# Kangfei/NNGP-src

Hardware: AMD Instinct MI355X
Metric: NNGP kernel-build + GP-solve wall-clock (ms) and GFLOP/s at N train queries (higher is better)
Workload: dtype f32 (Cholesky products as split f16 x3, f32 accumulate; f64 build/CG/means; the posterior's float64-grade residual as exact int8 digit-plane products); 1 GPU; synthetic N=32768, d=128, 5-layer ReLU NNGP + full Cholesky posterior (configs[2], north-star target); N=32768, d=128, n_relu=3, get=nngp, M_test=1024, parallelism=single GPU

## Files before the change

include/nngp_i8s.h:

```cpp
#ifndef NNGP_I8S_H
#define NNGP_I8S_H

#include "nngp_hip.h"

#ifdef __cplusplus
extern "C" {
#endif

int nngp_i8s_cut_rows(const double* src, int64_t ld, int64_t rows, int64_t cols, int32_t ns, const double* scale_in, double* scale_out,
                      int8_t* planes, int64_t ldp, double* writeback, void* stream);

int nngp_i8s_cut_sym(const double* src, int64_t ld, int64_t n, int32_t ns, double* scale_out, int8_t* planes, int64_t ldp,
                     int32_t by_rows, double* sqsum, void* stream);

int nngp_i8s_residual(double* out, int64_t ldo, const double* cin, int64_t ldcin, double* z, int64_t ldz, const double* kmat,
                      int64_t ldk, int64_t mp, int64_t n, double alpha, double beta, double gamma, int32_t ns_z, int32_t ns_k,
                      int32_t cut, int32_t round_z, int32_t sym, float* out32, const double* base, double* var, double* delta,
                      double* zstat, double* floor_rows, double* floor_z, void* stream);

#ifdef __cplusplus
}
#endif

#endif
```

nngp-src_amd/_lib.py:

```python
from __future__ import annotations

import ctypes
import os

import numpy as np

_HERE = os.path.dirname(os.path.abspath(__file__))
LIB_PATH = os.path.join(_HERE, "libnngp_hip.so")
KNOBS_LIB_PATH = os.path.join(_HERE, "libnngp_hip_knobs.so")

GET_NNGP, GET_NTK = 1, 2
DTYPE_F32, DTYPE_F64 = 0, 1
COV_NONE, COV_DIAG, COV_FULL = 0, 1, 2
MAX_DENSE = 16

ABI_SYMBOLS = (
    "nngp_version", "nngp_last_error", "nngp_kernel_build", "nngp_kernel_diag", "nngp_model_create",
    "nngp_model_destroy", "nngp_model_fit", "nngp_model_set_train", "nngp_model_build_rows",
    "nngp_model_factor", "nngp_model_factor_begin", "nngp_model_factor_panel", "nngp_model_factor_update",
    "nngp_model_factor_end", "nngp_model_factor_buffers", "nngp_model_solve", "nngp_model_append", "nngp_model_kernel_buffer", "nngp_model_info",
    "nngp_model_alpha", "nngp_model_predict", "nngp_model_set_refine", "nngp_model_cov_iters", "nngp_model_sweep_estimate", "nngp_model_factor_shift", "nngp_model_prepare_serving", "nngp_potrf_f32", "nngp_gemm_nt_f32",
    "nngp_gemm_nt_h3", "nngp_gemm_nt_f64", "nngp_trsm_rlt_f32", "nngp_model_apply_factor",
    "nngp_model_factor_input_rows", "nngp_model_factor_input_complete", "nngp_model_precond", "nngp_model_matvec_rows", "nngp_model_set_alpha", "nngp_encoder_create", "nngp_encoder_destroy", "nngp_encoder_dim",
    "nngp_encoder_encode", "nngp_comm_unique_id", "nngp_comm_create", "nngp_comm_destroy", "nngp_comm_library",
    "nngp_allgather_rows", "nngp_bcast", "nngp_model_update_timer", "nngp_model_update_timer_read", "nngp_symv_f64",
    "nngp_pool_select", "nngp_model_update_timer_bytes", "nngp_model_factor_update_cols", "nngp_gemm_nt_i8s", "nngp_model_residual_timer", "nngp_model_residual_timer_read", "nngp_model_trsm_timer", "nngp_model_trsm_timer_read", "nngp_model_residual_floor",
    "nngp_trsm_ticket_order", "nngp_trsm_ticket_queues", "nngp_model_reserve", "nngp_alloc_count",
)

GP_ABI_SYMBOLS = (
    "nngp_rbf_gp_create", "nngp_rbf_gp_destroy", "nngp_rbf_gp_set_train", "nngp_rbf_gp_evaluate", "nngp_rbf_gp_terms",
    "nngp_rbf_gp_predict", "nngp_rbf_gp_kernel", "nngp_rbf_gp_factor_buffer", "nngp_potrf_f64",
    "nngp_potrf_dinv_f64", "nngp_trsm_fwd_f64", "nngp_factor_solve_f64",
)


ACT_ABI_SYMBOLS = ("nngp_kernel_build_act", "nngp_kernel_diag_act", "nngp_model_create_act")
ACT_RELU, ACT_ABRELU, ACT_ERF = 0, 1, 2
ACTIVATIONS = {"relu": (ACT_RELU, 0), "abrelu": (ACT_ABRELU, 2), "erf": (ACT_ERF, 3)}

MLL_ABI_SYMBOLS = ("nngp_mll_create", "nngp_mll_destroy", "nngp_mll_set_train", "nngp_mll_evaluate", "nngp_mll_terms",
                   "nngp_mll_factor_buffer")


LOO_ABI_SYMBOLS = ("nngp_mll_loo_evaluate", "nngp_mll_loo_predictions", "nngp_mll_loo_terms")
LOO_NLPD, LOO_MSE = 0, 1

ARD_ABI_SYMBOLS = ("nngp_mll_reserve_ard", "nngp_mll_evaluate_ard", "nngp_mll_loo_evaluate_ard", "nngp_mll_ard_terms")

ADDITIVE_ABI_SYMBOLS = ("nngp_kernel_build_additive", "nngp_kernel_diag_additive", "nngp_model_create_additive")
MAX_GROUPS = 1024

ADDITIVE_MLL_ABI_SYMBOLS = ("nngp_mll_reserve_additive", "nngp_mll_evaluate_additive", "nngp_mll_additive_terms")

POOL_ABI_SYMBOLS = ("nngp_pool_select_greedy",)

SPARSE_ABI_SYMBOLS = ("nngp_sparse_create", "nngp_sparse_destroy", "nngp_sparse_set_inducing", "nngp_sparse_add_rows",
                      "nngp_sparse_finish", "nngp_sparse_predict", "nngp_sparse_info", "nngp_syrk_tn_f64")

SPARSE_EVIDENCE_ABI_SYMBOLS = ("nngp_sparse_reserve_evidence", "nngp_sparse_set_kernel", "nngp_sparse_evidence",
                               "nngp_sparse_evidence_grad", "nngp_sparse_evidence_terms", "nngp_sparse_adjoint_rect")
SPARSE_ARD_ABI_SYMBOLS = ("nngp_sparse_reserve_ard", "nngp_sparse_set_relevance", "nngp_sparse_evidence_grad_ard",
                          "nngp_sparse_ard_terms", "nngp_sparse_ard_rect")
I8S_ABI_SYMBOLS = ("nngp_i8s_cut_rows", "nngp_i8s_cut_sym", "nngp_i8s_residual")
MATFREE_ABI_SYMBOLS = ("nngp_matfree_create", "nngp_matfree_destroy", "nngp_matfree_fit", "nngp_matfree_solve",
                       "nngp_matfree_predict", "nngp_matfree_alpha", "nngp_matfree_info", "nngp_kmv_f64")
BOUND_DTC, BOUND_VFE = 0, 1
BOUNDS = {"dtc": BOUND_DTC, "vfe": BOUND_VFE}


class NngpArch(ctypes.Structure):
    _fields_ = [("n_dense", ctypes.c_int32), ("reserved", ctypes.c_int32),
                ("w_std", ctypes.c_double * MAX_DENSE), ("b_std", ctypes.c_double * MAX_DENSE)]


class NngpArchAct(ctypes.Structure):
    _fields_ = [("base", NngpArch), ("act", ctypes.c_int32 * (MAX_DENSE - 1)),
                ("p", (ctypes.c_double * 3) * (MAX_DENSE - 1))]


class NngpGroups(ctypes.Structure):
    _fields_ = [("n_groups", ctypes.c_int32), ("reserved", ctypes.c_int32),
                ("begin", ctypes.POINTER(ctypes.c_int32)), ("end", ctypes.POINTER(ctypes.c_int32)),
                ("weight", ctypes.POINTER(ctypes.c_double)), ("full_weight", ctypes.c_double)]


class NngpFitInfo(ctypes.Structure):
    _fields_ = [("reg", ctypes.c_double), ("trace_mean", ctypes.c_double), ("rel_residual", ctypes.c_double),
                ("refine_iters", ctypes.c_int32), ("clamped_pivots", ctypes.c_int32),
                ("n", ctypes.c_int64), ("n_padded", ctypes.c_int64)]


class NngpSparseInfo(ctypes.Structure):
    _fields_ = [("n", ctypes.c_int64), ("m", ctypes.c_int64), ("m_padded", ctypes.c_int64), ("chunks", ctypes.c_int64),
                ("sigma2", ctypes.c_double), ("trace_mean", ctypes.c_double), ("jitter_added", ctypes.c_double)]


class NngpMatfreeInfo(ctypes.Structure):
    _fields_ = [("n", ctypes.c_int64), ("m", ctypes.c_int64), ("sigma2", ctypes.c_double), ("iterations", ctypes.c_int32),
                ("k_passes", ctypes.c_int32), ("rel_residual", ctypes.c_double), ("converged", ctypes.c_int32),
                ("restarts", ctypes.c_int32)]


class NngpError(RuntimeError):
    pass


_libs = {}


def load(knobs: bool = False):
    knobs = bool(knobs) or os.environ.get("NNGP_KNOBS", "0") == "1"
    if knobs in _libs:
        return _libs[knobs]
    path = KNOBS_LIB_PATH if knobs else LIB_PATH
    if not os.path.exists(path):
        raise NngpError(
            "%s is missing (%s). Build it with `python -c 'import __graft_entry__ as g; g.build()'` "
            "or `make -C nngp-src_amd/csrc`; there is no CPU fallback." % (os.path.basename(path), path))
    import torch
    lib = ctypes.CDLL(path)
    bind_prototypes(lib, knobs)
    bind_gp_prototypes(lib)
    bind_act_prototypes(lib)
    bind_mll_prototypes(lib)
    bind_loo_prototypes(lib)
    bind_ard_prototypes(lib)
    bind_additive_prototypes(lib)
    bind_additive_mll_prototypes(lib)
    bind_pool_prototypes(lib)
    bind_sparse_prototypes(lib)
    bind_sparse_evidence_prototypes(lib)
    bind_sparse_ard_prototypes(lib)
    bind_i8s_prototypes(lib)
    bind_matfree_prototypes(lib)
    _libs[knobs] = lib
    return lib


def bind_prototypes(lib, knobs: bool = False):
    vp, i64, i32, dbl = ctypes.c_void_p, ctypes.c_int64, ctypes.c_int32, ctypes.c_double
    archp = ctypes.POINTER(NngpArch)
    lib.nngp_version.restype = ctypes.c_int
    lib.nngp_last_error.restype = ctypes.c_char_p
    if knobs:
        lib.nngp_debug_set.argtypes = [i32, i32]
        lib.nngp_debug_set.restype = ctypes.c_int
    lib.nngp_kernel_build.argtypes = [vp, i64, vp, i64, i32, archp, i32, vp, vp, i64, i64, i64, vp]
    lib.nngp_kernel_diag.argtypes = [vp, i64, i32, archp, vp, vp, vp]
    lib.nngp_model_create.argtypes = [ctypes.POINTER(vp), i64, i64, i32, i32, archp, i32, dbl, i32]
    lib.nngp_model_destroy.argtypes = [vp]
    lib.nngp_model_fit.argtypes = [vp, vp, vp, i64, vp]
    lib.nngp_model_set_train.argtypes = [vp, vp, vp, i64, vp]
    lib.nngp_model_build_rows.argtypes = [vp, i64, i64, vp]
    lib.nngp_model_factor.argtypes = [vp, vp]
    lib.nngp_model_factor_begin.argtypes = [vp, vp]
    lib.nngp_model_factor_panel.argtypes = [vp, i64, i64, vp]
    lib.nngp_model_factor_update.argtypes = [vp, i64, i64, i64, i64, vp]
    lib.nngp_model_factor_end.argtypes = [vp, vp]
    lib.nngp_model_factor_buffers.argtypes = [vp, ctypes.POINTER(vp), ctypes.POINTER(i64), ctypes.POINTER(vp)]
    lib.nngp_model_solve.argtypes = [vp, i32, dbl, vp]
    lib.nngp_model_kernel_buffer.argtypes = [vp, ctypes.POINTER(vp), ctypes.POINTER(i64)]
    lib.nngp_model_info.argtypes = [vp, ctypes.POINTER(NngpFitInfo)]
    lib.nngp_model_alpha.argtypes = [vp, vp, vp]
    lib.nngp_model_predict.argtypes = [vp, vp, i64, i32, vp, vp, vp]
    lib.nngp_encoder_create.argtypes = [ctypes.POINTER(vp), ctypes.c_char_p, i32, i32]
    lib.nngp_encoder_destroy.argtypes = [vp]
    lib.nngp_encoder_dim.argtypes = [vp]
    lib.nngp_encoder_encode.argtypes = [vp, ctypes.c_char_p, i64, i32, vp, vp, i64, ctypes.POINTER(i64)]
    lib.nngp_model_set_refine.argtypes = [vp, i32]
    lib.nngp_model_cov_iters.argtypes = [vp]
    lib.nngp_model_prepare_serving.argtypes = [vp, vp]
    lib.nngp_model_factor_shift.argtypes = [vp]
    lib.nngp_model_factor_shift.restype = ctypes.c_double
    lib.nngp_model_cov_iters.restype = ctypes.c_int
    lib.nngp_model_sweep_estimate.argtypes = [vp, ctypes.POINTER(dbl), ctypes.POINTER(dbl)]
    lib.nngp_model_append.argtypes = [vp, vp, vp, i64, vp]
    lib.nngp_gemm_nt_f64.argtypes = [vp, i64, vp, i64, vp, i64, vp, i64, i64, i64, i64, dbl, dbl, vp]
    lib.nngp_gemm_nt_i8s.argtypes = [vp, i64, vp, i64, vp, i64, vp, i64, i64, i64, i64, dbl, dbl, i32, i32, i32, vp]
    lib.nngp_potrf_f32.argtypes = [vp, i64, i64, vp, vp, vp]
    lib.nngp_gemm_nt_f32.argtypes = [vp, i64, vp, i64, vp, i64, i64, i64, i64, ctypes.c_float, ctypes.c_float, i32, vp]
    lib.nngp_gemm_nt_h3.argtypes = [vp, i64, vp, i64, vp, i64, i64, i64, i64, ctypes.c_float, ctypes.c_float,
                                    ctypes.c_float, i32, vp]
    lib.nngp_trsm_rlt_f32.argtypes = [vp, i64, i64, vp, i64, vp, i64, vp]
    lib.nngp_model_apply_factor.argtypes = [vp, vp, i64, i32, vp]
    lib.nngp_model_factor_input_rows.argtypes = [vp, i64, i64, ctypes.c_double, vp]
    lib.nngp_model_factor_input_complete.argtypes = [vp]
    lib.nngp_model_precond.argtypes = [vp, vp, vp, vp]
    lib.nngp_model_matvec_rows.argtypes = [vp, vp, vp, i64, i64, vp]
    lib.nngp_model_set_alpha.argtypes = [vp, vp, i32, ctypes.c_double, vp]
    lib.nngp_comm_unique_id.argtypes = [vp]
    lib.nngp_comm_create.argtypes = [ctypes.POINTER(vp), vp, i32, i32]
    lib.nngp_comm_destroy.argtypes = [vp]
    lib.nngp_comm_library.restype = ctypes.c_char_p
    lib.nngp_allgather_rows.argtypes = [vp, i64, i64, i32, vp, vp]
    lib.nngp_bcast.argtypes = [vp, i64, i32, i32, vp, vp]
    lib.nngp_symv_f64.argtypes = [vp, i64, i64, vp, vp, dbl, vp]
    lib.nngp_pool_select.argtypes = [vp, i64, i32, vp, i64, i32, ctypes.c_uint64, vp, vp]
    lib.nngp_model_update_timer.argtypes = [vp, i32]
    lib.nngp_model_update_timer_read.argtypes = [vp, ctypes.POINTER(i64), ctypes.POINTER(dbl), ctypes.POINTER(dbl)]
    lib.nngp_model_update_timer_bytes.argtypes = [vp, ctypes.POINTER(dbl)]
    lib.nngp_model_residual_timer.argtypes = [vp, i32]
    lib.nngp_model_residual_floor.argtypes = [vp, ctypes.POINTER(dbl), ctypes.POINTER(i32)]
    lib.nngp_model_residual_timer_read.argtypes = [vp, ctypes.POINTER(i64), ctypes.POINTER(dbl), ctypes.POINTER(dbl), ctypes.POINTER(dbl)]
    lib.nngp_model_trsm_timer.argtypes = [vp, i32]
    lib.nngp_model_trsm_timer_read.argtypes = [vp, ctypes.POINTER(i64), ctypes.POINTER(dbl), ctypes.POINTER(dbl)]
    lib.nngp_model_reserve.argtypes = [vp, i64, i32]
    lib.nngp_alloc_count.argtypes = []
    lib.nngp_trsm_ticket_order.argtypes = [i32, i32, i32, i32, i32, i32, vp, i64, ctypes.POINTER(i64)]
    lib.nngp_trsm_ticket_queues.argtypes = [i32, i32, i32, i32, i32, i32, i32, vp, vp, i64, ctypes.POINTER(i64)]
    lib.nngp_model_factor_update_cols.argtypes = [vp, i64, i64, ctypes.POINTER(i64), i32, i64, vp]
    for name in ABI_SYMBOLS:
        if name not in ("nngp_last_error", "nngp_model_factor_shift", "nngp_comm_library", "nngp_alloc_count"):
            getattr(lib, name).restype = ctypes.c_int
    lib.nngp_alloc_count.restype = ctypes.c_int64
    return lib

# ... 8 lines not shown
    lib.nngp_rbf_gp_predict.argtypes = [vp, vp, i64, i32, vp, vp, vp]
    lib.nngp_rbf_gp_kernel.argtypes = [vp, i64, vp, i64, i32, dbl, vp, i64, vp]
    lib.nngp_rbf_gp_factor_buffer.argtypes = [vp, ctypes.POINTER(vp), ctypes.POINTER(i64), ctypes.POINTER(i64)]
    lib.nngp_potrf_f64.argtypes = [vp, i64, i64, vp]
    lib.nngp_potrf_dinv_f64.argtypes = [vp, i64, i64, vp, vp]
    lib.nngp_trsm_fwd_f64.argtypes = [vp, i64, i64, vp, i64, vp, i64, i32, vp]
    lib.nngp_factor_solve_f64.argtypes = [vp, i64, vp, i64, i32, vp, vp, vp, vp, vp, vp, vp]
    for name in GP_ABI_SYMBOLS:
        getattr(lib, name).restype = ctypes.c_int
    return lib


def bind_act_prototypes(lib):
    vp, i64, i32, dbl = ctypes.c_void_p, ctypes.c_int64, ctypes.c_int32, ctypes.c_double
    archp = ctypes.POINTER(NngpArchAct)
    lib.nngp_kernel_build_act.argtypes = [vp, i64, vp, i64, i32, archp, i32, vp, vp, i64, i64, i64, vp]
    lib.nngp_kernel_diag_act.argtypes = [vp, i64, i32, archp, vp, vp, vp]
    lib.nngp_model_create_act.argtypes = [ctypes.POINTER(vp), i64, i64, i32, i32, archp, i32, dbl, i32]
    for name in ACT_ABI_SYMBOLS:
        getattr(lib, name).restype = ctypes.c_int
    return lib


def bind_mll_prototypes(lib):
    vp, i64, i32, dbl = ctypes.c_void_p, ctypes.c_int64, ctypes.c_int32, ctypes.c_double
    lib.nngp_mll_create.argtypes = [ctypes.POINTER(vp), i64, i32]
    lib.nngp_mll_destroy.argtypes = [vp]
    lib.nngp_mll_set_train.argtypes = [vp, vp, vp, i64, i32, vp]
    lib.nngp_mll_evaluate.argtypes = [vp, ctypes.POINTER(NngpArchAct), dbl, i32, ctypes.POINTER(dbl), ctypes.POINTER(dbl), vp]
    lib.nngp_mll_terms.argtypes = [vp, ctypes.POINTER(dbl), i32]
    lib.nngp_mll_factor_buffer.argtypes = [vp, ctypes.POINTER(vp), ctypes.POINTER(i64), ctypes.POINTER(i64)]
    for name in MLL_ABI_SYMBOLS:
        getattr(lib, name).restype = ctypes.c_int
    return lib


def bind_loo_prototypes(lib):
    vp, i32, dbl = ctypes.c_void_p, ctypes.c_int32, ctypes.c_double
    lib.nngp_mll_loo_evaluate.argtypes = [vp, ctypes.POINTER(NngpArchAct), i32, dbl, i32, i32, ctypes.POINTER(dbl),
                                          ctypes.POINTER(dbl), vp]
    lib.nngp_mll_loo_predictions.argtypes = [vp, vp, vp, vp]
    lib.nngp_mll_loo_terms.argtypes = [vp, ctypes.POINTER(dbl), i32]
    for name in LOO_ABI_SYMBOLS:
        getattr(lib, name).restype = ctypes.c_int
    return lib


def bind_ard_prototypes(lib):
    vp, i32, dbl = ctypes.c_void_p, ctypes.c_int32, ctypes.c_double
    pd = ctypes.POINTER(dbl)
    lib.nngp_mll_reserve_ard.argtypes = [vp]
    lib.nngp_mll_evaluate_ard.argtypes = [vp, ctypes.POINTER(NngpArchAct), pd, dbl, i32, pd, pd, pd, vp]
    lib.nngp_mll_loo_evaluate_ard.argtypes = [vp, ctypes.POINTER(NngpArchAct), i32, pd, dbl, i32, i32, pd, pd, pd, vp]
    lib.nngp_mll_ard_terms.argtypes = [vp, pd, i32]
    for name in ARD_ABI_SYMBOLS:
        getattr(lib, name).restype = ctypes.c_int
    return lib


def bind_additive_prototypes(lib):
    vp, i64, i32, dbl = ctypes.c_void_p, ctypes.c_int64, ctypes.c_int32, ctypes.c_double
    archp, groupsp = ctypes.POINTER(NngpArchAct), ctypes.POINTER(NngpGroups)
    lib.nngp_kernel_build_additive.argtypes = [vp, i64, vp, i64, i32, archp, groupsp, i32, vp, vp, i64, i64, i64, vp]
    lib.nngp_kernel_diag_additive.argtypes = [vp, i64, i32, archp, groupsp, vp, vp, vp]
    lib.nngp_model_create_additive.argtypes = [ctypes.POINTER(vp), i64, i64, i32, i32, archp, groupsp, i32, dbl, i32]
    for name in ADDITIVE_ABI_SYMBOLS:
        getattr(lib, name).restype = ctypes.c_int
    return lib


def bind_additive_mll_prototypes(lib):
    vp, i32, dbl = ctypes.c_void_p, ctypes.c_int32, ctypes.c_double
    pd = ctypes.POINTER(dbl)
    lib.nngp_mll_reserve_additive.argtypes = [vp, ctypes.POINTER(NngpGroups)]
    lib.nngp_mll_evaluate_additive.argtypes = [vp, ctypes.POINTER(NngpArchAct), pd, dbl, i32, pd, pd, pd, vp]
    lib.nngp_mll_additive_terms.argtypes = [vp, pd, i32]
    for name in ADDITIVE_MLL_ABI_SYMBOLS:
        getattr(lib, name).restype = ctypes.c_int
    return lib


def bind_pool_prototypes(lib):
    vp, i64, dbl = ctypes.c_void_p, ctypes.c_int64, ctypes.c_double
    lib.nngp_pool_select_greedy.argtypes = [vp, i64, i64, dbl, i64, vp, vp, vp, i64, vp]
    for name in POOL_ABI_SYMBOLS:
        getattr(lib, name).restype = ctypes.c_int
    return lib


def bind_sparse_prototypes(lib):
    vp, i64, i32, dbl = ctypes.c_void_p, ctypes.c_int64, ctypes.c_int32, ctypes.c_double
    lib.nngp_sparse_create.argtypes = [ctypes.POINTER(vp), i64, i64, i64, i32, i32, ctypes.POINTER(NngpArchAct),
                                       ctypes.POINTER(NngpGroups), dbl, i32, dbl]
    lib.nngp_sparse_destroy.argtypes = [vp]
    lib.nngp_sparse_set_inducing.argtypes = [vp, vp, i64, vp]
    lib.nngp_sparse_add_rows.argtypes = [vp, vp, vp, i64, vp]
    lib.nngp_sparse_finish.argtypes = [vp, vp]
    lib.nngp_sparse_predict.argtypes = [vp, vp, i64, i32, vp, vp, vp]
    lib.nngp_sparse_info.argtypes = [vp, ctypes.POINTER(NngpSparseInfo)]
    lib.nngp_syrk_tn_f64.argtypes = [vp, i64, vp, vp, i64, vp, i64, i64, i32, dbl, vp]
    for name in SPARSE_ABI_SYMBOLS:
        getattr(lib, name).restype = ctypes.c_int
    return lib


def bind_sparse_evidence_prototypes(lib):
    vp, i64, i32, dbl = ctypes.c_void_p, ctypes.c_int64, ctypes.c_int32, ctypes.c_double
    pd, archp = ctypes.POINTER(dbl), ctypes.POINTER(NngpArchAct)
    lib.nngp_sparse_reserve_evidence.argtypes = [vp]
    lib.nngp_sparse_set_kernel.argtypes = [vp, archp, dbl, i32]
    lib.nngp_sparse_evidence.argtypes = [vp, i32, pd, vp]
    lib.nngp_sparse_evidence_grad.argtypes = [vp, vp, vp, i64, i32, pd, pd, vp]
    lib.nngp_sparse_evidence_terms.argtypes = [vp, pd, i32]
    lib.nngp_sparse_adjoint_rect.argtypes = [vp, i64, vp, i64, i32, archp, vp, i64, vp, vp, pd, vp]
    for name in SPARSE_EVIDENCE_ABI_SYMBOLS:
        getattr(lib, name).restype = ctypes.c_int
    return lib


def bind_sparse_ard_prototypes(lib):
    vp, i64, i32, dbl = ctypes.c_void_p, ctypes.c_int64, ctypes.c_int32, ctypes.c_double
    pd, archp = ctypes.POINTER(dbl), ctypes.POINTER(NngpArchAct)
    lib.nngp_sparse_reserve_ard.argtypes = [vp]
    lib.nngp_sparse_set_relevance.argtypes = [vp, pd]
    lib.nngp_sparse_evidence_grad_ard.argtypes = [vp, vp, vp, i64, i32, pd, pd, pd, vp]
    lib.nngp_sparse_ard_terms.argtypes = [vp, pd, i32]
    lib.nngp_sparse_ard_rect.argtypes = [vp, i64, vp, i64, i32, archp, pd, vp, i64, vp, vp, pd, vp]
    for name in SPARSE_ARD_ABI_SYMBOLS:
        getattr(lib, name).restype = ctypes.c_int
    return lib


def bind_matfree_prototypes(lib):
    vp, i64, i32, dbl = ctypes.c_void_p, ctypes.c_int64, ctypes.c_int32, ctypes.c_double
    archp = ctypes.POINTER(NngpArchAct)
    lib.nngp_matfree_create.argtypes = [ctypes.POINTER(vp), i64, i64, i64, i64, i32, i32, archp, ctypes.POINTER(NngpGroups), i32, dbl,
                                        i32, dbl]
    lib.nngp_matfree_destroy.argtypes = [vp]
    lib.nngp_matfree_fit.argtypes = [vp, vp, vp, i64, vp, i64, dbl, i32, vp]
    lib.nngp_matfree_solve.argtypes = [vp, vp, i64, i32, vp, i64, dbl, i32, vp]
    lib.nngp_matfree_predict.argtypes = [vp, vp, i64, i32, vp, vp, dbl, i32, vp]
    lib.nngp_matfree_alpha.argtypes = [vp, vp, vp]
    lib.nngp_matfree_info.argtypes = [vp, ctypes.POINTER(NngpMatfreeInfo)]
    lib.nngp_kmv_f64.argtypes = [vp, i64, vp, i64, i32, vp, i64, i32, archp, dbl, vp]
    for name in MATFREE_ABI_SYMBOLS:
        getattr(lib, name).restype = ctypes.c_int
    return lib


def bind_i8s_prototypes(lib):
    vp, i64, i32, dbl = ctypes.c_void_p, ctypes.c_int64, ctypes.c_int32, ctypes.c_double
    lib.nngp_i8s_cut_rows.argtypes = [vp, i64, i64, i64, i32, vp, vp, vp, i64, vp, vp]
    lib.nngp_i8s_cut_sym.argtypes = [vp, i64, i64, i32, vp, vp, i64, i32, vp, vp]
    lib.nngp_i8s_residual.argtypes = [vp, i64, vp, i64, vp, i64, vp, i64, i64, i64, dbl, dbl, dbl, i32, i32, i32, i32, i32,
                                      vp, vp, vp, vp, vp, vp, vp, vp]
    for name in I8S_ABI_SYMBOLS:
        getattr(lib, name).restype = ctypes.c_int
    return lib


def check(rc: int, lib=None):
    if rc != 0:
        msg = (lib or load()).nngp_last_error()
        raise NngpError("libnngp_hip: rc=%d: %s" % (rc, (msg or b"").decode("utf-8", "replace")))


def make_arch(w_std, b_std) -> NngpArch:
    w_std = [float(v) for v in w_std]
    b_std = [float(v) for v in b_std]
    if len(w_std) != len(b_std) or not 1 <= len(w_std) <= MAX_DENSE:
        raise ValueError("architecture must have 1..%d Dense layers" % MAX_DENSE)
    arch = NngpArch()
    arch.n_dense = len(w_std)
    for i, (w, b) in enumerate(zip(w_std, b_std)):
        arch.w_std[i] = w
        arch.b_std[i] = b
    return arch


def canonical_activation(spec):
    kind = spec[0]
    if kind == "relu":
        return ("relu",)
    if kind == "abrelu" and len(spec) == 3:
        a, b = float(spec[1]), float(spec[2])
        return ("relu",) if (a == 0.0 and b == 1.0) else ("abrelu", a, b)
    if kind == "erf" and len(spec) == 4:
        return ("erf", float(spec[1]), float(spec[2]), float(spec[3]))
    raise ValueError("unknown activation %r" % (spec,))


def all_relu(activations) -> bool:
    return activations is None or all(canonical_activation(a) == ("relu",) for a in activations)


def make_arch_act(w_std, b_std, activations) -> NngpArchAct:
    arch = NngpArchAct()
    arch.base = make_arch(w_std, b_std)
    activations = list(activations)
    if len(activations) != arch.base.n_dense - 1:
        raise ValueError("%d Dense layers need %d activations, got %d" % (arch.base.n_dense, arch.base.n_dense - 1,
                                                                          len(activations)))
    for l, spec in enumerate(activations):
        spec = canonical_activation(spec)
        arch.act[l] = ACTIVATIONS[spec[0]][0]
        for e, v in enumerate(spec[1:]):
            arch.p[l][e] = v
    return arch


def pair_groups(d: int):
    d = int(d)
    if d < 2 or d % 2 != 0:
        raise ValueError("pair groups need an even number of features >= 2, got d = %d" % d)
    return tuple((i, i + 2) for i in range(0, d, 2))


def check_groups(groups, weights=None, full_weight=1.0, d=None):
    if isinstance(groups, str):
        if groups != "pairs":
            raise ValueError("groups must be a list of (begin, end) ranges or 'pairs', got %r" % (groups,))
        if d is None:
            raise ValueError("groups='pairs' needs the number of features")
        groups = pair_groups(d)
    try:
        out = tuple((int(b), int(e)) for b, e in groups)
        if any(float(b) != ib or float(e) != ie for (b, e), (ib, ie) in zip(groups, out)):
            raise TypeError
    except (TypeError, ValueError):
        raise ValueError("groups must be a list of (begin, end) integer ranges, got %r" % (groups,)) from None
    if len(out) > MAX_GROUPS:
        raise ValueError("at most %d groups, got %d" % (MAX_GROUPS, len(out)))
    for b, e in out:
        if not (0 <= b < e) or (d is not None and e > int(d)):
            raise ValueError("group range [%d, %d) is outside 0 <= begin < end%s" % (b, e, "" if d is None else " <= d = %d" % int(d)))
    w = (1.0,) * len(out) if weights is None else tuple(float(v) for v in weights)
    if len(w) != len(out):
        raise ValueError("%d groups need %d weights, got %d" % (len(out), len(out), len(w)))
    w0 = float(full_weight)
    if not all(np.isfinite(v) and v >= 0.0 for v in w + (w0,)):
        raise ValueError("group weights and full_weight must be finite and >= 0")
    if w0 == 0.0 and not any(v > 0.0 for v in w):
        raise ValueError("all weights are zero: the additive kernel has no term")
    return out, w, w0


def make_groups(groups, weights, full_weight) -> NngpGroups:
    g = NngpGroups()
    n = len(groups)
    g.n_groups = n
    g._begin = (ctypes.c_int32 * max(n, 1))(*[b for b, _ in groups])
    g._end = (ctypes.c_int32 * max(n, 1))(*[e for _, e in groups])
    g._weight = (ctypes.c_double * max(n, 1))(*weights)
    g.begin = ctypes.cast(g._begin, ctypes.POINTER(ctypes.c_int32))
    g.end = ctypes.cast(g._end, ctypes.POINTER(ctypes.c_int32))
    g.weight = ctypes.cast(g._weight, ctypes.POINTER(ctypes.c_double))
    g.full_weight = float(full_weight)
    return g


def require_gpu():
    import torch
    if not torch.cuda.is_available():
        raise NngpError("no MI355X/ROCm device visible: the NNGP hot path has no CPU fallback")
    return torch.device("cuda", torch.cuda.current_device())


def to_device_f64(a, device=None):
    import torch
    device = device or require_gpu()
    if isinstance(a, torch.Tensor):
        return a.to(device=device, dtype=torch.float64).contiguous()
    return torch.from_numpy(np.ascontiguousarray(a, dtype=np.float64)).to(device)


def stream_ptr():
    import torch
    return ctypes.c_void_p(torch.cuda.current_stream().cuda_stream)


def ptr(t):
    return ctypes.c_void_p(0 if t is None else t.data_ptr())
```

nngp-src_amd/csrc/api_ops.hip:

```cpp
#include "model.h"
#include "gp_f64.h"
#include "trsm_order.h"
#include "../../include/nngp_i8s.h"

extern "C" {

int nngp_trsm_ticket_order(int32_t row_tiles, int32_t block_cols, int32_t tail_tiles, int32_t backward, int32_t workers, int32_t merged,
                           int32_t* items, int64_t cap, int64_t* count) {
    return tk_order_export(row_tiles, block_cols, tail_tiles, backward, workers, merged, 1, items, nullptr, cap, count);
}

int nngp_trsm_ticket_queues(int32_t row_tiles, int32_t block_cols, int32_t tail_tiles, int32_t backward, int32_t workers, int32_t merged,
                            int32_t queues, int32_t* items, int32_t* queue_of, int64_t cap, int64_t* count) {
    return tk_order_export(row_tiles, block_cols, tail_tiles, backward, workers, merged, queues, items, queue_of, cap, count);
}

int nngp_potrf_f32(float* a, int64_t n, int64_t ld, float* dinv, int32_t* clamped, void* stream) {
    NNGP_REQUIRE(a != nullptr && dinv != nullptr, "potrf_f32: NULL argument");
    if (clamped) NNGP_HIP_CHECK(hipMemsetAsync(clamped, 0, sizeof(int32_t), (hipStream_t)stream));
    return potrf_f32(a, n, ld, dinv, clamped, 0.0f, (hipStream_t)stream);
}

int nngp_potrf_f64(double* a, int64_t n, int64_t ld, void* stream) {
    hipStream_t s = (hipStream_t)stream;
// ... 54 lines not shown
    if (l) NNGP_HIP_CHECK(hipMemcpyAsync(l, w->a, mat, hipMemcpyDeviceToDevice, s));
    if (wout) NNGP_HIP_CHECK(hipMemcpyAsync(wout, w->wrow, vec, hipMemcpyDeviceToDevice, s));
    if (zt) NNGP_HIP_CHECK(hipMemcpyAsync(zt, w->zt, mat, hipMemcpyDeviceToDevice, s));
    if (ainv) NNGP_HIP_CHECK(hipMemcpyAsync(ainv, w->ainv, mat, hipMemcpyDeviceToDevice, s));
    if (alpha) NNGP_HIP_CHECK(hipMemcpyAsync(alpha, w->alpha, vec, hipMemcpyDeviceToDevice, s));
    NNGP_HIP_CHECK(hipStreamSynchronize(s));
    return 0;
}
}

int nngp_factor_solve_f64(const double* a, int64_t lda, const double* y, int64_t n, int32_t mode, double* l, double* w, double* zt,
                          double* ainv, double* alpha, double* neg_rowsq, void* stream) {
    hipStream_t s = (hipStream_t)stream;
    NNGP_REQUIRE(a != nullptr && y != nullptr && n >= 1 && lda >= n, "factor_solve_f64: need a, y, n >= 1 and lda >= n (n=%lld lda=%lld)",
                 (long long)n, (long long)lda);
    NNGP_REQUIRE(mode == kGpSolveW || mode == kGpSolveInverse || mode == kGpSolveRows, "factor_solve_f64: unknown mode %d", (int)mode);
    NNGP_REQUIRE(mode != kGpSolveW || (zt == nullptr && alpha == nullptr && neg_rowsq == nullptr),
                 "factor_solve_f64: mode 0 produces L and w only");
    NNGP_REQUIRE(mode == kGpSolveInverse || ainv == nullptr, "factor_solve_f64: only mode 1 produces A^-1");
    GpWorkspace ws;
    const int rc = factor_solve_on(&ws, a, lda, y, n, mode, l, w, zt, ainv, alpha, neg_rowsq, s);
    if (rc != 0) (void)hipStreamSynchronize(s);
    ws_free(&ws);
    return rc;
}

int nngp_gemm_nt_f32(float* c, int64_t ldc, const float* a, int64_t lda, const float* b, int64_t ldb, int64_t m,
                     int64_t n, int64_t k, float alpha, float beta, int32_t lower_only, void* stream) {
    NNGP_REQUIRE(a != nullptr && b != nullptr && c != nullptr, "gemm_nt_f32: NULL argument");
    return launch_gemm_nt_f32(c, ldc, a, lda, b, ldb, m, n, k, alpha, beta, lower_only != 0, (hipStream_t)stream);
}

namespace {
struct H3Scratch {
    hipStream_t stream = nullptr;
    char* p = nullptr;
    size_t bytes = 0;
    bool used = false;
};
std::mutex g_h3_scratch_mutex;
H3Scratch g_h3_scratch[4];

int h3_scratch_get(hipStream_t s, size_t bytes, char** out) {
    std::lock_guard<std::mutex> lock(g_h3_scratch_mutex);
    H3Scratch* e = nullptr;
    for (auto& c : g_h3_scratch)
        if (c.used && c.stream == s) e = &c;
    if (e == nullptr)
        for (auto& c : g_h3_scratch)
            if (!c.used && e == nullptr) e = &c;
    if (e == nullptr) {
        e = &g_h3_scratch[0];
        if (hipStreamSynchronize(e->stream) != hipSuccess) {
            (void)hipGetLastError();
            NNGP_HIP_CHECK(hipDeviceSynchronize());
        }
        (void)hipFree(e->p);
        *e = H3Scratch();
    }
    if (e->bytes < bytes) {
        if (e->p != nullptr) {
            NNGP_HIP_CHECK(hipStreamSynchronize(s));
            (void)hipFree(e->p);
            e->p = nullptr;
            e->bytes = 0;
        }
        NNGP_HIP_CHECK(hipMalloc((void**)&e->p, bytes));
        e->bytes = bytes;
    }
    e->used = true;
    e->stream = s;
    *out = e->p;
    return 0;
}
}

int nngp_gemm_nt_h3(float* c, int64_t ldc, const float* a, int64_t lda, const float* b, int64_t ldb, int64_t m, int64_t n,
                    int64_t k, float alpha, float beta, float scale, int32_t lower_only, void* stream) {
    hipStream_t s = (hipStream_t)stream;
    NNGP_REQUIRE(a != nullptr && b != nullptr && c != nullptr && scale > 0.0f, "gemm_nt_h3: bad argument");
    NNGP_REQUIRE(m > 0 && n > 0 && k > 0 && k % 32 == 0, "gemm_nt_h3: k must be a multiple of 32");
    const int64_t mp = round_up(m, 256), np = round_up(n, 256), ldp = 4 * k;
    char* pa = nullptr;
    NNGP_TRY(h3_scratch_get(s, (size_t)((mp + np) * ldp + 64), &pa));
    char* pb = pa + mp * ldp;
    int* counters = reinterpret_cast<int*>(pb + np * ldp);
    if (mp > m) NNGP_HIP_CHECK(hipMemsetAsync(pa + m * ldp, 0, (size_t)((mp - m) * ldp), s));
    NNGP_HIP_CHECK(hipMemsetAsync(pb + n * ldp, 0, (size_t)((np - n) * ldp + 64), s));
    NNGP_TRY(launch_split_rows(a, lda, m, k, scale, pa, ldp, s));
    NNGP_TRY(launch_split_rows(b, ldb, n, k, scale, pb, ldp, s));
    return launch_gemm_nt_h3(c, ldc, pa, pb, ldp, m, n, k, alpha / (scale * scale), beta, lower_only != 0, 0, counters,
                             NNGP_KNOB(4) > 0 ? NNGP_KNOB(4) : 0, s);
}

int nngp_gemm_nt_f64(double* c, int64_t ldc, const double* cin, int64_t ldcin, const double* a, int64_t lda,
                     const double* b, int64_t ldb, int64_t m, int64_t n, int64_t k, double alpha, double beta,
                     void* stream) {
    NNGP_REQUIRE(a != nullptr && b != nullptr && c != nullptr, "gemm_nt_f64: NULL argument");
    return launch_gemm_nt_f64(c, ldc, cin, ldcin, a, lda, b, ldb, m, n, k, alpha, beta, (hipStream_t)stream);
}

int nngp_gemm_nt_i8s(double* c, int64_t ldc, const double* cin, int64_t ldcin, const double* a, int64_t lda, const double* b,
                     int64_t ldb, int64_t m, int64_t n, int64_t k, double alpha, double beta, int32_t slices_a, int32_t slices_b,
                     int32_t cut, void* stream) {
    hipStream_t s = (hipStream_t)stream;
    NNGP_REQUIRE(a != nullptr && b != nullptr && c != nullptr && m > 0 && n > 0 && k > 0 && m % TB == 0 && n % TB == 0 && ldc >= n &&
                     lda >= k && ldb >= k,
                 "gemm_nt_i8s: m, n must be multiples of %d", TB);
    I8Plan pl;
    NNGP_TRY(i8s_plan(slices_a, slices_b, cut, &pl));
    const int64_t mp = round_up(m, 256), np = round_up(n, 256), kp = round_up(k, 128);
    const int64_t nchunk = i8s_chunks(k, &pl);
    const int64_t slab = m * n;
    const size_t plane_bytes = (size_t)((mp * slices_a + np * slices_b) * kp);
    const size_t part_bytes = (size_t)(nchunk * pl.ndiag * slab) * sizeof(int32_t);
    NNGP_REQUIRE(part_bytes < (size_t)16 << 30, "gemm_nt_i8s: the test entry keeps all partial products (16 GB limit)");
    char* ws = nullptr;
    NNGP_HIP_CHECK(hipMalloc((void**)&ws, plane_bytes + part_bytes + sizeof(double) * (size_t)(m + n) + 64));
    NNGP_HIP_CHECK(hipMemsetAsync(ws, 0, plane_bytes, s));
    int8_t* pa = reinterpret_cast<int8_t*>(ws);
    int8_t* pb = pa + mp * slices_a * kp;
    int32_t* part = reinterpret_cast<int32_t*>(ws + plane_bytes);
    double* sca = reinterpret_cast<double*>(ws + plane_bytes + part_bytes);
    double* scb = sca + m;
    int* counters = reinterpret_cast<int*>(scb + n);
    NNGP_HIP_CHECK(hipMemsetAsync(counters, 0, 64, s));
    int rc = launch_i8s_slice_rows(a, lda, m, k, slices_a, nullptr, sca, pa, kp, mp * kp, s);
    if (rc == 0) rc = launch_i8s_slice_rows(b, ldb, n, k, slices_b, nullptr, scb, pb, kp, np * kp, s);
    if (rc == 0)
        rc = launch_gemm_nt_i8s(part, n, slab, pa, kp, mp * kp, pb, kp, np * kp, pl, m, n, k, counters,
                                NNGP_KNOB(4) > 0 ? NNGP_KNOB(4) : 0, s);
    if (rc == 0)
        rc = launch_i8s_combine(c, ldc, cin ? cin : c, cin ? ldcin : ldc, beta, alpha, nullptr, 0, 0.0, part, n, slab, (int)nchunk,
                                pl.ndiag, sca, scb, m, n, s);
    (void)hipStreamSynchronize(s);
    (void)hipFree(ws);
    return rc;
}

int nngp_i8s_cut_rows(const double* src, int64_t ld, int64_t rows, int64_t cols, int32_t ns, const double* scale_in, double* scale_out,
                      int8_t* planes, int64_t ldp, double* writeback, void* stream) {
    NNGP_REQUIRE(src != nullptr && planes != nullptr && (scale_in != nullptr || scale_out != nullptr), "i8s_cut_rows: NULL argument");
    NNGP_REQUIRE(ns >= 2 && ns <= 7, "i8s_cut_rows: 2..7 planes (ns=%d)", (int)ns);
    NNGP_REQUIRE(rows > 0 && cols > 0 && ld >= cols && ld % 2 == 0, "i8s_cut_rows: ld must be even and >= cols (rows=%lld cols=%lld ld=%lld)",
                 (long long)rows, (long long)cols, (long long)ld);
    NNGP_REQUIRE(ldp >= round_up(cols, 128) && ldp % 16 == 0, "i8s_cut_rows: ldp must be a multiple of 16 and >= cols rounded up to 128 (ldp=%lld)",
                 (long long)ldp);
    NNGP_REQUIRE((((uintptr_t)src | (uintptr_t)planes | (uintptr_t)writeback) & 15) == 0, "i8s_cut_rows: operands must be 16-byte aligned");
    return launch_i8s_slice_rows(src, ld, rows, cols, ns, scale_in, scale_out, planes, ldp, rows * ldp, (hipStream_t)stream, writeback);
}

int nngp_i8s_cut_sym(const double* src, int64_t ld, int64_t n, int32_t ns, double* scale_out, int8_t* planes, int64_t ldp,
                     int32_t by_rows, double* sqsum, void* stream) {
    hipStream_t s = (hipStream_t)stream;
    NNGP_REQUIRE(src != nullptr && planes != nullptr && scale_out != nullptr, "i8s_cut_sym: NULL argument");
    NNGP_REQUIRE(by_rows != 0 ? (ns >= 2 && ns <= 7) : (ns == 5 || ns == 7), "i8s_cut_sym: 5 or 7 planes (by rows: 2..7) (ns=%d)", (int)ns);
    NNGP_REQUIRE(n > 0 && n % TB == 0 && ld >= n && ld % 2 == 0, "i8s_cut_sym: n must be a positive multiple of %d, ld even and >= n (n=%lld ld=%lld)",
                 TB, (long long)n, (long long)ld);
    NNGP_REQUIRE(ldp >= n && ldp % 16 == 0, "i8s_cut_sym: ldp must be a multiple of 16 and >= n (ldp=%lld)", (long long)ldp);
    NNGP_REQUIRE((((uintptr_t)src | (uintptr_t)planes) & 15) == 0, "i8s_cut_sym: operands must be 16-byte aligned");
    NNGP_TRY(launch_i8s_diag_bound_scale(src, ld, n, scale_out, s));
    if (by_rows != 0)
        NNGP_TRY(launch_i8s_slice_rows(src, ld, n, n, ns, scale_out, nullptr, planes, ldp, n * ldp, s));
    else
        NNGP_TRY(launch_i8s_slice_sym(src, ld, n, ns, scale_out, planes, ldp, n * ldp, s));
    if (sqsum != nullptr) NNGP_TRY(launch_i8s_scale_sqsum(scale_out, n, sqsum, s));
    return 0;
}

namespace {
struct I8sResidualWs {
    int8_t *kplanes, *zplanes;
    double *kscale, *zscale, *rowpart;
    int32_t* partial;
    int* counters;
};

int i8s_residual_on(const I8sResidualWs& w, const I8Plan& pl, double* out, int64_t ldo, const double* cin, int64_t ldcin, double* z, int64_t ldz,
                    const double* kmat, int64_t ldk, int64_t mp, int64_t n, double alpha, double beta, double gamma, int ns_z, int ns_k,
                    bool round_z, bool sym, float* out32, const double* base, double* var, double* delta, double* zstat,
                    double* floor_rows, double* floor_z, hipStream_t s) {
    const int64_t kr = round_up(n, 256), zr = round_up(mp, 256);
    NNGP_TRY(launch_i8s_diag_bound_scale(kmat, ldk, n, w.kscale, s));
    if (sym)
        NNGP_TRY(launch_i8s_slice_sym(kmat, ldk, n, ns_k, w.kscale, w.kplanes, n, kr * n, s));
    else
        NNGP_TRY(launch_i8s_slice_rows(kmat, ldk, n, n, ns_k, w.kscale, nullptr, w.kplanes, n, kr * n, s));
    NNGP_TRY(launch_i8s_scale_sqsum(w.kscale, n, w.kscale + n, s));
    const int64_t nchunk = i8s_chunks(n, &pl), slab = mp * n;
    NNGP_TRY(launch_i8s_slice_rows(z, ldz, mp, n, ns_z, nullptr, w.zscale, w.zplanes, n, zr * n, s, round_z ? z : nullptr));
    NNGP_TRY(launch_gemm_nt_i8s(w.partial, n, slab, w.zplanes, n, zr * n, w.kplanes, n, kr * n, pl, mp, n, n, w.counters, 0, s));
    I8Fuse fuse;
    fuse.out32 = out32;
    fuse.ld32 = n;
    fuse.part = w.rowpart;
    NNGP_TRY(launch_i8s_combine(out, ldo, cin, ldcin, beta, alpha, z, ldz, gamma, w.partial, n, slab, (int)nchunk, pl.ndiag, w.zscale,
                                w.kscale, mp, n, s, out32 != nullptr ? &fuse : nullptr));
    if (out32 != nullptr) {
        NNGP_TRY(launch_i8s_rowstat_finish(w.rowpart, n, mp, base, var, delta, zstat, s));
        if (floor_rows != nullptr) {
            NNGP_HIP_CHECK(hipMemsetAsync(floor_rows, 0, sizeof(double), s));
            NNGP_TRY(launch_i8s_floor_ratio_rows(zstat, mp, var, pl, ns_z, ns_k, w.kscale + n, reinterpret_cast<unsigned long long*>(floor_rows), s));
        }
        if (floor_z != nullptr) {
            NNGP_HIP_CHECK(hipMemsetAsync(floor_z, 0, sizeof(double), s));
            NNGP_TRY(launch_i8s_floor_ratio(z, ldz, mp, n, var, pl, ns_z, ns_k, w.kscale + n, reinterpret_cast<unsigned long long*>(floor_z), s));
        }
    }
    return 0;
}
}

int nngp_i8s_residual(double* out, int64_t ldo, const double* cin, int64_t ldcin, double* z, int64_t ldz, const double* kmat,
                      int64_t ldk, int64_t mp, int64_t n, double alpha, double beta, double gamma, int32_t ns_z, int32_t ns_k,
                      int32_t cut, int32_t round_z, int32_t sym, float* out32, const double* base, double* var, double* delta,
                      double* zstat, double* floor_rows, double* floor_z, void* stream) {
    hipStream_t s = (hipStream_t)stream;
    NNGP_REQUIRE(out != nullptr && z != nullptr && kmat != nullptr && (beta == 0.0 || cin != nullptr), "i8s_residual: NULL argument");
    NNGP_REQUIRE(mp > 0 && n > 0 && mp % TB == 0 && n % TB == 0, "i8s_residual: mp, n must be positive multiples of %d (mp=%lld n=%lld)", TB,
                 (long long)mp, (long long)n);
    NNGP_REQUIRE(ns_z >= 2 && ns_z <= 7 && ns_k >= 2 && ns_k <= 7, "i8s_residual: 2..7 planes per operand (ns_z=%d ns_k=%d)", (int)ns_z, (int)ns_k);
    NNGP_REQUIRE(cut >= 0, "i8s_residual: cut must be >= 0 (cut=%d)", (int)cut);
    NNGP_REQUIRE(sym == 0 || ns_k == 5 || ns_k == 7, "i8s_residual: the symmetric cut makes 5 or 7 planes (ns_k=%d)", (int)ns_k);
    NNGP_REQUIRE(ldo >= n && ldz >= n && ldk >= n && (cin == nullptr || ldcin >= n) && ldo % 2 == 0 && ldz % 2 == 0 && ldk % 2 == 0 &&
                     (cin == nullptr || ldcin % 2 == 0),
                 "i8s_residual: leading dimensions must be even and >= n (ldo=%lld ldcin=%lld ldz=%lld ldk=%lld)", (long long)ldo,
                 (long long)ldcin, (long long)ldz, (long long)ldk);
    NNGP_REQUIRE((((uintptr_t)out | (uintptr_t)cin | (uintptr_t)z | (uintptr_t)kmat | (uintptr_t)out32) & 15) == 0,
                 "i8s_residual: operands must be 16-byte aligned");
    const bool any = out32 || base || var || delta || zstat, all = out32 && base && var && delta && zstat;
    NNGP_REQUIRE(any == all, "i8s_residual: the fused outputs (out32, base, var, delta, zstat) come all or none");
    NNGP_REQUIRE(!all || cin != nullptr, "i8s_residual: the fused outputs need cin");
    NNGP_REQUIRE(all || (floor_rows == nullptr && floor_z == nullptr), "i8s_residual: the floor ratios need the fused outputs");
    I8Plan pl;
    NNGP_TRY(i8s_plan(ns_z, ns_k, cut, &pl));
    const int64_t kr = round_up(n, 256), zr = round_up(mp, 256), nchunk = i8s_chunks(n, &pl);
    const size_t kp_bytes = (size_t)(ns_k * kr * n), zp_bytes = (size_t)(ns_z * zr * n);
    const size_t part_bytes = (size_t)(nchunk * pl.ndiag * mp * n) * sizeof(int32_t);
    const size_t f64s = (size_t)(n + 2) + (size_t)mp + (size_t)(mp * i8s_col_blocks(n) * 4);
    NNGP_REQUIRE(part_bytes < (size_t)16 << 30, "i8s_residual: the test entry keeps all partial products (16 GB limit)");
    char* ws = nullptr;
    NNGP_HIP_CHECK(hipMallocAsync(reinterpret_cast<void**>(&ws), kp_bytes + zp_bytes + part_bytes + sizeof(double) * f64s + 64, s));
    I8sResidualWs w;
    w.kplanes = reinterpret_cast<int8_t*>(ws);
    w.zplanes = w.kplanes + kp_bytes;
    w.partial = reinterpret_cast<int32_t*>(ws + kp_bytes + zp_bytes);
    w.kscale = reinterpret_cast<double*>(ws + kp_bytes + zp_bytes + part_bytes);
    w.zscale = w.kscale + n + 2;
    w.rowpart = w.zscale + mp;
    w.counters = reinterpret_cast<int*>(w.rowpart + mp * i8s_col_blocks(n) * 4);
    int rc = 0;
    if (hipMemsetAsync(ws, 0, kp_bytes + zp_bytes, s) != hipSuccess || hipMemsetAsync(w.counters, 0, 64, s) != hipSuccess) {
        nngp::set_error("i8s_residual: hipMemsetAsync failed");
        rc = -1;
    }
    if (rc == 0)
        rc = i8s_residual_on(w, pl, out, ldo, cin, ldcin, z, ldz, kmat, ldk, mp, n, alpha, beta, gamma, ns_z, ns_k, round_z != 0, sym != 0,
                             out32, base, var, delta, zstat, floor_rows, floor_z, s);
    (void)hipFreeAsync(ws, s);
    return rc;
}

int nngp_pool_select(const double* mean, int64_t m, int32_t ny, const double* var, int64_t count, int32_t biased, uint64_t seed,
                     int64_t* indices, void* stream) {
    hipStream_t s = (hipStream_t)stream;
    NNGP_REQUIRE(mean != nullptr && var != nullptr && indices != nullptr && m > 0 && ny >= 1 && count >= 0 && count <= m,
                 "pool_select: bad arguments (m=%lld, count=%lld)", (long long)m, (long long)count);
    if (count == 0) return 0;
    double* key = nullptr;
    NNGP_HIP_CHECK(hipMallocAsync(reinterpret_cast<void**>(&key), sizeof(double) * (size_t)m, s));
    const int rc = launch_pool_select(mean, m, ny, var, count, biased != 0, seed, key, indices, s);
    NNGP_HIP_CHECK(hipFreeAsync(key, s));
    return rc;
}

int nngp_pool_select_greedy(const double* cov, int64_t m, int64_t ld, double noise, int64_t count, int64_t* indices, double* gains,
                            double* factor, int64_t ldf, void* stream) {
    hipStream_t s = (hipStream_t)stream;
    NNGP_REQUIRE(cov != nullptr && indices != nullptr, "pool_select_greedy: NULL cov or indices");
    NNGP_REQUIRE(m >= 1 && count >= 0 && count <= m, "pool_select_greedy: need m >= 1 and 0 <= count <= m (m=%lld, count=%lld)",
                 (long long)m, (long long)count);
    NNGP_REQUIRE(ld >= m, "pool_select_greedy: ld < m (ld=%lld, m=%lld)", (long long)ld, (long long)m);
    NNGP_REQUIRE(factor == nullptr || ldf >= m, "pool_select_greedy: ldf < m (ldf=%lld, m=%lld)", (long long)ldf, (long long)m);
    NNGP_REQUIRE(noise >= 0.0 && noise <= 1.7976931348623157e308, "pool_select_greedy: noise must be finite and >= 0 (noise=%g)", noise);
    if (count == 0) return 0;
    const size_t own = (factor == nullptr) ? (size_t)count * (size_t)m : 0;
    double* ws = nullptr;
    NNGP_HIP_CHECK(hipMallocAsync(reinterpret_cast<void**>(&ws), sizeof(double) * ((size_t)2 * (size_t)m + own), s));
    const int rc = launch_pool_greedy(cov, m, ld, noise, count, indices, gains, own ? ws + 2 * m : factor, own ? m : ldf, ws, s);
    NNGP_HIP_CHECK(hipFreeAsync(ws, s));
    return rc;
}

int nngp_syrk_tn_f64(double* c, int64_t ldc, double* r, const double* a, int64_t lda, const double* y, int64_t rows, int64_t mp,
                     int32_t ny, double beta, void* stream) {
    hipStream_t s = (hipStream_t)stream;
    NNGP_TRY(syrk_check(c, ldc, r, a, lda, y, rows, mp, ny, beta));
    double* ws = nullptr;
    const int64_t ws_doubles = syrk_ws_doubles(rows, mp);
    NNGP_HIP_CHECK(hipMallocAsync(reinterpret_cast<void**>(&ws), sizeof(double) * (size_t)ws_doubles, s));
    const int rc = launch_syrk_tn_f64(c, ldc, r, a, lda, y, rows, mp, ny, beta, ws, ws_doubles, s);
    NNGP_HIP_CHECK(hipFreeAsync(ws, s));
    return rc;
}

int nngp_symv_f64(const double* a, int64_t lda, int64_t n, const double* x, double* y, double diag_add, void* stream) {
    hipStream_t s = (hipStream_t)stream;
    NNGP_REQUIRE(a != nullptr && x != nullptr && y != nullptr && n > 0 && lda >= n, "symv_f64: bad arguments");
    const int64_t np = round_up(n, TB);
    double* part = nullptr;
    NNGP_HIP_CHECK(hipMallocAsync(reinterpret_cast<void**>(&part), sizeof(double) * (size_t)(np / TB) * np, s));
    const int rc = launch_symv_f64(a, lda, n, x, y, diag_add, part, np, s);
    NNGP_HIP_CHECK(hipFreeAsync(part, s));
    return rc;
}

int nngp_trsm_rlt_f32(float* b, int64_t ldb, int64_t m, const float* l, int64_t ldl, const float* dinv, int64_t n,
                      void* stream) {
    NNGP_REQUIRE(b != nullptr && l != nullptr && dinv != nullptr, "trsm_rlt_f32: NULL argument");
    NNGP_REQUIRE(m % TB == 0 && n % TB == 0 && m > 0 && n > 0, "trsm_rlt_f32: m, n must be multiples of %d", TB);
    return trsm_rlt_f32(b, ldb, m, l, ldl, dinv, n, (hipStream_t)stream);
}

}
```

nngp-src_amd/csrc/api_predict.hip:

```cpp
#include "model.h"

namespace nngp {

int ensure_predict_capacity(nngp_model* m, int64_t mt, bool need_ktd) {
    if (mt > m->m_cap || m->b32 == nullptr) {
        const int64_t cap = mt > m->m_cap ? mt : m->m_cap;
        NNGP_HIP_CHECK(hipDeviceSynchronize());
        dev_free(m->xt_q); dev_free(m->tt_diag); dev_free(m->b32); dev_free(m->trsm_tmp);
        NNGP_TRY(dev_alloc(&m->xt_q, cap));
        NNGP_TRY(dev_alloc(&m->tt_diag, cap));
        NNGP_TRY(dev_alloc(&m->b32, round_up(cap, TB) * m->np_cap));
        NNGP_TRY(dev_alloc(&m->trsm_tmp, round_up(cap, TB) * triinv_block(m->np_cap)));
        if (m->split.planes != nullptr) {
            dev_free(m->split.planes_b); dev_free(m->split.row_inv);
            m->split.planes_b = nullptr; m->split.row_inv = nullptr;
            m->split.mb_cap = round_up(cap, TB);
            m->split.b_panels = (int)((triinv_block(m->np_cap) + m->split.k_cap - 1) / m->split.k_cap);
            NNGP_TRY(dev_alloc(&m->split.planes_b, (int64_t)(m->split.b_panels - 1) * m->split.col_stride + (m->split.mb_cap + 256) * m->split.k_cap * 4));
            NNGP_TRY(dev_alloc(&m->split.row_inv, m->split.mb_cap));
            tk_destroy(m->tk);
            m->tk = nullptr;
            if (m->split.k_cap == 1024 && triinv_block(m->np_cap) == 1024) NNGP_TRY(tk_create(&m->tk, m->np_cap, m->split.mb_cap) < 0 ? -1 : 0);
        }
        m->m_cap = cap;
    }
    if (need_ktd && mt > m->ktd_cap) {
        const int64_t cap = mt > m->m_cap ? mt : m->m_cap;
        NNGP_HIP_CHECK(hipDeviceSynchronize());
        dev_free(m->ktd64);
        NNGP_TRY(dev_alloc(&m->ktd64, round_up(cap, TB) * m->np_cap));
        m->ktd_cap = cap;
    }
    return 0;
}

int ensure_full_cov_capacity(nngp_model* m, int64_t mt) {
    if (mt > m->full_cap) {
        NNGP_HIP_CHECK(hipDeviceSynchronize());
        dev_free(m->ktt64); dev_free(m->vvt32);
        const int64_t mp = round_up(mt, TB);
        dev_free(m->covp64);
        NNGP_TRY(dev_alloc(&m->ktt64, mp * mp));
        NNGP_TRY(dev_alloc(&m->vvt32, mp * mp));
        NNGP_TRY(dev_alloc(&m->covp64, mp * mp));
        m->full_cap = mt;
    }
    return 0;
}

void set_split_scale(nngp_model* m) {
    const double lmax = sqrt(fmax(m->diag_max, m->trace_mean) + m->reg_fac);
    int e = 0;
    (void)frexp(lmax, &e);
    m->split.scale = (lmax > 0.0 && std::isfinite(lmax)) ? (float)ldexp(1.0, 15 - e) : 1.0f;
}

int ensure_refine_capacity(nngp_model* m, int64_t mp) {
    if (mp > m->refine_cap) {
        NNGP_HIP_CHECK(hipDeviceSynchronize());
        dev_free(m->z64); dev_free(m->r64);
        NNGP_TRY(dev_alloc(&m->z64, mp * m->np_cap));
        NNGP_TRY(dev_alloc(&m->r64, mp * m->np_cap));
        m->refine_cap = mp;
    }
    if (mp > m->rows.cap) {
        NNGP_HIP_CHECK(hipDeviceSynchronize());
        RowsPcg& w = m->rows;
        dev_free(w.rho); dev_free(w.coef); dev_free(w.tol); dev_free(w.delta); dev_free(w.var); dev_free(w.state); dev_free(w.zstat);
        NNGP_TRY(dev_alloc(&w.rho, mp)); NNGP_TRY(dev_alloc(&w.coef, mp)); NNGP_TRY(dev_alloc(&w.tol, mp));
        NNGP_TRY(dev_alloc(&w.delta, mp)); NNGP_TRY(dev_alloc(&w.var, mp)); NNGP_TRY(dev_alloc(&w.state, mp));
        NNGP_TRY(dev_alloc(&w.zstat, 2 * mp));
        if (w.live == nullptr) {
            NNGP_TRY(dev_alloc(&w.live, 6));
            NNGP_HIP_CHECK(hipHostMalloc(reinterpret_cast<void**>(&w.host), 6 * sizeof(int32_t), hipHostMallocDefault));
        }
        w.cap = mp;
    }
    return 0;
}

int ensure_lt_alloc(nngp_model* m) {
    if (m->lt32 != nullptr) return 0;
    NNGP_HIP_CHECK(hipDeviceSynchronize());
    NNGP_TRY(dev_alloc(&m->lt32, m->np_cap * m->np_cap));
    NNGP_TRY(dev_alloc(&m->dinvt, (m->np_cap / TB) * TB * TB));
    return 0;
}
int ensure_lt(nngp_model* m, hipStream_t s) {
    if (m->lt_ready) return 0;
    NNGP_TRY(ensure_lt_alloc(m));
    NNGP_TRY(launch_transpose_f32(m->a32, m->ld, m->lt32, m->np, m->np, s));
    NNGP_TRY(launch_transpose_blocks_f32(m->dinv, m->dinvt, TB, m->np / TB, s));
    m->lt_ready = true;
    return 0;
}

int ensure_lt_split(nngp_model* m, hipStream_t s) {
    if (m->split.lt_ready) return 0;
    if (m->split.planes_t == nullptr) {
        NNGP_HIP_CHECK(hipDeviceSynchronize());
        const int64_t ncols = (m->np_cap + m->split.k_cap - 1) / m->split.k_cap;
        NNGP_TRY(dev_alloc(&m->split.planes_t, ncols * m->split.col_stride));
    }
    NNGP_TRY(launch_split_lower_t(m->a32, m->ld, m->np, m->split.k_cap, m->split.scale, m->split.planes_t,
                                  m->split.col_stride, s));
    m->split.lt_ready = true;
    return 0;
}


int tri_join(nngp_model* m, hipStream_t s) {
    if (m->tri_stale) {
        if (m->ev_tri == nullptr) NNGP_HIP_CHECK(hipEventCreateWithFlags(&m->ev_tri, hipEventDisableTiming));
        NNGP_TRY(triinv_build(m->a32, m->ld, m->dinv, m->np, m->tri, s));
        if (m->tk != nullptr && m->tri.bs == 1024) NNGP_TRY(tk_prepare_inverses(m->tk, m->tri, m->np, m->a32, m->ld, s));
        NNGP_HIP_CHECK(hipEventRecord(m->ev_tri, s));
        m->tri_stale = false;
        m->tri_pending = true;
        return 0;
    }
    if (m->tri_pending) NNGP_HIP_CHECK(hipStreamWaitEvent(s, m->ev_tri, 0));
    if (m->tk != nullptr && !tk_inverses_ready(m->tk) && m->tri.bs == 1024) {
        NNGP_TRY(tk_prepare_inverses(m->tk, m->tri, m->np, m->a32, m->ld, s));
        if (m->ev_tri == nullptr) NNGP_HIP_CHECK(hipEventCreateWithFlags(&m->ev_tri, hipEventDisableTiming));
        NNGP_HIP_CHECK(hipEventRecord(m->ev_tri, s));
        m->tri_pending = true;
    }
    return 0;
}

int tri_fork(nngp_model* m, hipStream_t s) {
    if (!m->tri_stale || m->la == nullptr || m->la->panel == nullptr || NNGP_KNOB(5) == 61) return 0;
    if (m->ev_tri == nullptr) NNGP_HIP_CHECK(hipEventCreateWithFlags(&m->ev_tri, hipEventDisableTiming));
    if (m->ev_tri_fork == nullptr) NNGP_HIP_CHECK(hipEventCreateWithFlags(&m->ev_tri_fork, hipEventDisableTiming));
    NNGP_HIP_CHECK(hipEventRecord(m->ev_tri_fork, s));
    NNGP_HIP_CHECK(hipStreamWaitEvent(m->la->panel, m->ev_tri_fork, 0));
    NNGP_TRY(triinv_build(m->a32, m->ld, m->dinv, m->np, m->tri, m->la->panel));
    if (m->tk != nullptr && m->tri.bs == 1024) NNGP_TRY(tk_prepare_inverses(m->tk, m->tri, m->np, m->a32, m->ld, m->la->panel));
    NNGP_HIP_CHECK(hipEventRecord(m->ev_tri, m->la->panel));
    m->tri_stale = false;
    m->tri_pending = true;
    return 0;
}

bool use_split_solves(const nngp_model* m, int64_t mp) {
    return m->split.l_ready && m->split.planes_b != nullptr && mp <= m->split.mb_cap && m->tri.bs % m->split.k_cap == 0 &&
           m->tri.bs / m->split.k_cap <= m->split.b_panels && m->tri.bs <= 2048 && NNGP_KNOB(7) == 0 && mp >= 256 && mp * m->np >= 7000000;
}

bool use_tickets(const nngp_model* m, int64_t mp) {
    return !m->tk_failed && m->tri.bs == 1024 && tk_usable(m->tk, mp, m->np) && NNGP_KNOB(9) != 16;
}

SolvePath solve_path(const nngp_model* m, int64_t mp) {
    if (NNGP_KNOB(7) == 1) return SolvePath::Recursion128;
    if (!use_split_solves(m, mp)) return SolvePath::BlocksF32;
    return use_tickets(m, mp) ? SolvePath::Tickets : SolvePath::BlocksH3;
}

struct TicketSchedule { int gate, reserve, cutstream; };
static const TicketSchedule& ticket_schedule() {
#ifdef NNGP_TIMING_KNOBS
    auto env = [](const char* name, int dflt) { const char* v = getenv(name); return v ? atoi(v) : dflt; };
    static const TicketSchedule t = {env("NNGP_TK_GATE", 1), env("NNGP_TK_RESERVE", 0), env("NNGP_TK_CUTSTREAM", 2)};
#else
    static const TicketSchedule t = {1, 0, 2};
#endif
    return t;
}

bool cg_from_the_start(const nngp_model* m, int64_t mp) { return ticket_schedule().gate != 0 && solve_path(m, mp) == SolvePath::Tickets; }

int tickets_reserve(const nngp_model* m) { return m->i8.k_pending ? ticket_schedule().reserve : 0; }

hipStream_t early_cut_stream(const nngp_model* m, int64_t mp) {
    const int cut_stream = ticket_schedule().cutstream;
    hipStream_t cs = m->solve_stream;
    if (cut_stream != 0 && cg_from_the_start(m, mp) && m->la != nullptr && m->la->panel != nullptr)
        cs = (cut_stream == 2 && m->la->update != nullptr) ? m->la->update : m->la->panel;
    return cs;
}

int tickets_check(nngp_model* m, bool wait) {
    const int e = tk_poll_error(m->tk, wait);
    if (e == 0) return 0;
    m->tk_failed = true;
    set_error("a persistent blocked solve gave up waiting for a dependency (error word 0x%x): its results are invalid; the model now uses the step-by-step solves", e);
    return -6;
}

static int trsm_timer_begin(nngp_model* m, int64_t mp, hipStream_t s, int* slot) {
    NNGP_TRY(m->trsm_t.begin(s, slot));
    if (*slot >= 0) m->trsm_flops[*slot] = (double)m->np * (double)m->np * (double)mp;
    return 0;
}

static int apply_forward_untimed(nngp_model* m, int64_t mp, hipStream_t s);

int apply_forward_f32(nngp_model* m, int64_t mp, hipStream_t s) {
    NNGP_TRY(tickets_check(m, false));
    NNGP_TRY(tri_join(m, s));
    int slot = -1;
    NNGP_TRY(trsm_timer_begin(m, mp, s, &slot));
    NNGP_TRY(apply_forward_untimed(m, mp, s));
    return m->trsm_t.end(slot);
}

static int apply_forward_untimed(nngp_model* m, int64_t mp, hipStream_t s) {
    m->split.solve_reserve = (m->alpha_solve.gate_recorded && NNGP_KNOB(13) > 0) ? NNGP_KNOB(13) : 0;
    switch (solve_path(m, mp)) {
    case SolvePath::Recursion128: return trsm_rlt_f32(m->b32, m->np, mp, m->a32, m->ld, m->dinv, m->np, s);
    case SolvePath::Tickets: return tk_solve(m->tk, m->b32, m->np, mp, m->np, m->split, false, s, tickets_reserve(m));
    case SolvePath::BlocksH3: return trsm_rlt_blocks_h3(m->b32, m->np, mp, m->a32, m->ld, m->tri, m->np, m->trsm_tmp, m->split, s);
    case SolvePath::BlocksF32: break;
    }
    return trsm_rlt_blocks_f32(m->b32, m->np, mp, m->a32, m->ld, m->tri, m->np, m->trsm_tmp, s);
}

int apply_inverse_f32(nngp_model* m, int64_t mp, hipStream_t s) {
    const bool lt_aside = !needs_lt32(solve_path(m, mp)) && !m->split.lt_ready && m->split.planes_t != nullptr &&
                          m->ev_lt != nullptr && NNGP_KNOB(2) != 7;
    if (lt_aside) {
        NNGP_HIP_CHECK(hipEventRecord(m->ev_lt, s));
        NNGP_HIP_CHECK(hipStreamWaitEvent(m->solve_stream, m->ev_lt, 0));
        NNGP_TRY(ensure_lt_split(m, m->solve_stream));
        NNGP_HIP_CHECK(hipEventRecord(m->ev_lt, m->solve_stream));
    }
    NNGP_TRY(apply_forward_f32(m, mp, s));
    if (NNGP_KNOB(2) == 10 && !m->alpha_solve.gate_recorded && m->alpha_solve.plan.pending) {
        NNGP_TRY(record_cg_gate(m, s));
    }
    if (lt_aside) NNGP_HIP_CHECK(hipStreamWaitEvent(s, m->ev_lt, 0));
    const SolvePath path = solve_path(m, mp);
    if (needs_lt32(path)) NNGP_TRY(ensure_lt(m, s));
    else NNGP_TRY(ensure_lt_split(m, s));
    if (path == SolvePath::Recursion128) return trsm_rut_f32(m->b32, m->np, mp, m->lt32, m->np, m->dinvt, m->np, s);
    int slot = -1;
    NNGP_TRY(trsm_timer_begin(m, mp, s, &slot));
    if (path == SolvePath::Tickets)
        NNGP_TRY(tk_solve(m->tk, m->b32, m->np, mp, m->np, m->split, true, s, tickets_reserve(m)));
    else if (path == SolvePath::BlocksH3)
        NNGP_TRY(trsm_rut_blocks_h3(m->b32, m->np, mp, m->lt_ready ? m->lt32 : nullptr, m->np, m->tri, m->np, m->trsm_tmp, m->split, s));
    else
        NNGP_TRY(trsm_rut_blocks_f32(m->b32, m->np, mp, m->lt32, m->np, m->tri, m->np, m->trsm_tmp, s));
    return m->trsm_t.end(slot);
}

static int ntk_sweeps(const nngp_model* m) { return m->var_refine < 2 ? 2 : m->var_refine; }

int refined_solve_rows(nngp_model* m, const double* rhs, int64_t mp, int sweeps, bool final_residual, hipStream_t s,
                       bool measure, ResidualNote* note) {
    const int64_t np = m->np;
    measure = measure && sweeps >= 2;
    NNGP_TRY(launch_convert_f64_f32(rhs, np, m->b32, np, mp, np, mp, np, s));
    NNGP_TRY(apply_inverse_f32(m, mp, s));
    NNGP_TRY(launch_f32_to_f64_mat(m->b32, np, m->z64, np, mp, np, false, s));
    for (int it = 0; it < sweeps + (final_residual ? 1 : 0); ++it) {
        NNGP_TRY(residual_rows(m, m->r64, rhs, m->z64, mp, s, it == 0, note));
        if (it == sweeps) break;
        NNGP_TRY(launch_convert_f64_f32(m->r64, np, m->b32, np, mp, np, mp, np, s));
        NNGP_TRY(apply_inverse_f32(m, mp, s));
        if (measure && it < 2) NNGP_TRY(launch_rows_energy(m->r64, m->b32, np, mp, np, it == 0 ? m->rows.var : m->rows.delta, s));
        NNGP_TRY(launch_f32_to_f64_mat(m->b32, np, m->z64, np, mp, np, true, s));
    }
    if (measure) NNGP_TRY(launch_rowdot_f64(m->z64, nullptr, 0.0, rhs, np, mp, np, nullptr, 1.0, m->rows.tol, s));
    return 0;
}

int rows_pcg_continue(nngp_model* m, int64_t mp, int max_iters, hipStream_t s) {
    const int64_t np = m->np;
    RowsPcg& w = m->rows;
    if (mp > m->rows_pq_cap) {
        NNGP_HIP_CHECK(hipDeviceSynchronize());
        dev_free(w.p); dev_free(w.q);
        w.p = w.q = nullptr;
        NNGP_TRY(dev_alloc(&w.p, mp * m->np_cap));
        NNGP_TRY(dev_alloc(&w.q, mp * m->np_cap));
        m->rows_pq_cap = mp;
    }
    m->cov_iters = 0;
    for (int it = 0; it < max_iters; ++it) {
        NNGP_TRY(launch_convert_f64_f32(m->r64, np, m->b32, np, mp, np, mp, np, s));
        NNGP_TRY(apply_inverse_f32(m, mp, s));
        NNGP_TRY(launch_rows_rho(m->r64, m->b32, np, mp, np, it == 0, w, s));
        NNGP_TRY(launch_rows_update_p(w.p, m->b32, np, mp, np, w, s));
        NNGP_TRY(launch_gemm_nt_f64(w.q, np, w.p, np, w.p, np, m->k64, m->ld, mp, np, np, 1.0, m->reg, s));
        NNGP_TRY(launch_rows_alpha(w.p, w.q, np, mp, np, w, s));
        NNGP_TRY(launch_rows_axpy2(m->z64, m->r64, w.p, w.q, np, mp, np, w, s));
        NNGP_HIP_CHECK(hipMemcpyAsync(w.host, w.live, sizeof(int32_t), hipMemcpyDeviceToHost, s));
        NNGP_HIP_CHECK(hipStreamSynchronize(s));
        m->cov_iters = it + 1;
        if (w.host[0] == 0) break;
    }
    return 0;
}

int build_cross(nngp_model* m, const double* xt, const double* qt, int64_t mt, int64_t mp, bool nngp, double* out,
                hipStream_t s) {
    NNGP_HIP_CHECK(hipMemsetAsync(out, 0, sizeof(double) * mp * m->np, s));
    BuildArgs a{};
    a.x1 = xt; a.x2 = m->x; a.q1 = qt; a.q2 = m->q;
    a.n1 = mt; a.n2 = m->n; a.d = m->d;
    a.row_begin = 0; a.row_end = mt; a.sym = 0;
    a.ld64 = a.ld32 = m->np;
    if (nngp) a.nngp64 = out; else a.ntk64 = out;
    return launch_kernel_build(a, m->arch, s);
}

struct ScopedFlag {
    bool& f;
    explicit ScopedFlag(bool& b) : f(b) { f = true; }
    ~ScopedFlag() { f = false; }
    ScopedFlag(const ScopedFlag&) = delete;
};

static int continuation_budget(const nngp_model* m) {
    const double shift = (m->reg > 0.0 && m->reg_fac > m->reg) ? sqrt(m->reg_fac / m->reg) : 1.0;
    return (int)fmin(1000.0, 80.0 * shift);
}


static double row_flag_threshold() {
    return (NNGP_KNOB(6) >= 2 && NNGP_KNOB(6) <= 30) ? pow(10.0, -(double)NNGP_KNOB(6)) : 1e-8;
}
constexpr double kSweepEstThr = 3e-7;

static int predict_open(nngp_model* m, const double* x_test, int64_t mt, int32_t cov_mode, double* mean, double* var_or_cov,
                        hipStream_t s, PredictCall& c) {
    NNGP_REQUIRE(m != nullptr && m->alpha_solve.plan.solved, "predict: fit the model first");
    NNGP_REQUIRE(cov_mode >= NNGP_COV_NONE && cov_mode <= NNGP_COV_FULL, "predict: bad cov_mode");
    NNGP_REQUIRE(mean != nullptr && (cov_mode == NNGP_COV_NONE || var_or_cov != nullptr), "predict: NULL output");
    c.on_train = (x_test == nullptr);
    if (c.on_train) mt = m->n;
    NNGP_REQUIRE(mt >= 0, "predict: negative row count");
    NNGP_REQUIRE(!m->k64_partial || (cov_mode == NNGP_COV_NONE && !c.on_train),
                 "predict: this model holds only its own kernel rows (row-sharded layout): it serves means of test rows; covariances are "
                 "formed by the caller from nngp_model_apply_factor and its row block (shard32.py)");
    c.s = s; c.mt = mt; c.mp = round_up(mt, TB); c.mean = mean; c.var_or_cov = var_or_cov;
    c.xt = c.on_train ? m->x : x_test; c.qt = m->q; c.ktd = m->k64;
    c.compact_train = c.on_train && m->ld != m->np;
    c.is_ntk = (m->get == NNGP_GET_NTK);
    c.want_cov = (cov_mode != NNGP_COV_NONE); c.full = (cov_mode == NNGP_COV_FULL);
    c.serving = m->serving_ready && !c.is_ntk;
    if (mt == 0) return 0;
    return ensure_predict_capacity(m, mt, !c.on_train || c.compact_train);
}

static int build_cross_kernel(nngp_model* m, PredictCall& c) {
    const int64_t np = m->np;
    if (!c.on_train) {
        NNGP_TRY(launch_row_sqnorm(c.xt, c.mt, m->d, m->xt_q, c.s));
        c.qt = m->xt_q;
        NNGP_TRY(build_cross(m, c.xt, c.qt, c.mt, c.mp, !c.is_ntk, m->ktd64, c.s));
        c.ktd = m->ktd64;
    }
    if (c.compact_train) {
        NNGP_HIP_CHECK(hipMemsetAsync(m->ktd64, 0, sizeof(double) * c.mp * np, c.s));
        NNGP_HIP_CHECK(hipMemcpy2DAsync(m->ktd64, sizeof(double) * np, m->k64, sizeof(double) * m->ld, sizeof(double) * np, c.mt,
                                        hipMemcpyDeviceToDevice, c.s));
        c.ktd = m->ktd64;
    }
    return 0;
}


static int build_ktt(nngp_model* m, const PredictCall& c) {
    BuildArgs a = symmetric_build_args(c.xt, c.qt, c.mt, m->d);
    a.ld64 = a.ld32 = c.mp;
    a.nngp64 = m->ktt64;
    return launch_kernel_build(a, m->arch, c.s);
}

static int solve_cross_rows(nngp_model* m, const PredictCall& c, int sweeps, bool final_residual, ResidualNote* note = nullptr) {
    const int64_t np = m->np;
    if (!c.serving) return refined_solve_rows(m, c.ktd, c.mp, sweeps, final_residual, c.s, false, note);
    NNGP_TRY(launch_gemm_nt_f64(m->z64, np, nullptr, 0, c.ktd, np, m->ainv64, np, c.mp, np, np, 1.0, 0.0, c.s));
    if (m->serving_weak) {
        NNGP_TRY(residual_rows(m, m->r64, c.ktd, m->z64, c.mp, c.s, false, note));
        NNGP_TRY(launch_gemm_nt_f64(m->z64, np, m->z64, np, m->r64, np, m->ainv64, np, c.mp, np, np, 1.0, 1.0, c.s));
    }
    if (final_residual) NNGP_TRY(residual_rows(m, m->r64, c.ktd, m->z64, c.mp, c.s, false, note));
    return 0;
}

static int cov_float32_only(nngp_model* m, PredictCall& c) {
    const int64_t np = m->np, mt = c.mt, mp = c.mp;
    NNGP_TRY(launch_convert_f64_f32(c.ktd, np, m->b32, np, mp, np, mp, np, c.s));
    NNGP_TRY(apply_forward_f32(m, mp, c.s));
    if (!c.full) return launch_row_sqsum_f32(m->b32, np, mt, np, m->tt_diag, c.var_or_cov, c.s);
    NNGP_TRY(build_ktt(m, c));
    NNGP_TRY(launch_gemm_nt_f32(m->vvt32, mp, m->b32, np, m->b32, np, mp, mp, np, 1.0f, 0.0f, false, c.s));
    return launch_cov_finish(m->ktt64, mp, m->vvt32, mp, mt, c.var_or_cov, c.s);
}
// ... 291 lines not shown
```

nngp-src_amd/csrc/common.h:

```cpp
#pragma once
#include <hip/hip_runtime.h>
#include <stdint.h>
#include <atomic>
#include <stdio.h>
#include <string.h>

#include "../../include/nngp_hip.h"
#include "../../include/nngp_rbf_gp.h"
#include "../../include/nngp_activations.h"
#include "../../include/nngp_mll.h"
#include "../../include/nngp_additive.h"
#include "../../include/nngp_pool.h"
#include "../../include/nngp_sparse.h"

namespace nngp {

constexpr int TB = 128;

void set_error(const char* fmt, ...);
void note_alloc();
#ifdef NNGP_TIMING_KNOBS
extern std::atomic<int> g_knobs[16];
#define NNGP_KNOB(i) (nngp::g_knobs[i].load(std::memory_order_relaxed))
#else
// ... 71 lines not shown
    a.x1 = a.x2 = x;
    a.q1 = a.q2 = q;
    a.n1 = a.n2 = n;
    a.d = d;
    a.row_begin = 0;
    a.row_end = n;
    a.sym = 1;
    return a;
}
int launch_row_sqnorm(const double* x, int64_t n, int d, double* q, hipStream_t s);
int launch_diag_from_q(const double* q, int64_t n, const ArchDev& arch, double* dn, double* dt, hipStream_t s);
int launch_kernel_build(const BuildArgs& a, const ArchDev& arch, hipStream_t s);
int launch_kernel_build_plain(const BuildArgs& a, const ArchDev& arch, hipStream_t s);
int launch_kernel_diag(const double* x, const double* q, int64_t n, int d, const ArchDev& arch, double* dn, double* dt,
                       hipStream_t s);

int groups_create(const nngp_groups* g, int d, GroupsDev* out, bool* plain);
void groups_destroy(GroupsDev* g);
int launch_kernel_build_additive(const BuildArgs& a, const ArchDev& arch, hipStream_t s);
int launch_diag_additive(const double* x, const double* q, int64_t n, int d, const ArchDev& arch, double* dn, double* dt,
                         hipStream_t s);

int launch_gemm_nt_f32(float* c, int64_t ldc, const float* a, int64_t lda, const float* b, int64_t ldb,
                       int64_t m, int64_t n, int64_t k, float alpha, float beta, bool lower_only, hipStream_t s, int tri = 0);

int launch_gemm_nt_f32_batched(float* c, int64_t ldc, const float* a, int64_t lda, const float* b, int64_t ldb,
                               int64_t m, int64_t n, int64_t k, float alpha, float beta, bool lower_only, int batch,
                               int64_t stride_c, int64_t stride_a, int64_t stride_b, hipStream_t s, int tri = 0);

int launch_split_rows(const float* p, int64_t ld, int64_t rows, int64_t k, float scale, char* out, int64_t out_ld,
                      hipStream_t s);
int launch_split_rows_rowscale(const float* src, int64_t ld_src, int64_t rows, int64_t k, float* copy_dst, int64_t ld_copy,
                               char* out, int64_t out_ld, float* row_inv, hipStream_t s, int64_t pan_stride = 0);
int launch_split_lower_t(const float* l, int64_t ld, int64_t n, int64_t bs, float scale, char* out, int64_t col_stride,
                         hipStream_t s);
int launch_gemm_nt_h3(float* c, int64_t ldc, const char* a, const char* b, int64_t ldp, int64_t m, int64_t n, int64_t k,
                      float alpha, float beta, bool lower_only, int64_t diag_shift, int* counters, int reserve_cus,
                      hipStream_t s, const float* row_alpha = nullptr);
struct H3RegionSpec {
    int64_t row0, col0, m, n, shift;
};
int launch_gemm_nt_h3r(float* c, int64_t ldc, const char* a, const char* b, int64_t ldp, int64_t pstride, int npanels, int64_t lead,
                       const H3RegionSpec* spec, int nreg, int64_t k, float alpha, float beta, bool lower_only, int* counters,
                       int reserve_cus, hipStream_t s, const float* row_alpha = nullptr, int helper = 0);
int launch_gemm_nt_h3x(float* c, int64_t ldc, const char* a, const char* b, int64_t ldp, int64_t pstride, int npanels, int64_t lead,
                       int64_t m, int64_t n, int64_t k, float alpha, float beta, bool lower_only, int64_t diag_shift, int* counters,
                       int reserve_cus, hipStream_t s, const float* row_alpha = nullptr);

int launch_potrf_leaf(float* a, int64_t ld, float* dinv_block, int32_t* clamped, float pivot_floor, hipStream_t s);
int potrf_f32(float* a, int64_t n, int64_t ld, float* dinv, int32_t* clamped, float pivot_floor, hipStream_t s);
int potrf_rec(float* a, int64_t n, int64_t ld, float* dinv, int32_t* clamped, float pivot_floor, hipStream_t s);
int trsm_rlt_f32(float* b, int64_t ldb, int64_t m, const float* l, int64_t ldl, const float* dinv, int64_t n,
                 hipStream_t s);
int trsm_rut_f32(float* b, int64_t ldb, int64_t m, const float* lt, int64_t ldl, const float* dinvt, int64_t n,
                 hipStream_t s);

int launch_trsm_panel_f32(float* b, int64_t ldb, int64_t m, const float* l, int64_t ldl, const float* dinv, int64_t w,
                          char* planes, int64_t ldp, float scale, hipStream_t s, char* planes_t = nullptr, int64_t tstride = 0,
                          int64_t row0 = 0, int64_t col0 = 0);
int launch_split_diag_frag(const float* a, int64_t ld, int64_t w, float scale, char* out, const float* dinv, float* dfrag,
                           float* dscale, hipStream_t s);
int launch_trsm_panel_h3(float* b, int64_t ldb, int64_t m, const char* lfrag, const float* dfrag, const float* dscale, int64_t w,
                         char* planes, int64_t ldp, float scale, hipStream_t s, char* planes_t = nullptr, int64_t tstride = 0,
                         int64_t row0 = 0, int64_t col0 = 0);


struct SplitWork {
    char* planes = nullptr;
    int64_t rows_cap = 0, k_cap = 0, col_stride = 0;
    float scale = 1.0f;
    int* counters = nullptr;
    bool l_ready = false;
    int64_t split_panel = -1;
    char* ldiag = nullptr;
    float* dfrag = nullptr;
    float* dscale = nullptr;
    char* planes_t = nullptr;
    bool lt_ready = false;
    char* planes_b = nullptr;
    int b_panels = 1;
    int solve_reserve = 0;
    float* row_inv = nullptr;
    int64_t mb_cap = 0;
};

struct LookAhead {
    static constexpr int kMaxSteps = 64;
    hipStream_t panel = nullptr, update = nullptr;
    hipStream_t bulk = nullptr;
    hipStream_t aux = nullptr;
    hipStream_t side = nullptr;
    hipEvent_t ev_side_done = nullptr;
    int prio_levels = 0;
    bool masked = false;
    hipEvent_t ev_in = nullptr, ev_panel_done = nullptr, ev_update_done = nullptr;
    hipEvent_t ev_panel[kMaxSteps] = {}, ev_col[kMaxSteps] = {};
    hipEvent_t ev_chunk[kMaxSteps] = {}, ev_helper[kMaxSteps] = {};
    hipEvent_t ev_far[kMaxSteps] = {}, ev_near[kMaxSteps] = {}, ev_tc[kMaxSteps] = {}, ev_tb[kMaxSteps] = {}, ev_split[kMaxSteps] = {},
               ev_gp[kMaxSteps] = {};
    hipEvent_t ev_c1[kMaxSteps] = {};
    hipEvent_t ev_chain[kMaxSteps] = {};
    hipEvent_t ev_bulk_done = nullptr;
    static constexpr int kMaxTimed = 320;
    bool time_updates = false;
    hipEvent_t tu0[kMaxTimed] = {}, tu1[kMaxTimed] = {};
    int tu_count = 0;
    double tu_flops[kMaxTimed] = {};
    double tu_bytes[kMaxTimed] = {};
};
int lookahead_create(LookAhead** out);
void lookahead_destroy(LookAhead* la);
struct TriInv;
int potrf_lookahead_f32(float* a, int64_t n, int64_t ld, float* dinv, int32_t* clamped, float pivot_floor,
                        LookAhead* la, SplitWork* sw, hipStream_t user, TriInv* ti = nullptr);
constexpr int64_t kLookAheadNb = 1024;
constexpr int kLookAheadGroup = 4;
int potrf_panel_f32(float* a, int64_t n, int64_t ld, float* dinv, int32_t* clamped, float pivot_floor, int64_t o,
                    int64_t w, hipStream_t s, SplitWork* sw = nullptr);
int potrf_update_f32(float* a, int64_t n, int64_t ld, int64_t po, int64_t pw, int64_t o, int64_t w, hipStream_t s,
                     SplitWork* sw = nullptr);
int potrf_update_cols_f32(float* a, int64_t n, int64_t ld, int64_t po, int64_t pw, const int64_t* cols, int ncols, int64_t w,
                          hipStream_t s, SplitWork* sw = nullptr);

struct I8Plan {
    int ndiag, npairs;
    int dstart[9];
    int pa[32], pb[32];
};
struct I8Planes {
    int8_t* planes = nullptr;
    double* scale = nullptr;
    bool ready = false;
    int ns_done = 0;
    int alloc_planes = 0;
};
struct I8Work {
    I8Planes k, aux;
    int64_t k_rows = 0;
    int8_t* zplanes = nullptr;
    double* zscale = nullptr;
    int64_t z_rows = 0;
    int z_planes = 0;
    int32_t* partial = nullptr;
    double* rowpart = nullptr;
    int64_t rowpart_rows = 0;
    int* counters = nullptr;
    int ns_k = 5, ns_z = 5, cut = 4;
    static constexpr int kMaxTimed = 64;
    double t_ops[kMaxTimed] = {};
    double t_flops[kMaxTimed] = {};
};
int i8s_plan(int nsa, int nsb, int cut, I8Plan* pl);
int64_t i8s_chunks(int64_t k, const I8Plan* pl = nullptr);
int launch_i8s_diag_bound_scale(const double* src, int64_t ld, int64_t n, double* scale, hipStream_t s);
int launch_i8s_scale_sqsum(const double* scale, int64_t n, double* out, hipStream_t s);
int launch_i8s_floor_ratio(const double* z, int64_t ld, int64_t rows, int64_t cols, const double* var, const I8Plan& pl, int nsa, int nsb,
                           const double* sk2, unsigned long long* out, hipStream_t s);
int launch_i8s_floor_ratio_rows(const double* zstat, int64_t rows, const double* var, const I8Plan& pl, int nsa, int nsb, const double* sk2,
                                unsigned long long* out, hipStream_t s);
int launch_i8s_slice_rows(const double* src, int64_t ld, int64_t rows, int64_t cols, int ns, const double* scale_in, double* scale_out,
                          int8_t* planes, int64_t ldp, int64_t pstride, hipStream_t s, double* writeback = nullptr);
int launch_i8s_slice_sym(const double* src, int64_t ld, int64_t n, int ns, const double* scale, int8_t* planes, int64_t ldp,
                         int64_t pstride, hipStream_t s);
int launch_gemm_nt_i8s(int32_t* partial, int64_t ldc, int64_t slab, const int8_t* a, int64_t lda, int64_t sa, const int8_t* b,
                       int64_t ldb, int64_t sb, const I8Plan& pl, int64_t m, int64_t n, int64_t k, int* counters, int reserve_cus,
                       hipStream_t s);
struct I8Fuse {
    float* out32 = nullptr;
    int64_t ld32 = 0;
    double* part = nullptr;
};
int64_t i8s_col_blocks(int64_t cols);
int launch_i8s_combine(double* out, int64_t ldo, const double* cin, int64_t ldcin, double beta, double alpha, const double* g,
                       int64_t ldg, double gamma, const int32_t* partial, int64_t ldc, int64_t slab, int nchunk, int ndiag,
                       const double* sa, const double* sb, int64_t rows, int64_t cols, hipStream_t s, const I8Fuse* fuse = nullptr);
int launch_i8s_rowstat_finish(const double* part, int64_t cols, int64_t rows, const double* base, double* var, double* delta,
                              double* zstat, hipStream_t s);

int launch_gemm_nt_f64(double* c, int64_t ldc, const double* cin, int64_t ldcin, const double* a, int64_t lda,
                       const double* b, int64_t ldb, int64_t m, int64_t n, int64_t k, double alpha, double beta,
                       hipStream_t s, int kmode = 0);

int launch_transpose_blocks_f32(const float* src, float* dst, int64_t bs, int64_t count, hipStream_t s);
struct TriInv {
    int64_t bs = 0;
    float* tinv = nullptr;
    float* xinv = nullptr;
    float* partial = nullptr;
    float* tmp = nullptr;
    int64_t done_blocks = 0;
};
int64_t triinv_block(int64_t np);
int triinv_build(const float* l, int64_t ld, const float* dinv, int64_t np, TriInv& ti, hipStream_t s);
int triinv_build_range(const float* l, int64_t ld, const float* dinv, int64_t np, TriInv& ti, int64_t j0, int64_t j1, hipStream_t s);
int trsm_rlt_blocks_f32(float* b, int64_t ldb, int64_t m, const float* l, int64_t ld, const TriInv& ti, int64_t np,
                        float* tmp, hipStream_t s);
int trsm_rut_blocks_f32(float* b, int64_t ldb, int64_t m, const float* lt, int64_t ld, const TriInv& ti, int64_t np,
                        float* tmp, hipStream_t s);
int trsm_rlt_blocks_h3(float* b, int64_t ldb, int64_t m, const float* l, int64_t ld, const TriInv& ti, int64_t np,
                       float* tmp, const SplitWork& sw, hipStream_t s);
int trsm_rut_blocks_h3(float* b, int64_t ldb, int64_t m, const float* lt, int64_t ld, const TriInv& ti, int64_t np,
                       float* tmp, const SplitWork& sw, hipStream_t s);
int trsv_forward_f32(const float* l, int64_t ld, const TriInv& ti, int64_t np, float* b, float* x, hipStream_t s);
int trsv_backward_f32(const float* l, int64_t ld, const TriInv& ti, int64_t np, float* b, float* x, hipStream_t s);
struct TrsmTickets;
int tk_create(TrsmTickets** out, int64_t np_cap, int64_t m_cap);
void tk_destroy(TrsmTickets* tk);
int tk_prepare_inverses(TrsmTickets* tk, const TriInv& ti, int64_t np, const float* l, int64_t ld, hipStream_t s);
bool tk_inverses_ready(const TrsmTickets* tk);
void tk_invalidate_inverses(TrsmTickets* tk);
bool tk_usable(const TrsmTickets* tk, int64_t m, int64_t np);
int tk_solve(TrsmTickets* tk, float* b, int64_t ldb, int64_t m, int64_t np, const SplitWork& sw, bool backward, hipStream_t s, int reserve_cus = 0);
int tk_poll_error(TrsmTickets* tk, bool wait);
int launch_symv_f64(const double* a, int64_t lda, int64_t n, const double* x, double* y, double diag_add, double* part,
                    int64_t np, hipStream_t s);
int launch_gemv_f64(const double* a, int64_t lda, int64_t rows, int64_t cols, const double* x, int64_t incx,
                    double* y, int64_t incy, double diag_add, hipStream_t s);
struct PcgWork {
    double* r; double* z; double* p; double* q; double* xcol; double* bcol;
    float* f32a; float* f32b; float* f32c;
    double* dot_part = nullptr;
    unsigned* dot_ctr = nullptr;
    double* symv_part = nullptr;
    int64_t symv_np = 0;
    double* scal;
    double* host_scal;
    hipGraphExec_t iter_graph = nullptr;
    const void* graph_key[4] = {nullptr, nullptr, nullptr, nullptr};
    int64_t graph_dims[4] = {0, 0, 0, 0};
    double graph_reg = 0.0;
};
int pcg_finish(const double* k64, int64_t ld, int64_t n, double reg, const float* l32, int64_t ld32, const TriInv& ti,
               int64_t np, double* xcol, PcgWork& w, int iters_done, int max_iters, double tol, int* iters_out,
               double* relres_out, hipStream_t s);
int pcg_solve(const double* k64, int64_t ld, int64_t n, double reg, const float* l32, int64_t ld32,
              const TriInv& ti, int64_t np, const double* bcol, double* xcol, PcgWork& w, int max_iters,
              double tol, int* iters_out, double* relres_out, hipStream_t s);
int precond_apply(const float* l32, int64_t ld32, const TriInv& ti, int64_t n, int64_t np, const double* r, double* z, PcgWork& w,
                  hipStream_t s);

int launch_convert_f64_f32(const double* src, int64_t lds, float* dst, int64_t ldd, int64_t rows, int64_t cols,
                           int64_t rows_p, int64_t cols_p, hipStream_t s);
int launch_factor_input(const double* k64, int64_t ld64, float* a32, int64_t ld32, int64_t n, int64_t np,
                        double reg, double pad_diag, hipStream_t s, int64_t row_begin = 0, int64_t row_end = -1);
int launch_mirror_rows_f64(double* k, int64_t ld, int64_t n0, int64_t n1, hipStream_t s);
int launch_row_sqsum_f32(const float* v, int64_t ld, int64_t rows, int64_t cols, const double* base,
                         double* out, hipStream_t s);
int launch_cov_finish(const double* ktt, int64_t ldk, const float* vvt, int64_t ldv, int64_t m, double* cov,
                      hipStream_t s);
int launch_zero_pad_f64(double* a, int64_t ld, int64_t n, int64_t np, hipStream_t s);
int launch_f32_to_f64_mat(const float* src, int64_t lds, double* dst, int64_t ldd, int64_t rows, int64_t cols,
                          bool accumulate, hipStream_t s);
int launch_axpby_mat(double* r, double a, const double* k, double b, int64_t ld, int64_t rows, int64_t cols,
                     hipStream_t s);
int launch_rowdot_f64(const double* z, const double* k, double kscale, const double* r, int64_t ld, int64_t rows,
                      int64_t cols, const double* base, double sign, double* out, hipStream_t s, double* zstat = nullptr);
int launch_copy_mat_f64(const double* src, int64_t lds, double* dst, int64_t m, hipStream_t s);
int launch_skinny_nt_f64(double* c, int64_t ldc, const double* cin, int64_t ldcin, const double* a, int64_t lda,
                         const double* b, int64_t ldb, int64_t m, int64_t n, int64_t k, double alpha, double beta, hipStream_t s);
int launch_identity_rows(double* e, int64_t ld, int64_t cols, int64_t r0, int64_t rows, int64_t rows_p, hipStream_t s);
int launch_symmetrize_f64(double* a, int64_t ld, int64_t n, hipStream_t s);
struct RowsPcg {
    int64_t cap = 0;
    double* p = nullptr;
    double* q = nullptr;
    double* rho = nullptr;
    double* coef = nullptr;
    double* tol = nullptr;
    double* delta = nullptr;
    double* var = nullptr;
    double* zstat = nullptr;
    int32_t* state = nullptr;
    int32_t* live = nullptr;
    int32_t* host = nullptr;
};
int launch_rows_prepare(const double* delta, const double* ktt, const double* var, const double* q, int mode, double thr,
                        int64_t rows, double* tol, int32_t* flagged, hipStream_t s);
int launch_rows_energy(const double* r, const float* s32, int64_t ld, int64_t rows, int64_t cols, double* out, hipStream_t s);
int launch_rows_prepare_ntk(const double* e1, const double* dv, double* zk_tol, const double* var, int64_t vstride,
                            int64_t rows, double tau, hipStream_t s);
int launch_rows_dvar(const float* d32, const double* w, const double* k, double kscale, int64_t ld, int64_t rows,
                     int64_t cols, double* out, hipStream_t s);
int launch_sweep_estimate(const double* e0, const double* e1, const double* zk, const double* dv, const double* var,
                          int64_t vstride, int64_t rows, double* out, hipStream_t s);
int launch_rows_rho(const double* r, const float* s32, int64_t ld, int64_t rows, int64_t cols, bool first, RowsPcg& w,
                    hipStream_t s);
int launch_rows_update_p(double* p, const float* s32, int64_t ld, int64_t rows, int64_t cols, RowsPcg& w, hipStream_t s);
int launch_rows_alpha(const double* p, const double* q, int64_t ld, int64_t rows, int64_t cols, RowsPcg& w, hipStream_t s);
int launch_rows_axpy2(double* z, double* r, const double* p, const double* q, int64_t ld, int64_t rows, int64_t cols,
                      RowsPcg& w, hipStream_t s);

int launch_pool_select(const double* mean, int64_t m, int ny, const double* var, int64_t count, int biased, uint64_t seed,
                       double* key_ws, int64_t* indices, hipStream_t s);
int launch_pool_greedy(const double* cov, int64_t m, int64_t ld, double noise, int64_t count, int64_t* indices, double* gains,
                       double* factor, int64_t ldf, double* ws, hipStream_t s);
int64_t syrk_ws_doubles(int64_t rows, int64_t mp);
int syrk_check(const double* c, int64_t ldc, const double* r, const double* a, int64_t lda, const double* y, int64_t rows, int64_t mp,
               int ny, double beta);
int launch_syrk_tn_f64(double* c, int64_t ldc, double* r, const double* a, int64_t lda, const double* y, int64_t rows, int64_t mp,
                       int ny, double beta, double* ws, int64_t ws_doubles, hipStream_t s);
int launch_transpose_f32(const float* src, int64_t lds, float* dst, int64_t ldd, int64_t n, hipStream_t s);
int launch_strided_copy_f64(const double* src, int64_t incs, double* dst, int64_t incd, int64_t n, hipStream_t s);

}
```

nngp-src_amd/csrc/gemm_i8s.hip:

```cpp
#include <atomic>

#include "common.h"

namespace nngp {

namespace {

typedef int i32x4 __attribute__((ext_vector_type(4)));
typedef double f64x2 __attribute__((ext_vector_type(2)));
typedef __attribute__((address_space(3))) void lds_void;
typedef const __attribute__((address_space(1))) void glb_void;

constexpr int IT = 256;
constexpr int IROW = 128;
constexpr int ISTAGE = 2 * IT * IROW;
constexpr int kI8ChunkBlocks = 128;
constexpr int kI8ChunkBlocks3 = 320;

__device__ __forceinline__ double i8s_scale_of(double mx) {
    if (!(mx < 1.0e300)) return __builtin_nan("");
    if (!(mx >= 0x1p-960)) return 1.0;
    int e = 0;
    const double f = frexp(mx, &e);
    return ldexp(1.0, f <= 0.984375 ? e + 1 : e + 2);
}

__device__ __forceinline__ double i8s_mag(double v) {
    const double a = fabs(v);
    return a < 1.0e300 ? a : __builtin_inf();
}

__global__ __launch_bounds__(1024) void k_i8s_diag_bound_scale(const double* __restrict__ src, int64_t ld, int64_t n,
                                                               double* __restrict__ scale) {
    __shared__ double red[16];
    double mx = 0.0;
    for (int64_t i = threadIdx.x; i < n; i += 1024) mx = fmax(mx, i8s_mag(src[i * ld + i]));
#pragma unroll
    for (int off = 32; off > 0; off >>= 1) mx = fmax(mx, __shfl_xor(mx, off));
    if ((threadIdx.x & 63) == 0) red[threadIdx.x >> 6] = mx;
    __syncthreads();
    mx = 0.0;
#pragma unroll
    for (int i = 0; i < 16; ++i) mx = fmax(mx, red[i]);
    for (int64_t i = threadIdx.x; i < n; i += 1024) {
        scale[i] = i8s_scale_of(sqrt(fabs(src[i * ld + i]) * mx) * (1.0 + 1e-9));
    }
}

template <int NS>
__global__ __launch_bounds__(256) void k_i8s_slice_rows(const double* src, int64_t ld, int64_t cols, int64_t kp,
                                                        const double* __restrict__ scale_in, double* __restrict__ scale_out,
                                                        int8_t* __restrict__ planes, int64_t ldp, int64_t pstride, double* wb) {
    __shared__ __attribute__((aligned(16))) unsigned char dig[NS][4096];
    __shared__ double red[4];
    const int t = threadIdx.x;
    const int64_t r = blockIdx.x;
    const double* p = src + r * ld;
    double scale;
    if (scale_in != nullptr) {
        scale = scale_in[r];
    } else {
        double mx = 0.0;
        for (int64_t c = 2 * (int64_t)t; c < cols; c += 512) {
            if (c + 1 < cols) {
                const f64x2 v = *reinterpret_cast<const f64x2*>(p + c);
                mx = fmax(mx, fmax(i8s_mag(v[0]), i8s_mag(v[1])));
            } else {
                mx = fmax(mx, i8s_mag(p[c]));
            }
        }
#pragma unroll
        for (int off = 32; off > 0; off >>= 1) mx = fmax(mx, __shfl_xor(mx, off));
        if ((t & 63) == 0) red[t >> 6] = mx;
        __syncthreads();
        scale = i8s_scale_of(fmax(fmax(red[0], red[1]), fmax(red[2], red[3])));
        if (t == 0) scale_out[r] = scale;
    }
    const double inv = ldexp(1.0, 8 * NS) / scale;
    const double back = scale * ldexp(1.0, -8 * NS);
    double* q = wb != nullptr ? wb + r * ld : nullptr;
    for (int64_t seg0 = 0; seg0 < kp; seg0 += 4096) {
#pragma unroll
        for (int i = 0; i < 8; ++i) {
            const int lc = 2 * t + 512 * i;
            const int64_t c = seg0 + lc;
            f64x2 v = {0.0, 0.0};
            if (c + 1 < cols) {
                v = *reinterpret_cast<const f64x2*>(p + c);
            } else if (c < cols) {
                v[0] = p[c];
            }
            long long x0 = __double2ll_rn(v[0] * inv), x1 = __double2ll_rn(v[1] * inv);
            if (q != nullptr) {
                if (c + 1 < cols) {
                    *reinterpret_cast<f64x2*>(q + c) = f64x2{(double)x0 * back, (double)x1 * back};
                } else if (c < cols) {
                    q[c] = (double)x0 * back;
                }
            }
#pragma unroll
            for (int s = NS - 1; s >= 1; --s) {
                const long long d0 = ((x0 + 128) & 255) - 128, d1 = ((x1 + 128) & 255) - 128;
                x0 = (x0 - d0) >> 8;
                x1 = (x1 - d1) >> 8;
                *reinterpret_cast<unsigned short*>(&dig[s][lc]) = (unsigned short)((d0 & 255) | ((d1 & 255) << 8));
            }
            *reinterpret_cast<unsigned short*>(&dig[0][lc]) = (unsigned short)((x0 & 255) | ((x1 & 255) << 8));
        }
        __syncthreads();
        const int64_t c16 = seg0 + 16 * t;
        if (c16 < kp) {
#pragma unroll
            for (int s = 0; s < NS; ++s)
                *reinterpret_cast<i32x4*>(planes + s * pstride + r * ldp + c16) = *reinterpret_cast<const i32x4*>(&dig[s][16 * t]);
        }
        __syncthreads();
    }
}

constexpr int kSymT = 128, kSymLd = kSymT + 1;
template <int NS>
__device__ __forceinline__ void i8s_digits16(const double* v, int stride, double inv, i32x4* dig) {
    unsigned char b[NS][16];
#pragma unroll
    for (int c = 0; c < 16; ++c) {
        long long x = __double2ll_rn(v[c * stride] * inv);
#pragma unroll
        for (int s = NS - 1; s >= 1; --s) {
            const long long d = ((x + 128) & 255) - 128;
            x = (x - d) >> 8;
            b[s][c] = (unsigned char)(d & 255);
        }
        b[0][c] = (unsigned char)(x & 255);
    }
#pragma unroll
    for (int s = 0; s < NS; ++s) {
        i32x4 w;
#pragma unroll
        for (int q = 0; q < 4; ++q)
            w[q] = (int)((unsigned)b[s][4 * q] | ((unsigned)b[s][4 * q + 1] << 8) | ((unsigned)b[s][4 * q + 2] << 16) | ((unsigned)b[s][4 * q + 3] << 24));
        dig[s] = w;
    }
}

template <int NS>
__global__ __launch_bounds__(256) void k_i8s_slice_sym(const double* __restrict__ src, int64_t ld, const double* __restrict__ scale,
                                                       int8_t* __restrict__ planes, int64_t ldp, int64_t pstride) {
    __shared__ double tile[kSymT * kSymLd];
    const int t = threadIdx.x;
    const long long b = blockIdx.x;
    long long I = (long long)((sqrt(8.0 * (double)b + 1.0) - 1.0) * 0.5);
    while ((I + 1) * (I + 2) / 2 <= b) ++I;
    while (I * (I + 1) / 2 > b) --I;
    const long long J = b - I * (I + 1) / 2;
    const double* p = src + (I * kSymT) * ld + J * kSymT;
#pragma unroll 8
    for (int i = 0; i < 32; ++i) {
        const int row = 4 * i + (t >> 6), col = 2 * (t & 63);
        const f64x2 v = *reinterpret_cast<const f64x2*>(p + (int64_t)row * ld + col);
        tile[row * kSymLd + col] = v[0];
        tile[row * kSymLd + col + 1] = v[1];
    }
    __syncthreads();
    const double top = ldexp(1.0, 8 * NS);
#pragma unroll 1
    for (int it = 0; it < 4; ++it) {
        const int item = it * 256 + t, row = item >> 3, g = item & 7;
        const int64_t r = I * kSymT + row;
        i32x4 dig[NS];
        i8s_digits16<NS>(tile + row * kSymLd + 16 * g, 1, top / scale[r], dig);
#pragma unroll
        for (int s = 0; s < NS; ++s) *reinterpret_cast<i32x4*>(planes + s * pstride + r * ldp + J * kSymT + 16 * g) = dig[s];
    }
    if (I == J) return;
#pragma unroll 1
    for (int it = 0; it < 4; ++it) {
        const int item = it * 256 + t, col = item >> 3, g = item & 7;
        const int64_t r = J * kSymT + col;
        i32x4 dig[NS];
        i8s_digits16<NS>(tile + (16 * g) * kSymLd + col, kSymLd, top / scale[r], dig);
#pragma unroll
        for (int s = 0; s < NS; ++s) *reinterpret_cast<i32x4*>(planes + s * pstride + r * ldp + I * kSymT + 16 * g) = dig[s];
    }
}

struct I8Tile {
    const char* pa;
    const char* pb;
    int* pc;
    int row0, col0;
    int p0, p1;
    int kb0, nk;
};

__global__ __launch_bounds__(512) void k_gemm_nt_i8s(int* P, int64_t ldc, int64_t slab, const char* A, int64_t lda, int64_t sa,
                                                     const char* B, int64_t ldb, int64_t sb, int m, int n, int nkb, int kcb, int nchunk,
                                                     int ndiag, unsigned long long pa_lo, unsigned long long pa_hi,
                                                     unsigned long long pb_lo, unsigned long long pb_hi, unsigned long long dstart_lo,
                                                     unsigned dstart_hi, int order_br, int order_bc, int* counters, int slots_per_xcd,
                                                     int total_wgs) {
    __shared__ __attribute__((aligned(1024))) char smem[2 * ISTAGE];
    int& s_slot = *reinterpret_cast<int*>(smem);
    const int tid = threadIdx.x;
    const int lane = tid & 63, wave = tid >> 6;
    const int xcd = blockIdx.x & 7;
    const int group = __builtin_amdgcn_readfirstlane(wave >> 2);
    const int w4 = __builtin_amdgcn_readfirstlane(wave & 3);
    const int l3 = lane >> 3;
    const int r16 = lane & 15, q4 = lane >> 4;
    const unsigned swz = (((lane & 7) ^ ((4 * (w4 & 1) + (l3 >> 1)) & 7)) << 4);
    const unsigned lane_off_a = (unsigned)l3 * (unsigned)lda + swz;
    const unsigned lane_off_b = (unsigned)l3 * (unsigned)ldb + swz;
    const unsigned frag_hi = (unsigned)r16 * IROW + (((unsigned)q4 ^ ((unsigned)r16 >> 1)) << 4);
    const unsigned frag_lo = frag_hi ^ 64u;

    auto nib = [&](unsigned long long lo, unsigned long long hi, int p) -> int {
        return (int)(((p < 16 ? lo : hi) >> (4 * (p & 15))) & 15ull);
    };
    auto dstart = [&](int dd) -> int {
        return dd < 8 ? (int)((dstart_lo >> (8 * dd)) & 255ull) : (int)(dstart_hi & 255u);
    };
    const int tiles_m = (m + IT - 1) / IT, tiles_n = (n + IT - 1) / IT;
    const int bm = (tiles_m + order_br - 1) / order_br, bn = (tiles_n + order_bc - 1) / order_bc;
    const int nb = bm * bn;

    int vx = xcd, tries = 0;
    auto decode = [&](int slot, I8Tile& tl) -> bool {
        const int per = order_br * order_bc;
        const int G = (slot / per) * 8 + vx;
        const int i = slot % per;
        if (G >= ndiag * nchunk * nb) return false;
        const int dd = G / (nchunk * nb);
        const int rem = G - dd * (nchunk * nb);
        const int ch = rem / nb, blk = rem - ch * nb;
        const int gr = blk / bn, gc = blk - gr * bn;
        const int bi = gr * order_br + (i % order_br);
        const int bj = gc * order_bc + (i / order_br);
        if (bi >= tiles_m || bj >= tiles_n) return false;
        tl.pa = A + (int64_t)bi * IT * lda;
        tl.pb = B + (int64_t)bj * IT * ldb;
        tl.pc = P + ((int64_t)ch * ndiag + dd) * slab + (int64_t)bi * IT * ldc + (int64_t)bj * IT;
        tl.row0 = bi * IT;
        tl.col0 = bj * IT;
        tl.p0 = dstart(dd);
        tl.p1 = dstart(dd + 1);
        tl.kb0 = ch * kcb;
        tl.nk = (nkb - tl.kb0 < kcb) ? nkb - tl.kb0 : kcb;
        return true;
    };
    int cur_p = 0, cur_kb = 0;
    auto cursor_reset = [&](const I8Tile& tl) { cur_p = tl.p0; cur_kb = tl.nk - 1; };
    auto cursor_take = [&](const I8Tile& tl, int64_t& offa, int64_t& offb) {
        const int64_t kbyte = (int64_t)(tl.kb0 + cur_kb) * 128;
        offa = (int64_t)nib(pa_lo, pa_hi, cur_p) * sa + kbyte;
        offb = (int64_t)nib(pb_lo, pb_hi, cur_p) * sb + kbyte;
        if (--cur_kb < 0) {
            ++cur_p;
            cur_kb = tl.nk - 1;
        }
    };
    auto glds_b = [&](int t, int64_t koff, const char* tile_pb) {
        const char* pb = tile_pb + koff;
        char* dst = smem + (t & 1) * ISTAGE + IT * IROW;
#pragma unroll
        for (int e = 0; e < 4; ++e) {
            const int piece = group * 16 + e * 4 + w4;
            __builtin_amdgcn_global_load_lds((glb_void*)(pb + (int64_t)piece * 8 * ldb + lane_off_b), (lds_void*)(dst + piece * 1024), 16, 0, 0);
        }
    };
    auto glds_a = [&](int t, int64_t koff, const char* tile_pa) {
        const char* pa = tile_pa + koff;
        char* dst = smem + (t & 1) * ISTAGE;
#pragma unroll
        for (int e = 0; e < 4; ++e) {
            const int piece = group * 16 + e * 4 + w4;
            __builtin_amdgcn_global_load_lds((glb_void*)(pa + (int64_t)piece * 8 * lda + lane_off_a), (lds_void*)(dst + piece * 1024), 16, 0, 0);
        }
    };
    auto fetch_tile = [&](I8Tile& tl) -> bool {
        for (;;) {
            if (tid == 0) s_slot = atomicAdd(&counters[vx], 1);
            __syncthreads();
            const int slot = __builtin_amdgcn_readfirstlane(s_slot);
            __syncthreads();
            if (slot >= slots_per_xcd) {
                if (++tries >= 8) return false;
                vx = (vx + 1) & 7;
                continue;
            }
            if (decode(slot, tl)) return true;
        }
    };

    I8Tile tl = {};
    bool have = fetch_tile(tl);
    bool stored = false;
    if (have) {
        cursor_reset(tl);
        int64_t oa, ob;
        cursor_take(tl, oa, ob);
        glds_b(0, ob, tl.pb);
        glds_a(0, oa, tl.pa);
    }
    while (have) {
        i32x4 acc[8][4];
#pragma unroll
        for (int i = 0; i < 8; ++i)
#pragma unroll
            for (int j = 0; j < 4; ++j) acc[i][j] = i32x4{0, 0, 0, 0};
        const int nstage = (tl.p1 - tl.p0) * tl.nk;

        if (stored)
            asm volatile("s_waitcnt vmcnt(32)" ::: "memory");
        else
            asm volatile("s_waitcnt vmcnt(0)" ::: "memory");
        __builtin_amdgcn_s_barrier();
        if (group == 1) __builtin_amdgcn_s_barrier();
        int next_slot = 0;
        for (int t = 0; t < nstage; ++t) {
            const char* sa_ = smem + (t & 1) * ISTAGE;
            const char* sb_ = sa_ + IT * IROW;
            const bool more = t + 1 < nstage;
            int64_t na = 0, nbo = 0;
            if (more) cursor_take(tl, na, nbo);
            i32x4 bh[4], bl[4], ah[4], al[4];
#pragma unroll
            for (int j = 0; j < 4; ++j) {
                const int rb = (w4 * 64 + j * 16) * IROW;
                bh[j] = *reinterpret_cast<const i32x4*>(sb_ + rb + frag_hi);
                bl[j] = *reinterpret_cast<const i32x4*>(sb_ + rb + frag_lo);
            }
#pragma unroll
            for (int i = 0; i < 4; ++i) {
                const int rb = (group * 128 + i * 16) * IROW;
                ah[i] = *reinterpret_cast<const i32x4*>(sa_ + rb + frag_hi);
// ... 21 lines not shown
                for (int j = 0; j < 4; ++j) acc[i][j] = __builtin_amdgcn_mfma_i32_16x16x64_i8(bh[j], ah[i], acc[i][j], 0, 0, 0);
            __builtin_amdgcn_s_setprio(0);
            __builtin_amdgcn_sched_barrier(0);
            __builtin_amdgcn_s_barrier();
            __builtin_amdgcn_sched_barrier(0);
#pragma unroll
            for (int i = 0; i < 4; ++i) {
                const int rb = (group * 128 + 64 + i * 16) * IROW;
                ah[i] = *reinterpret_cast<const i32x4*>(sa_ + rb + frag_hi);
                al[i] = *reinterpret_cast<const i32x4*>(sa_ + rb + frag_lo);
            }
            if (more) {
                glds_a(t + 1, na, tl.pa);
                asm volatile("s_waitcnt vmcnt(4)" ::: "memory");
            }
            asm volatile("s_waitcnt lgkmcnt(0)" ::: "memory");
            __builtin_amdgcn_sched_barrier(0);
            __builtin_amdgcn_s_barrier();
            __builtin_amdgcn_sched_barrier(0);
            __builtin_amdgcn_s_setprio(1);
#pragma unroll
            for (int i = 0; i < 4; ++i)
#pragma unroll
                for (int j = 0; j < 4; ++j) acc[4 + i][j] = __builtin_amdgcn_mfma_i32_16x16x64_i8(bl[j], al[i], acc[4 + i][j], 0, 0, 0);
#pragma unroll
            for (int i = 0; i < 4; ++i)
#pragma unroll
                for (int j = 0; j < 4; ++j) acc[4 + i][j] = __builtin_amdgcn_mfma_i32_16x16x64_i8(bh[j], ah[i], acc[4 + i][j], 0, 0, 0);
            __builtin_amdgcn_s_setprio(0);
            __builtin_amdgcn_sched_barrier(0);
            if (more) asm volatile("s_waitcnt vmcnt(2)" ::: "memory");
            __builtin_amdgcn_s_barrier();
            __builtin_amdgcn_sched_barrier(0);
        }
        if (group == 0) __builtin_amdgcn_s_barrier();

        const I8Tile ct = tl;
        if (tid == 0) s_slot = next_slot;
        __syncthreads();
        const int slot = __builtin_amdgcn_readfirstlane(s_slot);
        __syncthreads();
        have = slot < slots_per_xcd && decode(slot, tl);
        if (!have) {
            if (slot >= slots_per_xcd) {
                ++tries;
                vx = (vx + 1) & 7;
            }
            have = tries < 8 && fetch_tile(tl);
        }
        if (have) {
            cursor_reset(tl);
            int64_t oa, ob;
            cursor_take(tl, oa, ob);
            glds_b(0, ob, tl.pb);
            glds_a(0, oa, tl.pa);
        }
        const int row_base = ct.row0 + group * 128, col_base = ct.col0 + w4 * 64;
        stored = row_base < m && col_base < n;
        if (stored) {
            const unsigned voff = ((unsigned)r16 * (unsigned)ldc + 4u * (unsigned)q4) * 4u;
            char* cw = reinterpret_cast<char*>(ct.pc + (int64_t)(group * 128) * ldc + w4 * 64);
            const int64_t band = (int64_t)16 * ldc * 4;
#pragma unroll
            for (int i = 0; i < 8; ++i)
#pragma unroll
                for (int j = 0; j < 4; ++j) *reinterpret_cast<i32x4*>(cw + i * band + voff + 64 * j) = acc[i][j];
        }
    }
    if (tid == 0 && atomicAdd(&counters[8], 1) == total_wgs - 1)
        for (int i = 0; i < 9; ++i) __hip_atomic_store(&counters[i], 0, __ATOMIC_RELAXED, __HIP_MEMORY_SCOPE_AGENT);
}

template <bool FUSE>
__global__ __launch_bounds__(256) void k_i8s_combine(double* __restrict__ out, int64_t ldo, const double* __restrict__ cin, int64_t ldcin,
                                                     double beta, double alpha, const double* __restrict__ g, int64_t ldg, double gamma,
                                                     const int* __restrict__ P, int64_t ldc, int64_t slab, int nchunk, int ndiag,
                                                     const double* __restrict__ sa, const double* __restrict__ sb, int64_t rows,
                                                     int64_t cols, float* __restrict__ out32, int64_t ld32, double* __restrict__ part) {
    const int64_t c4 = ((int64_t)blockIdx.x * 256 + threadIdx.x) * 4;
    const int64_t r = blockIdx.y;
    const bool live = c4 < cols && r < rows;
    if (!FUSE && !live) return;
    double s1 = 0.0, s2 = 0.0, s3 = 0.0, mx = 0.0;
    if (live) {
        double t[4] = {0.0, 0.0, 0.0, 0.0};
        for (int dd = 0; dd < ndiag; ++dd) {
            long long sum[4] = {0, 0, 0, 0};
            for (int ch = 0; ch < nchunk; ++ch) {
                const i32x4 v = *reinterpret_cast<const i32x4*>(P + ((int64_t)ch * ndiag + dd) * slab + r * ldc + c4);
#pragma unroll
                for (int e = 0; e < 4; ++e) sum[e] += v[e];
            }
#pragma unroll
            for (int e = 0; e < 4; ++e) t[e] = t[e] * 0.00390625 + (double)sum[e];
        }
        const double w = alpha * sa[r] * (1.0 / 65536.0);
#pragma unroll
        for (int e = 0; e < 4; ++e) {
            if (c4 + e >= cols) break;
            double v = w * sb[c4 + e] * t[e];
            const double cv = (beta != 0.0 || FUSE) ? cin[r * ldcin + c4 + e] : 0.0;
            const double gv = (gamma != 0.0 || FUSE) ? g[r * ldg + c4 + e] : 0.0;
            if (beta != 0.0) v += beta * cv;
            if (gamma != 0.0) v += gamma * gv;
            out[r * ldo + c4 + e] = v;
            if (FUSE) {
                out32[r * ld32 + c4 + e] = (float)v;
                s1 = fma(gv, cv + v, s1);
                s2 = fma(gv, v, s2);
                s3 = fma(gv, gv, s3);
                mx = fmax(mx, fabs(gv));
            }
        }
    }
    if (FUSE) {
        __shared__ double red[16];
#pragma unroll
        for (int off = 32; off > 0; off >>= 1) {
            s1 += __shfl_down(s1, off);
            s2 += __shfl_down(s2, off);
            s3 += __shfl_down(s3, off);
            mx = fmax(mx, __shfl_down(mx, off));
        }
        if ((threadIdx.x & 63) == 0) {
            const int w = threadIdx.x >> 6;
            red[w] = s1; red[4 + w] = s2; red[8 + w] = s3; red[12 + w] = mx;
        }
        __syncthreads();
        if (threadIdx.x < 4 && r < rows) {
            const int q = threadIdx.x;
            const double v = q < 3 ? (red[4 * q] + red[4 * q + 1]) + (red[4 * q + 2] + red[4 * q + 3])
                                   : fmax(fmax(red[12], red[13]), fmax(red[14], red[15]));
            part[(r * gridDim.x + blockIdx.x) * 4 + q] = v;
        }
    }
}

__global__ void k_i8s_rowstat_finish(const double* __restrict__ part, int nblk, int64_t rows, const double* __restrict__ base,
                                     double* __restrict__ var, double* __restrict__ delta, double* __restrict__ zstat) {
    const int64_t r = (int64_t)blockIdx.x * blockDim.x + threadIdx.x;
    if (r >= rows) return;
    double s1 = 0.0, s2 = 0.0, s3 = 0.0, mx = 0.0;
    for (int b = 0; b < nblk; ++b) {
        const double* p = part + (r * nblk + b) * 4;
        s1 += p[0]; s2 += p[1]; s3 += p[2]; mx = fmax(mx, p[3]);
    }
    var[r] = base[r] - s1;
    delta[r] = s2;
    zstat[2 * r] = s3;
    zstat[2 * r + 1] = mx;
}


__global__ __launch_bounds__(1024) void k_i8s_scale_sqsum(const double* __restrict__ scale, int64_t n, double* __restrict__ out) {
    __shared__ double red[16];
    double s = 0.0;
    for (int64_t i = threadIdx.x; i < n; i += 1024) s += scale[i] * scale[i];
#pragma unroll
    for (int off = 32; off > 0; off >>= 1) s += __shfl_down(s, off);
    if ((threadIdx.x & 63) == 0) red[threadIdx.x >> 6] = s;
    __syncthreads();
    if (threadIdx.x == 0) {
        double t = 0.0;
        for (int w = 0; w < 16; ++w) t += red[w];
        out[0] = t;
    }
}

__global__ __launch_bounds__(256) void k_i8s_floor_ratio(const double* __restrict__ z, int64_t ld, int64_t cols, const double* __restrict__ var,
                                                         double coef, const double* __restrict__ sk2, unsigned long long* out) {
    __shared__ double red[8];
    const int64_t r = blockIdx.x;
    const double* p = z + r * ld;
    double mx = 0.0, s2 = 0.0;
    for (int64_t c = 2 * (int64_t)threadIdx.x; c + 1 < cols; c += 512) {
        const f64x2 v = *reinterpret_cast<const f64x2*>(p + c);
        mx = fmax(mx, fmax(fabs(v[0]), fabs(v[1])));
        s2 += v[0] * v[0] + v[1] * v[1];
    }
#pragma unroll
    for (int off = 32; off > 0; off >>= 1) {
        mx = fmax(mx, __shfl_xor(mx, off));
        s2 += __shfl_xor(s2, off);
    }
    if ((threadIdx.x & 63) == 0) { red[threadIdx.x >> 6] = mx; red[4 + (threadIdx.x >> 6)] = s2; }
    __syncthreads();
    if (threadIdx.x == 0) {
        mx = fmax(fmax(red[0], red[1]), fmax(red[2], red[3]));
        s2 = (red[4] + red[5]) + (red[6] + red[7]);
        const double est = sqrt(s2) * coef * i8s_scale_of(mx) * sqrt(sk2[0]);
        const double v = var[r];
        double ratio = v > 0.0 ? est / v : (est > 0.0 ? 1.0e300 : 0.0);
        if (ratio != ratio) ratio = 1.0e300;
        atomicMax(out, (unsigned long long)__double_as_longlong(ratio));
    }
}

__global__ __launch_bounds__(256) void k_i8s_floor_ratio_rows(const double* __restrict__ zstat, int64_t rows, const double* __restrict__ var,
                                                              double coef, const double* __restrict__ sk2, unsigned long long* out) {
    const int64_t r = (int64_t)blockIdx.x * 256 + threadIdx.x;
    if (r >= rows) return;
    const double est = sqrt(zstat[2 * r]) * coef * i8s_scale_of(zstat[2 * r + 1]) * sqrt(sk2[0]);
    const double v = var[r];
    double ratio = v > 0.0 ? est / v : (est > 0.0 ? 1.0e300 : 0.0);
    if (ratio != ratio) ratio = 1.0e300;
    atomicMax(out, (unsigned long long)__double_as_longlong(ratio));
}

}

int launch_i8s_diag_bound_scale(const double* src, int64_t ld, int64_t n, double* scale, hipStream_t s) {
    if (n <= 0) return 0;
    hipLaunchKernelGGL(k_i8s_diag_bound_scale, dim3(1), dim3(1024), 0, s, src, ld, n, scale);
    NNGP_HIP_CHECK(hipGetLastError());
    return 0;
}

int launch_i8s_slice_rows(const double* src, int64_t ld, int64_t rows, int64_t cols, int ns, const double* scale_in, double* scale_out,
                          int8_t* planes, int64_t ldp, int64_t pstride, hipStream_t s, double* writeback) {
    if (rows <= 0) return 0;
    const int64_t kp = round_up(cols, 128);
    NNGP_REQUIRE(ns >= 2 && ns <= 7 && ld % 2 == 0 && ((uintptr_t)src & 15) == 0 && ((uintptr_t)planes & 15) == 0 && ldp >= kp &&
                     ldp % 16 == 0 && pstride % 16 == 0 && rows < 2147483647LL && (scale_in != nullptr || scale_out != nullptr),
                 "i8s_slice_rows: 2..7 planes, 16-byte aligned operands");
    const dim3 g((unsigned)rows);
    switch (ns) {
        case 2: hipLaunchKernelGGL(k_i8s_slice_rows<2>, g, dim3(256), 0, s, src, ld, cols, kp, scale_in, scale_out, planes, ldp, pstride, writeback); break;
        case 3: hipLaunchKernelGGL(k_i8s_slice_rows<3>, g, dim3(256), 0, s, src, ld, cols, kp, scale_in, scale_out, planes, ldp, pstride, writeback); break;
        case 4: hipLaunchKernelGGL(k_i8s_slice_rows<4>, g, dim3(256), 0, s, src, ld, cols, kp, scale_in, scale_out, planes, ldp, pstride, writeback); break;
        case 5: hipLaunchKernelGGL(k_i8s_slice_rows<5>, g, dim3(256), 0, s, src, ld, cols, kp, scale_in, scale_out, planes, ldp, pstride, writeback); break;
        case 6: hipLaunchKernelGGL(k_i8s_slice_rows<6>, g, dim3(256), 0, s, src, ld, cols, kp, scale_in, scale_out, planes, ldp, pstride, writeback); break;
        default: hipLaunchKernelGGL(k_i8s_slice_rows<7>, g, dim3(256), 0, s, src, ld, cols, kp, scale_in, scale_out, planes, ldp, pstride, writeback); break;
    }
    NNGP_HIP_CHECK(hipGetLastError());
    return 0;
}

int launch_i8s_slice_sym(const double* src, int64_t ld, int64_t n, int ns, const double* scale, int8_t* planes, int64_t ldp,
                         int64_t pstride, hipStream_t s) {
    if (n <= 0) return 0;
    NNGP_REQUIRE((ns == 5 || ns == 7) && n % kSymT == 0 && ld % 2 == 0 && ((uintptr_t)src & 15) == 0 && ((uintptr_t)planes & 15) == 0 &&
                     ldp >= n && ldp % 16 == 0 && pstride % 16 == 0 && scale != nullptr,
                 "i8s_slice_sym: 5 or 7 planes of a matrix padded to 128");
    const int64_t tn = n / kSymT, tiles = tn * (tn + 1) / 2;
    NNGP_REQUIRE(tiles < 2147483647LL, "i8s_slice_sym: too many tiles");
    if (ns == 5) hipLaunchKernelGGL(k_i8s_slice_sym<5>, dim3((unsigned)tiles), dim3(256), 0, s, src, ld, scale, planes, ldp, pstride);
    else hipLaunchKernelGGL(k_i8s_slice_sym<7>, dim3((unsigned)tiles), dim3(256), 0, s, src, ld, scale, planes, ldp, pstride);
    NNGP_HIP_CHECK(hipGetLastError());
    return 0;
}

int launch_i8s_scale_sqsum(const double* scale, int64_t n, double* out, hipStream_t s) {
    hipLaunchKernelGGL(k_i8s_scale_sqsum, dim3(1), dim3(1024), 0, s, scale, n, out);
    NNGP_HIP_CHECK(hipGetLastError());
    return 0;
}

int launch_i8s_floor_ratio(const double* z, int64_t ld, int64_t rows, int64_t cols, const double* var, const I8Plan& pl, int nsa, int nsb,
                           const double* sk2, unsigned long long* out, hipStream_t s) {
    if (rows <= 0) return 0;
    NNGP_REQUIRE(cols % 2 == 0 && ld % 2 == 0 && ((uintptr_t)z & 15) == 0, "i8s_floor_ratio: cols and ld must be even, z 16-byte aligned (cols=%lld)",
                 (long long)cols);
    int cut = -1;
    for (int p = 0; p < pl.npairs; ++p) cut = pl.pa[p] + pl.pb[p] > cut ? pl.pa[p] + pl.pb[p] : cut;
    int dropped = 2;
    for (int ia = 0; ia < nsa; ++ia) dropped += (cut + 1 - ia >= 0 && cut + 1 - ia < nsb) ? 1 : 0;
    const double coef = 5404.7 * sqrt((double)dropped) * pow(256.0, -(double)(cut + 3));
    hipLaunchKernelGGL(k_i8s_floor_ratio, dim3((unsigned)rows), dim3(256), 0, s, z, ld, cols, var, coef, sk2, out);
    NNGP_HIP_CHECK(hipGetLastError());
    return 0;
}

static double i8s_floor_coef(const I8Plan& pl, int nsa, int nsb) {
    int cut = -1;
    for (int p = 0; p < pl.npairs; ++p) cut = pl.pa[p] + pl.pb[p] > cut ? pl.pa[p] + pl.pb[p] : cut;
    int dropped = 2;
    for (int ia = 0; ia < nsa; ++ia) dropped += (cut + 1 - ia >= 0 && cut + 1 - ia < nsb) ? 1 : 0;
    return 5404.7 * sqrt((double)dropped) * pow(256.0, -(double)(cut + 3));
}

int launch_i8s_floor_ratio_rows(const double* zstat, int64_t rows, const double* var, const I8Plan& pl, int nsa, int nsb, const double* sk2,
                                unsigned long long* out, hipStream_t s) {
    if (rows <= 0) return 0;
    hipLaunchKernelGGL(k_i8s_floor_ratio_rows, dim3((unsigned)((rows + 255) / 256)), dim3(256), 0, s, zstat, rows, var,
                       i8s_floor_coef(pl, nsa, nsb), sk2, out);
    NNGP_HIP_CHECK(hipGetLastError());
    return 0;
}

int i8s_plan(int nsa, int nsb, int cut, I8Plan* pl) {
    NNGP_REQUIRE(nsa >= 1 && nsa <= 7 && nsb >= 1 && nsb <= 7 && cut >= 0, "i8s: 1..7 planes per operand");
    if (cut > nsa + nsb - 2) cut = nsa + nsb - 2;
    *pl = I8Plan{};
    int np = 0;
    for (int e = cut; e >= 0; --e) {
        NNGP_REQUIRE(pl->ndiag < 8, "i8s: too many diagonals");
        pl->dstart[pl->ndiag++] = np;
        int cnt = 0;
        for (int ia = 0; ia < nsa; ++ia) {
            const int ib = e - ia;
            if (ib < 0 || ib >= nsb) continue;
            NNGP_REQUIRE(np < 32, "i8s: too many slice pairs");
            pl->pa[np] = ia;
            pl->pb[np] = ib;
            ++np;
            ++cnt;
        }
        NNGP_REQUIRE(cnt >= 1 && cnt <= 7, "i8s: a diagonal needs 1..7 pairs (int32 accumulation over 16384 k)");
    }
    pl->dstart[pl->ndiag] = np;
    pl->npairs = np;
    return 0;
}

static int chunk_blocks(const I8Plan* pl) {
    if (pl == nullptr || NNGP_KNOB(5) == 60) return kI8ChunkBlocks;
    int most = 0;
    for (int d = 0; d < pl->ndiag; ++d) most = pl->dstart[d + 1] - pl->dstart[d] > most ? pl->dstart[d + 1] - pl->dstart[d] : most;
    return most <= 3 ? kI8ChunkBlocks3 : kI8ChunkBlocks;
}

int64_t i8s_chunks(int64_t k, const I8Plan* pl) {
    const int64_t nkb = (k + 127) / 128, cb = chunk_blocks(pl);
    return (nkb + cb - 1) / cb;
}

int launch_gemm_nt_i8s(int32_t* partial, int64_t ldc, int64_t slab, const int8_t* a, int64_t lda, int64_t sa, const int8_t* b,
                       int64_t ldb, int64_t sb, const I8Plan& pl, int64_t m, int64_t n, int64_t k, int* counters, int reserve_cus,
                       hipStream_t s) {
    if (m <= 0 || n <= 0 || k <= 0) return 0;
    NNGP_REQUIRE(m % 128 == 0 && n % 128 == 0 && m < (1 << 30) && n < (1 << 30) && ldc >= n && ldc % 4 == 0 && slab >= m * ldc &&
                     ((uintptr_t)partial & 15) == 0,
                 "gemm_nt_i8s: m, n must be multiples of 128 (m=%lld n=%lld)", (long long)m, (long long)n);
    const int64_t nkb = (k + 127) / 128;
    NNGP_REQUIRE(lda >= nkb * 128 && ldb >= nkb * 128 && lda % 128 == 0 && ldb % 128 == 0 && sa % 16 == 0 && sb % 16 == 0 &&
                     ((uintptr_t)a & 15) == 0 && ((uintptr_t)b & 15) == 0 && counters != nullptr && 8 * lda < (1LL << 31) &&
                     8 * ldb < (1LL << 31) && 16 * ldc * 4 < (1LL << 31),
                 "gemm_nt_i8s: operand planes must be 16-byte aligned with row strides that are multiples of 128");
    const int64_t nchunk = i8s_chunks(k, &pl);
    const int64_t kcb = (nkb + nchunk - 1) / nchunk;
    unsigned long long pa_lo = 0, pa_hi = 0, pb_lo = 0, pb_hi = 0, ds_lo = 0;
    unsigned ds_hi = 0;
    for (int p = 0; p < pl.npairs; ++p) {
        (p < 16 ? pa_lo : pa_hi) |= (unsigned long long)pl.pa[p] << (4 * (p & 15));
        (p < 16 ? pb_lo : pb_hi) |= (unsigned long long)pl.pb[p] << (4 * (p & 15));
    }
    for (int d = 0; d <= pl.ndiag; ++d) {
        if (d < 8) ds_lo |= (unsigned long long)pl.dstart[d] << (8 * d);
        else ds_hi = (unsigned)pl.dstart[d];
    }
    const int br = 4, bc = 8;
    const int64_t tm = (m + IT - 1) / IT, tn = (n + IT - 1) / IT;
    const int64_t nb = ((tm + br - 1) / br) * ((tn + bc - 1) / bc);
    const int64_t nblk = nb * nchunk * pl.ndiag;
    const int64_t slots_per_xcd = ((nblk + 7) / 8) * br * bc;
    NNGP_REQUIRE(slots_per_xcd < 2147483647LL / 8 && nblk < 2147483647LL, "gemm_nt_i8s: too many tiles");
    static std::atomic<int> ncu_cached{0};
    int ncu = ncu_cached.load(std::memory_order_relaxed);
    if (ncu == 0) {
        int dev = 0, count = 0;
        ncu = (hipGetDevice(&dev) == hipSuccess &&
               hipDeviceGetAttribute(&count, hipDeviceAttributeMultiprocessorCount, dev) == hipSuccess && count > 0) ? count : 256;
        ncu_cached.store(ncu, std::memory_order_relaxed);
    }
    int64_t grid = ncu - reserve_cus;
    if (grid > slots_per_xcd * 8) grid = slots_per_xcd * 8;
    grid = (grid / 8) * 8;
    if (grid < 8) grid = 8;
    hipLaunchKernelGGL(k_gemm_nt_i8s, dim3((unsigned)grid), dim3(512), 0, s, partial, ldc, slab, reinterpret_cast<const char*>(a), lda, sa,
                       reinterpret_cast<const char*>(b), ldb, sb, (int)m, (int)n, (int)nkb, (int)kcb, (int)nchunk, pl.ndiag, pa_lo, pa_hi,
                       pb_lo, pb_hi, ds_lo, ds_hi, br, bc, counters, (int)slots_per_xcd, (int)grid);
    NNGP_HIP_CHECK(hipGetLastError());
    return 0;
}

int launch_i8s_combine(double* out, int64_t ldo, const double* cin, int64_t ldcin, double beta, double alpha, const double* g,
                       int64_t ldg, double gamma, const int32_t* partial, int64_t ldc, int64_t slab, int nchunk, int ndiag,
                       const double* sa, const double* sb, int64_t rows, int64_t cols, hipStream_t s, const I8Fuse* fuse) {
    if (rows <= 0 || cols <= 0) return 0;
    NNGP_REQUIRE((beta == 0.0 || cin != nullptr) && (gamma == 0.0 || g != nullptr) && ldc % 4 == 0, "i8s_combine: NULL input");
    NNGP_REQUIRE(fuse == nullptr || (cin != nullptr && g != nullptr && fuse->out32 != nullptr && fuse->part != nullptr && fuse->ld32 >= cols),
                 "i8s_combine: the fused row statistics need both addends");
    const unsigned nbx = (unsigned)i8s_col_blocks(cols);
    for (int64_t r0 = 0; r0 < rows; r0 += 65535) {
        const int64_t nr = rows - r0 < 65535 ? rows - r0 : 65535;
        if (fuse != nullptr)
            hipLaunchKernelGGL(k_i8s_combine<true>, dim3(nbx, (unsigned)nr), dim3(256), 0, s, out + r0 * ldo, ldo, cin + r0 * ldcin, ldcin,
                               beta, alpha, g + r0 * ldg, ldg, gamma, partial + r0 * ldc, ldc, slab, nchunk, ndiag, sa + r0, sb, nr, cols,
                               fuse->out32 + r0 * fuse->ld32, fuse->ld32, fuse->part + r0 * nbx * 4);
        else
            hipLaunchKernelGGL(k_i8s_combine<false>, dim3(nbx, (unsigned)nr), dim3(256), 0, s, out + r0 * ldo, ldo,
                               cin ? cin + r0 * ldcin : nullptr, ldcin, beta, alpha, g ? g + r0 * ldg : nullptr, ldg, gamma,
                               partial + r0 * ldc, ldc, slab, nchunk, ndiag, sa + r0, sb, nr, cols, (float*)nullptr, (int64_t)0,
                               (double*)nullptr);
    }
    NNGP_HIP_CHECK(hipGetLastError());
    return 0;
}

int64_t i8s_col_blocks(int64_t cols) { return (cols + 1023) / 1024; }

int launch_i8s_rowstat_finish(const double* part, int64_t cols, int64_t rows, const double* base, double* var, double* delta,
                              double* zstat, hipStream_t s) {
    if (rows <= 0) return 0;
    hipLaunchKernelGGL(k_i8s_rowstat_finish, dim3((unsigned)((rows + 255) / 256)), dim3(256), 0, s, part, (int)i8s_col_blocks(cols), rows,
                       base, var, delta, zstat);
// ... 6 lines not shown
```

nngp-src_amd/csrc/model.h:

```cpp
#pragma once
#include <stdarg.h>
#include <stdlib.h>
#include <cmath>
#include <new>
#include <mutex>
#include "common.h"
#include "i8_trust.h"
#include "alpha_plan.h"
#include <atomic>

namespace nngp {
extern std::atomic<long long> g_alloc_count;

template <typename T>
inline int dev_alloc(T** p, int64_t count) {
    *p = nullptr;
    if (count <= 0) return 0;
    NNGP_HIP_CHECK(hipMalloc(reinterpret_cast<void**>(p), sizeof(T) * (size_t)count));
    g_alloc_count.fetch_add(1, std::memory_order_relaxed);
    return 0;
}

template <typename T>
inline void dev_free(T*& p) {
// ... 104 lines not shown
using namespace nngp;

struct nngp_model {
    int64_t n_cap = 0, np_cap = 0, m_cap = 0;
    int d = 0, ny = 1, get = NNGP_GET_NNGP;
    ArchDev arch{};
    GroupsDev groups{};
    double diag_reg = 1e-3;
    int absolute = 0;

    int64_t n = 0, np = 0;
    int64_t ld = 0;
    bool have_train = false, built = false, factored = false;
    bool a32_built = false;
    bool a32_complete = false, k64_partial = false;
    bool k64_symmetric = false;

    double* x = nullptr;
    double* y = nullptr;
    double* q = nullptr;
    double* kdiag = nullptr;
    double* k64 = nullptr;
    float* a32 = nullptr;
    float* dinv = nullptr;
    int32_t* clamped = nullptr;
    double* alpha = nullptr;
    PcgWork pcg{};
    TriInv tri{};
    LookAhead* la = nullptr;
    SplitWork split{};
    TrsmTickets* tk = nullptr;
    bool tk_failed = false;
    double diag_max = 0.0;

    double* xt_q = nullptr;
    double* tt_diag = nullptr;
    double* ktd64 = nullptr;
    float* b32 = nullptr;
    float* trsm_tmp = nullptr;
    int64_t ktd_cap = 0;
    int64_t full_cap = 0;
    double* ktt64 = nullptr;
    float* vvt32 = nullptr;

    int var_refine = 1;
    float* lt32 = nullptr;
    float* dinvt = nullptr;
    bool lt_ready = false;
    int64_t refine_cap = 0;
    double* z64 = nullptr;
    double* r64 = nullptr;
    double* covp64 = nullptr;
    double* ainv64 = nullptr;
    bool serving_ready = false;
    bool serving_weak = false;
    RowsPcg rows{};
    int64_t rows_pq_cap = 0;
    int cov_iters = 0;
    double sweep_est_var = -1.0;
    double sweep_est = -1.0;
    double* kaux64 = nullptr;
    bool aux_ready = false;
    double* ktd_aux = nullptr;
    int64_t ktd_aux_cap = 0;

    I8Residual i8;
    AlphaSolve alpha_solve;

    double reg = 0.0, trace_mean = 0.0;
    double reg_fac = 0.0;
    hipStream_t solve_stream = nullptr;
    bool tri_stale = false, tri_pending = false;
    EventPairTimer<32> trsm_t;
    double trsm_flops[decltype(trsm_t)::kMax] = {};
    hipEvent_t ev_tri = nullptr, ev_tri_fork = nullptr;
    hipEvent_t ev_lt = nullptr;

    ~nngp_model() {
        dev_free(x); dev_free(y); dev_free(q); dev_free(kdiag); dev_free(k64); dev_free(a32); dev_free(dinv);
        dev_free(clamped); dev_free(alpha);
        groups_destroy(&groups);
        dev_free(pcg.r); dev_free(pcg.z); dev_free(pcg.p); dev_free(pcg.q); dev_free(pcg.xcol); dev_free(pcg.bcol);
        dev_free(pcg.f32a); dev_free(pcg.f32b); dev_free(pcg.f32c); dev_free(pcg.scal); dev_free(pcg.symv_part); dev_free(pcg.dot_part); dev_free(pcg.dot_ctr);
        if (pcg.host_scal) (void)hipHostFree(pcg.host_scal);
        if (pcg.iter_graph) (void)hipGraphExecDestroy(pcg.iter_graph);
        dev_free(tri.tinv); dev_free(tri.xinv); dev_free(tri.partial); dev_free(tri.tmp);
        lookahead_destroy(la);
        if (solve_stream) (void)hipStreamDestroy(solve_stream);
        if (ev_lt) (void)hipEventDestroy(ev_lt);
        if (ev_tri) (void)hipEventDestroy(ev_tri);
        if (ev_tri_fork) (void)hipEventDestroy(ev_tri_fork);
        dev_free(split.planes); dev_free(split.counters); dev_free(split.planes_t); dev_free(split.planes_b); dev_free(split.row_inv);
        dev_free(split.ldiag); dev_free(split.dfrag); dev_free(split.dscale);
        tk_destroy(tk);
        dev_free(xt_q); dev_free(tt_diag); dev_free(ktd64); dev_free(b32); dev_free(trsm_tmp); dev_free(ktt64); dev_free(vvt32);
        dev_free(lt32); dev_free(dinvt); dev_free(z64); dev_free(r64); dev_free(covp64); dev_free(kaux64); dev_free(ktd_aux);
        dev_free(ainv64);
        dev_free(rows.p); dev_free(rows.q); dev_free(rows.rho); dev_free(rows.coef); dev_free(rows.tol); dev_free(rows.delta);
        dev_free(rows.var); dev_free(rows.state); dev_free(rows.live); dev_free(rows.zstat);
        if (rows.host) (void)hipHostFree(rows.host);
    }
};


namespace nngp {
struct ResidualNote {
    bool want_fused_rows = false;
    bool fused = false;
    bool used_int8 = false;
};


enum class CovCheck {
    None,
    NngpDiag,
    NngpFull,
    Ntk,
    NngpDiagLevel1,
};

struct PredictCall {
    hipStream_t s = nullptr;
    const double* xt = nullptr;
    const double* qt = nullptr;
    const double* ktd = nullptr;
    const double* ktd_nngp = nullptr;
    int64_t mt = 0, mp = 0;
    bool on_train = false, is_ntk = false, want_cov = false, full = false;
    bool compact_train = false;
    bool serving = false;
    double *mean = nullptr, *var_or_cov = nullptr;
    bool z_valid = false;
    bool used_i8 = false;
    bool i8_check_pending = false;
    CovCheck check = CovCheck::None;
};

int ensure_predict_capacity(nngp_model* m, int64_t mt, bool need_ktd);
int ensure_full_cov_capacity(nngp_model* m, int64_t mt);
void set_split_scale(nngp_model* m);
int ensure_refine_capacity(nngp_model* m, int64_t mp);
int ensure_lt_alloc(nngp_model* m);
int ensure_lt(nngp_model* m, hipStream_t s);
int ensure_lt_split(nngp_model* m, hipStream_t s);
int tri_join(nngp_model* m, hipStream_t s);
int tri_fork(nngp_model* m, hipStream_t s);
bool use_split_solves(const nngp_model* m, int64_t mp);
bool use_tickets(const nngp_model* m, int64_t mp);
enum class SolvePath { Recursion128, BlocksF32, BlocksH3, Tickets };
SolvePath solve_path(const nngp_model* m, int64_t mp);
inline bool needs_lt32(SolvePath p) { return p == SolvePath::Recursion128 || p == SolvePath::BlocksF32; }
bool cg_from_the_start(const nngp_model* m, int64_t mp);
hipStream_t early_cut_stream(const nngp_model* m, int64_t mp);
int tickets_reserve(const nngp_model* m);
int tickets_check(nngp_model* m, bool wait);
int apply_forward_f32(nngp_model* m, int64_t mp, hipStream_t s);
int apply_inverse_f32(nngp_model* m, int64_t mp, hipStream_t s);
int refined_solve_rows(nngp_model* m, const double* rhs, int64_t mp, int sweeps, bool final_residual, hipStream_t s,
                       bool measure = false, ResidualNote* note = nullptr);
int rows_pcg_continue(nngp_model* m, int64_t mp, int max_iters, hipStream_t s);
int build_cross(nngp_model* m, const double* xt, const double* qt, int64_t mt, int64_t mp, bool nngp, double* out,
                hipStream_t s);
bool use_i8s(const nngp_model* m, int64_t mp);
int i8s_reserve(nngp_model* m, int64_t mp, int32_t cov_mode);
void i8s_kernel_changed(nngp_model* m);
int cut_planes_early(nngp_model* m, PredictCall& c);
int residual_rows(nngp_model* m, double* out, const double* rhs, double* z, int64_t mp, hipStream_t s, bool first_residual,
                  ResidualNote* note = nullptr);
int kaux_product_rows(nngp_model* m, double* out, double* z, int64_t mp, hipStream_t s);
void take_in_guard_word(nngp_model* m);
int record_i8_guard_estimate(nngp_model* m, PredictCall& c);
int first_guard_verdict(nngp_model* m, PredictCall& c, bool* redo);
int i8s_timer_enable(nngp_model* m, int32_t enable);
int i8s_timer_read(nngp_model* m, int64_t* launches, double* ms_total, double* flops_total, double* int8_ops_total);
int i8s_residual_floor(nngp_model* m, double* ratio, int32_t* distrusted);
int run_pending_solve(nngp_model* m, hipStream_t user, bool order_user, bool allow_partial = false);
void open_gate_epoch(nngp_model* m);
int record_cg_gate(nngp_model* m, hipStream_t s);
int record_predict_end(nngp_model* m, hipStream_t s);
}
```

nngp-src_amd/csrc/residual_i8.hip:

```cpp
#include "model.h"

namespace nngp {

constexpr int64_t kI8RowBlock = 2048;

bool use_i8s(const nngp_model* m, int64_t mp) {
    if (m->i8.suspended || m->i8.unavailable || m->i8.trust.distrusted) return false;
    if (NNGP_KNOB(5) == 54) return true;
    return i8_coarse_pays(m->np, mp) && NNGP_KNOB(5) != 50;
}

enum { I8_COARSE = 0, I8_FINE = 1 };
constexpr int kI8FinePlanes = 7, kI8FineCut = 6;
constexpr int kI8CoarseZPlanes = 3;
constexpr int kI8FineZPlanes = 5;

static bool use_i8s_fine(const nngp_model* m, int64_t mp) { return use_i8s(m, mp) && i8_fine_pays(m->np, mp) && NNGP_KNOB(5) != 57; }
static int i8s_planes_policy(const nngp_model* m) {
    return (m->get == NNGP_GET_NTK || m->var_refine >= 2 || m->i8.want_fine) && NNGP_KNOB(5) != 57 ? kI8FinePlanes : 5;
}


static int ensure_i8s(nngp_model* m, int64_t mp, I8Planes& pk, int planes) {
    I8Work& w = m->i8.work;
    if (NNGP_KNOB(5) == 51) { w.ns_k = w.ns_z = 4; w.cut = 3; }
    else if (NNGP_KNOB(5) == 52) { w.ns_k = w.ns_z = 6; w.cut = 5; }
    else { w.ns_k = 5; w.ns_z = NNGP_KNOB(5) == 58 ? 5 : kI8CoarseZPlanes; w.cut = 4; }
    if (planes < w.ns_k) planes = w.ns_k;
    w.k_rows = round_up(m->np_cap, 256);
    auto give_up = [&]() -> int {
        dev_free(w.k.planes); dev_free(w.k.scale); dev_free(w.aux.planes); dev_free(w.aux.scale);
        dev_free(w.zplanes); dev_free(w.zscale); dev_free(w.partial); dev_free(w.rowpart);
        w.rowpart_rows = 0;
        w.k.ready = w.aux.ready = false;
        w.k.alloc_planes = w.aux.alloc_planes = 0;
        w.z_rows = 0;
        w.z_planes = 0;
        m->i8.unavailable = true;
        return 1;
    };
    if (pk.alloc_planes < planes) {
        NNGP_HIP_CHECK(hipDeviceSynchronize());
        dev_free(pk.planes); dev_free(pk.scale);
        pk.alloc_planes = 0;
        if (!soft_alloc(&pk.planes, planes * w.k_rows * m->np_cap) || !soft_alloc(&pk.scale, m->np_cap + 1)) return give_up();
        NNGP_HIP_CHECK(hipMemset(pk.planes, 0, (size_t)(planes * w.k_rows * m->np_cap)));
        pk.alloc_planes = planes;
        pk.ready = false;
    }
    if (mp > w.rowpart_rows) {
        NNGP_HIP_CHECK(hipDeviceSynchronize());
        dev_free(w.rowpart);
        w.rowpart_rows = 0;
        NNGP_TRY(dev_alloc(&w.rowpart, mp * i8s_col_blocks(m->np_cap) * 4));
        w.rowpart_rows = mp;
    }
    if (w.counters == nullptr) {
        NNGP_TRY(dev_alloc(&w.counters, 16));
        NNGP_HIP_CHECK(hipMemset(w.counters, 0, 16 * sizeof(int)));
    }
    const int64_t rows = mp < kI8RowBlock ? mp : kI8RowBlock;
    if (rows > w.z_rows || planes > w.z_planes) {
        NNGP_HIP_CHECK(hipDeviceSynchronize());
        dev_free(w.zplanes); dev_free(w.zscale); dev_free(w.partial);
        const int64_t nr = rows > w.z_rows ? rows : w.z_rows;
        const int np_ = planes > w.z_planes ? planes : w.z_planes;
        w.z_rows = 0;
        w.z_planes = 0;
        if (!soft_alloc(&w.zplanes, np_ * (nr + 256) * m->np_cap) || !soft_alloc(&w.zscale, nr) ||
            !soft_alloc(&w.partial, i8s_chunks(m->np_cap) * np_ * nr * m->np_cap))
            return give_up();
        NNGP_HIP_CHECK(hipMemset(w.zplanes, 0, (size_t)(np_ * (nr + 256) * m->np_cap)));
        w.z_rows = nr;
        w.z_planes = np_;
    }
    return 0;
}

static int i8s_cut_planes(nngp_model* m, I8Planes& pk, const double* kmat, int64_t kld, hipStream_t s) {
    I8Work& w = m->i8.work;
    NNGP_TRY(launch_i8s_diag_bound_scale(kmat, kld, m->np, pk.scale, s));
    const bool sym = (kmat == m->kaux64 || m->k64_symmetric) && (pk.alloc_planes == 5 || pk.alloc_planes == 7) && NNGP_KNOB(5) != 62;
    if (sym)
        NNGP_TRY(launch_i8s_slice_sym(kmat, kld, m->np, pk.alloc_planes, pk.scale, pk.planes, m->np_cap, w.k_rows * m->np_cap, s));
    else
        NNGP_TRY(launch_i8s_slice_rows(kmat, kld, m->np, m->np, pk.alloc_planes, pk.scale, nullptr, pk.planes, m->np_cap, w.k_rows * m->np_cap, s));
    NNGP_TRY(launch_i8s_scale_sqsum(pk.scale, m->np, pk.scale + m->np_cap, s));
    pk.ns_done = pk.alloc_planes;
    pk.ready = true;
    return 0;
}

static int i8s_product_rows(nngp_model* m, I8Planes& pk, const double* kmat, int64_t kld, double* out, const double* cin, double beta,
                            double alpha, double* z, double gamma, int64_t mp, hipStream_t s, int grade, ResidualNote* note = nullptr) {
    const int64_t np = m->np;
    I8Work& w = m->i8.work;
    const int fine_z = NNGP_KNOB(5) == 64 ? kI8FinePlanes : kI8FineZPlanes;
    const bool round_z = grade == I8_COARSE ? w.ns_z < w.ns_k : fine_z < kI8FinePlanes;
    const bool fuse_rows = grade == I8_COARSE && note != nullptr && note->want_fused_rows && cin != nullptr && w.rowpart_rows >= mp && NNGP_KNOB(5) != 59;
    const int ns_z = grade == I8_FINE ? fine_z : w.ns_z, ns_k = grade == I8_FINE ? kI8FinePlanes : w.ns_k;
    const int cut = grade == I8_FINE ? kI8FineCut : w.cut;
    NNGP_REQUIRE(pk.alloc_planes >= ns_k && w.z_planes >= ns_z, "i8s_product_rows: workspace for %d planes missing", ns_k);
    if (!pk.ready || pk.ns_done < ns_k) {
        NNGP_TRY(i8s_cut_planes(m, pk, kmat, kld, s));
    } else if (&pk == &w.k && m->i8.k_pending) {
        NNGP_HIP_CHECK(hipStreamWaitEvent(s, m->i8.ev_i8, 0));
    }
    if (&pk == &w.k) m->i8.k_pending = false;
    I8Plan pl;
    NNGP_TRY(i8s_plan(ns_z, ns_k, cut, &pl));
    const int64_t nchunk = i8s_chunks(np, &pl);
    for (int64_t r0 = 0; r0 < mp; r0 += kI8RowBlock) {
        const int64_t mb = mp - r0 < kI8RowBlock ? mp - r0 : kI8RowBlock;
        const int64_t slab = mb * np;
        NNGP_TRY(launch_i8s_slice_rows(z + r0 * np, np, mb, np, ns_z, nullptr, w.zscale, w.zplanes, m->np_cap, (w.z_rows + 256) * m->np_cap, s,
                                       round_z ? z + r0 * np : nullptr));
        if (r0 == 0 && grade == I8_COARSE && !m->alpha_solve.gate_recorded && NNGP_KNOB(2) != 8 && NNGP_KNOB(2) != 9 && !cg_from_the_start(m, mp)) {
            NNGP_TRY(record_cg_gate(m, s));
        }
        int slot = -1;
        NNGP_TRY(m->i8.timer.begin(s, &slot));
        NNGP_TRY(launch_gemm_nt_i8s(w.partial, np, slab, w.zplanes, m->np_cap, (w.z_rows + 256) * m->np_cap, pk.planes, m->np_cap,
                                    w.k_rows * m->np_cap, pl, mb, np, np, w.counters, 0, s));
        NNGP_TRY(m->i8.timer.end(slot));
        if (slot >= 0) {
            w.t_flops[slot] = 2.0 * (double)mb * (double)np * (double)np;
            w.t_ops[slot] = w.t_flops[slot] * pl.npairs;
        }
        I8Fuse fuse;
        fuse.out32 = m->b32 + r0 * np;
        fuse.ld32 = np;
        fuse.part = w.rowpart + r0 * i8s_col_blocks(np) * 4;
        NNGP_TRY(launch_i8s_combine(out + r0 * np, np, cin ? cin + r0 * np : nullptr, np, beta, alpha, z + r0 * np, np, gamma, w.partial, np,
                                    slab, (int)nchunk, pl.ndiag, w.zscale, pk.scale, mb, np, s, fuse_rows ? &fuse : nullptr));
    }
    if (fuse_rows) note->fused = true;
    if (grade == I8_COARSE && !m->alpha_solve.gate_recorded && NNGP_KNOB(2) == 9) NNGP_TRY(record_cg_gate(m, s));
    return 0;
}

int residual_rows(nngp_model* m, double* out, const double* rhs, double* z, int64_t mp, hipStream_t s, bool first_residual,
                  ResidualNote* note) {
    const int64_t np = m->np;
    const bool coarse = first_residual;
    if (!coarse && use_i8s_fine(m, mp)) m->i8.want_fine = true;
    if (coarse ? use_i8s(m, mp) : use_i8s_fine(m, mp)) {
        const int rc = ensure_i8s(m, mp, m->i8.work.k, coarse ? i8s_planes_policy(m) : kI8FinePlanes);
        if (rc == 0) {
            if (coarse && note != nullptr) note->used_int8 = true;
            return i8s_product_rows(m, m->i8.work.k, m->k64, m->ld, out, rhs, 1.0, -1.0, z, -m->reg, mp, s, coarse ? I8_COARSE : I8_FINE,
                                    note);
        }
        if (rc != 1) return rc;
    }
    NNGP_TRY(launch_gemm_nt_f64(out, np, rhs, np, z, np, m->k64, m->ld, mp, np, np, -1.0, 1.0, s));
    return launch_axpby_mat(out, 1.0, z, -m->reg, np, mp, np, s);
}

int kaux_product_rows(nngp_model* m, double* out, double* z, int64_t mp, hipStream_t s) {
    const int64_t np = m->np;
    const int rc_w = use_i8s_fine(m, mp) ? ensure_i8s(m, mp, m->i8.work.aux, kI8FinePlanes) : 1;
    if (rc_w == 0) return i8s_product_rows(m, m->i8.work.aux, m->kaux64, np, out, nullptr, 0.0, 1.0, z, 0.0, mp, s, I8_FINE);
    if (rc_w != 1) return rc_w;
    return launch_gemm_nt_f64(out, np, nullptr, 0, z, np, m->kaux64, np, mp, np, np, 1.0, 0.0, s);
}

int cut_planes_early(nngp_model* m, PredictCall& c) {
    if (!(c.want_cov && m->var_refine >= 1 && use_i8s(m, c.mp) && !c.serving && NNGP_KNOB(5) != 53)) return 0;
    I8Residual& r = m->i8;
    if (c.full && use_i8s_fine(m, c.mp)) r.want_fine = true;
    const int rc_i8 = ensure_i8s(m, c.mp, r.work.k, i8s_planes_policy(m));
    if (rc_i8 != 0 && rc_i8 != 1) return rc_i8;
    if (rc_i8 != 0 || r.work.k.ready) return 0;
    if (r.ev_i8 == nullptr) NNGP_HIP_CHECK(hipEventCreateWithFlags(&r.ev_i8, hipEventDisableTiming));
    NNGP_HIP_CHECK(hipEventRecord(r.ev_i8, c.s));
    const hipStream_t cs = early_cut_stream(m, c.mp);
    NNGP_HIP_CHECK(hipStreamWaitEvent(cs, r.ev_i8, 0));
    NNGP_TRY(i8s_cut_planes(m, r.work.k, m->k64, m->ld, cs));
    NNGP_HIP_CHECK(hipEventRecord(r.ev_i8, cs));
    r.k_pending = true;
    return 0;
}

static int ensure_guard_word(nngp_model* m) {
    if (m->i8.guard != nullptr) return 0;
    NNGP_TRY(dev_alloc(&m->i8.guard, 1));
    NNGP_HIP_CHECK(hipHostMalloc(reinterpret_cast<void**>(&m->i8.guard_host), sizeof(unsigned long long), hipHostMallocDefault));
    return 0;
}

int i8s_reserve(nngp_model* m, int64_t mp, int32_t cov_mode) {
    if (!(i8_coarse_pays(m->np_cap, mp) && !m->i8.unavailable && (m->var_refine >= 1 || m->get == NNGP_GET_NTK))) return 0;
    if (cov_mode == NNGP_COV_FULL && i8_fine_pays(m->np_cap, mp)) m->i8.want_fine = true;
    const int rc = ensure_i8s(m, mp, m->i8.work.k, i8s_planes_policy(m));
    if (rc != 0 && rc != 1) return rc;
    if (rc == 0) NNGP_TRY(ensure_guard_word(m));
    return 0;
}

void i8s_kernel_changed(nngp_model* m) {
    m->i8.work.k.ready = false;
    m->i8.trust.new_kernel();
}

static double guard_threshold() { return NNGP_KNOB(5) == 56 ? 0.0 : kI8FloorThr; }

int record_i8_guard_estimate(nngp_model* m, PredictCall& c) {
    I8Residual& r = m->i8;
    const I8Work& w = r.work;
    I8Plan pl;
    NNGP_TRY(i8s_plan(w.ns_z, w.ns_k, w.cut, &pl));
    NNGP_TRY(ensure_guard_word(m));
    if (r.ev_guard == nullptr) NNGP_HIP_CHECK(hipEventCreateWithFlags(&r.ev_guard, hipEventDisableTiming));
    NNGP_HIP_CHECK(hipMemsetAsync(r.guard, 0, sizeof(unsigned long long), c.s));
    NNGP_TRY(launch_i8s_floor_ratio_rows(m->rows.zstat, c.mt, c.var_or_cov, pl, w.ns_z, w.ns_k, w.k.scale + m->np_cap, r.guard, c.s));
    if (!r.trust.checked) {
        c.i8_check_pending = true;
    } else {
        NNGP_HIP_CHECK(hipMemcpyAsync(r.guard_host, r.guard, sizeof(unsigned long long), hipMemcpyDeviceToHost, c.s));
        NNGP_HIP_CHECK(hipEventRecord(r.ev_guard, c.s));
        r.trust.pending = true;
    }
    return 0;
}

void take_in_guard_word(nngp_model* m) {
    if (!(m->i8.trust.pending && hipEventQuery(m->i8.ev_guard) == hipSuccess)) return;
    double ratio = 0.0;
    memcpy(&ratio, m->i8.guard_host, sizeof(double));
    m->i8.trust.fold(ratio, guard_threshold());
}

int first_guard_verdict(nngp_model* m, PredictCall& c, bool* redo) {
    *redo = false;
// ... 49 lines not shown
```

nngp-src_amd/csrc/trsm_tickets.hip:

```cpp
#include <stddef.h>
#include <stdlib.h>

#include <algorithm>
#include <vector>

#include "common.h"
#include "trsm_order.h"

namespace nngp {

static_assert(sizeof(TkItem) == sizeof(int4) && offsetof(TkItem, word) == offsetof(int4, x) && offsetof(TkItem, r) == offsetof(int4, y) &&
                  offsetof(TkItem, c) == offsetof(int4, z) && offsetof(TkItem, J) == offsetof(int4, w),
              "TkItem must lie in memory like int4");

namespace {

typedef _Float16 h8 __attribute__((ext_vector_type(8)));
typedef float f32x4v __attribute__((ext_vector_type(4)));
typedef __attribute__((address_space(3))) void lds_void;
typedef const __attribute__((address_space(1))) void glb_void;

constexpr int TT = 128;
constexpr int TROW = 128;
constexpr int TSTAGE = 2 * TT * TROW;
// ... 636 lines not shown
    *reinterpret_cast<h8*>(dst + 64) = lo;
}

__global__ __launch_bounds__(256) void k_transpose_1024(const float* __restrict__ src, int64_t lds, int64_t sstride, float* __restrict__ dst, int rows_valid_last, int nblk) {
    __shared__ float tile[32][33];
    const int b = blockIdx.z;
    const float* sp = src + (int64_t)b * sstride;
    float* dp = dst + (int64_t)b * kBs * kBs;
    const int n0 = blockIdx.y * 32, c0 = blockIdx.x * 32;
    const int tx = threadIdx.x & 31, ty = threadIdx.x >> 5;
    const int nvalid = (b == nblk - 1) ? rows_valid_last : kBs;
#pragma unroll
    for (int i = 0; i < 4; ++i) {
        const int n = n0 + ty + 8 * i;
        tile[ty + 8 * i][tx] = n < nvalid ? sp[(int64_t)n * lds + c0 + tx] : 0.0f;
    }
    __syncthreads();
#pragma unroll
    for (int i = 0; i < 4; ++i) dp[(int64_t)(c0 + ty + 8 * i) * kBs + n0 + tx] = tile[tx][ty + 8 * i];
}

struct TkDevSwitches {
    TkOrderOptions order;
    int merge = -1;
};
const TkDevSwitches& tk_dev_switches() {
#ifdef NNGP_TIMING_KNOBS
    static const TkDevSwitches sw = [] {
        TkDevSwitches v;
        if (const char* e = getenv("NNGP_TK_MAXPAN")) v.order.max_pan = std::max(1, std::min(4, atoi(e)));
        v.order.no_big = getenv("NNGP_TK_NOBIG") != nullptr;
        if (const char* e = getenv("NNGP_TK_MERGE")) v.merge = atoi(e) != 0 ? 1 : 0;
        return v;
    }();
#else
    static const TkDevSwitches sw;
#endif
    return sw;
}

struct TkTableKey {
    int mt = 0, nb = 0, tail_ct = 0;
    int merged[2] = {-1, -1};
    bool operator==(const TkTableKey& o) const { return mt == o.mt && nb == o.nb && tail_ct == o.tail_ct && merged[0] == o.merged[0] && merged[1] == o.merged[1]; }
};

}

struct TrsmTickets {
    int64_t m_cap = 0, np_cap = 0, nb_cap = 0;
    char* planes_x = nullptr;
    char* planes_d = nullptr;
    float* rinv_x = nullptr;
    float* rinv_d = nullptr;
    char* xinv_s = nullptr;
    char* tinv_s = nullptr;
    float* inv_iscale = nullptr;
    float* wtmp = nullptr;
    float* ltb = nullptr;
    char* wplanes[2] = {nullptr, nullptr};
    float* w_iscale = nullptr;
    unsigned* wmax = nullptr;
    bool w_ready[2] = {false, false};
    unsigned* amax = nullptr;
    int* sync = nullptr;
    int64_t sync_ints = 0;
    int4* items[2] = {nullptr, nullptr};
    int64_t items_cap = 0;
    int n_items[2] = {0, 0};
    int nq = 1;
    int q_off[2][kMaxQ + 1] = {};
    int nq_dir[2] = {1, 1};
    TkTableKey key;
    std::vector<TkItem> host_items[2];
    int* host_err = nullptr;
    hipEvent_t ev_err = nullptr;
    bool err_pending = false;
    bool inv_ready = false;
    int workers = 256;
};

static int64_t tk_items_bound(int64_t mt, int64_t nb) { return mt * (8 * nb * (nb - 1) / 2 + 24 * nb) + 64; }

void tk_destroy(TrsmTickets* tk) {
    if (tk == nullptr) return;
    (void)hipFree(tk->planes_x); (void)hipFree(tk->planes_d); (void)hipFree(tk->rinv_x); (void)hipFree(tk->rinv_d);
    (void)hipFree(tk->xinv_s); (void)hipFree(tk->tinv_s); (void)hipFree(tk->inv_iscale); (void)hipFree(tk->amax);
    (void)hipFree(tk->sync); (void)hipFree(tk->items[0]); (void)hipFree(tk->items[1]);
    (void)hipFree(tk->wtmp); (void)hipFree(tk->ltb); (void)hipFree(tk->wplanes[0]); (void)hipFree(tk->wplanes[1]); (void)hipFree(tk->w_iscale);
    (void)hipFree(tk->wmax);
    if (tk->host_err) (void)hipHostFree(tk->host_err);
    if (tk->ev_err) (void)hipEventDestroy(tk->ev_err);
    delete tk;
}

int tk_create(TrsmTickets** out, int64_t np_cap, int64_t m_cap) {
    *out = nullptr;
    if (np_cap < 2 * kBs || m_cap < TT || m_cap > 64 * TT) return 1;
    TrsmTickets* tk = new (std::nothrow) TrsmTickets();
    NNGP_REQUIRE(tk != nullptr, "tk_create: out of host memory");
    tk->m_cap = round_up(m_cap, TT);
    tk->np_cap = np_cap;
    tk->nb_cap = (np_cap + kBs - 1) / kBs;
    const int64_t nb = tk->nb_cap, mt = tk->m_cap / TT;
    tk->sync_ints = SY_COUNTERS + 3 * mt * nb + mt * nb * 8;
    tk->items_cap = tk_items_bound(mt, nb);
    bool ok = true;
    auto A = [&](void** p, size_t bytes) { if (ok && hipMalloc(p, bytes) != hipSuccess) { (void)hipGetLastError(); ok = false; } note_alloc(); };
    A((void**)&tk->planes_x, (size_t)nb * tk->m_cap * kLdp);
    A((void**)&tk->planes_d, (size_t)nb * tk->m_cap * kLdp);
    A((void**)&tk->rinv_x, sizeof(float) * nb * tk->m_cap);
    A((void**)&tk->rinv_d, sizeof(float) * nb * tk->m_cap);
    A((void**)&tk->xinv_s, (size_t)nb * kBs * kLdp);
    A((void**)&tk->tinv_s, (size_t)nb * kBs * kLdp);
    A((void**)&tk->inv_iscale, sizeof(float) * 2 * nb);
    A((void**)&tk->amax, sizeof(unsigned) * 2 * nb);
    A((void**)&tk->sync, sizeof(int) * tk->sync_ints);
    A((void**)&tk->items[0], sizeof(int4) * tk->items_cap);
    A((void**)&tk->items[1], sizeof(int4) * tk->items_cap);
    A((void**)&tk->wtmp, sizeof(float) * nb * kBs * kBs);
    A((void**)&tk->ltb, sizeof(float) * nb * kBs * kBs);
    A((void**)&tk->wplanes[0], (size_t)nb * kBs * kLdp);
    A((void**)&tk->wplanes[1], (size_t)nb * kBs * kLdp);
    A((void**)&tk->w_iscale, sizeof(float) * 2 * nb);
    A((void**)&tk->wmax, sizeof(unsigned) * 2 * nb);
    if (ok && hipHostMalloc(reinterpret_cast<void**>(&tk->host_err), 2 * sizeof(int), hipHostMallocDefault) != hipSuccess) ok = false;
    if (ok && hipEventCreateWithFlags(&tk->ev_err, hipEventDisableTiming) != hipSuccess) ok = false;
    if (!ok) {
        (void)hipGetLastError();
        tk_destroy(tk);
        return 1;
    }
    tk->host_err[0] = tk->host_err[1] = 0;
    if (hipMemset(tk->sync, 0, sizeof(int) * tk->sync_ints) != hipSuccess) {
        (void)hipGetLastError();
        tk_destroy(tk);
        return 1;
    }
    int dev = 0, count = 0;
    if (hipGetDevice(&dev) == hipSuccess && hipDeviceGetAttribute(&count, hipDeviceAttributeMultiprocessorCount, dev) == hipSuccess && count > 0)
        tk->workers = count;
    tk->nq = 1;
    if (const char* e = getenv("NNGP_TK_QUEUES")) tk->nq = (atoi(e) == 8 && tk->workers == 256) ? kMaxQ : 1;
    *out = tk;
    return 0;
}

int tk_prepare_inverses(TrsmTickets* tk, const TriInv& ti, int64_t np, const float* l, int64_t ld, hipStream_t s) {
    NNGP_REQUIRE(tk != nullptr && ti.bs == kBs && np <= tk->np_cap, "tk_prepare_inverses: bad arguments");
    const int nb = (int)((np + kBs - 1) / kBs);
    const int tail = (int)(np - (int64_t)(nb - 1) * kBs);
    NNGP_HIP_CHECK(hipMemsetAsync(tk->amax, 0, sizeof(unsigned) * 2 * tk->nb_cap, s));
    const dim3 g1(64, (unsigned)nb), g2((unsigned)((int64_t)kBs * (kBs / 8) / 256), (unsigned)nb);
    hipLaunchKernelGGL(k_block_absmax, g1, dim3(256), 0, s, ti.xinv, (int64_t)kBs * kBs, tk->amax);
    hipLaunchKernelGGL(k_block_absmax, g1, dim3(256), 0, s, ti.tinv, (int64_t)kBs * kBs, tk->amax + tk->nb_cap);
    hipLaunchKernelGGL(k_split_blocks, g2, dim3(256), 0, s, ti.xinv, kBs, tk->amax, tk->xinv_s, tk->inv_iscale);
    hipLaunchKernelGGL(k_split_blocks, g2, dim3(256), 0, s, ti.tinv, kBs, tk->amax + tk->nb_cap, tk->tinv_s, tk->inv_iscale + tk->nb_cap);
    NNGP_HIP_CHECK(hipGetLastError());
    tk->inv_ready = true;
    tk->w_ready[0] = tk->w_ready[1] = false;
    const int forced = tk_dev_switches().merge;
    const bool want = forced >= 0 ? forced != 0 : (tk->m_cap / TT) * (int64_t)nb <= 192;
    if (l == nullptr || nb < 2 || !want) return 0;
    const int64_t blk = (int64_t)kBs * kBs;
    NNGP_HIP_CHECK(hipMemsetAsync(tk->wmax, 0, sizeof(unsigned) * 2 * tk->nb_cap, s));
    {
        const int full = (tail == kBs) ? nb - 1 : nb - 2;
        if (full > 0)
            NNGP_TRY(launch_gemm_nt_f32_batched(tk->wtmp, kBs, l + (int64_t)kBs * ld, ld, ti.tinv, kBs, kBs, kBs, kBs, 1.0f, 0.0f, false, full, blk,
                                                (int64_t)kBs * ld + kBs, blk, s, 2));
        if (full < nb - 1) {
            NNGP_HIP_CHECK(hipMemsetAsync(tk->wtmp + (int64_t)(nb - 2) * blk, 0, sizeof(float) * blk, s));
            NNGP_TRY(launch_gemm_nt_f32(tk->wtmp + (int64_t)(nb - 2) * blk, kBs, l + (int64_t)(nb - 1) * kBs * ld + (int64_t)(nb - 2) * kBs, ld,
                                        ti.tinv + (int64_t)(nb - 2) * blk, kBs, tail, kBs, kBs, 1.0f, 0.0f, false, s, 2));
        }
        const dim3 gw1(64, (unsigned)(nb - 1)), gw2((unsigned)((int64_t)kBs * (kBs / 8) / 256), (unsigned)(nb - 1));
        hipLaunchKernelGGL(k_block_absmax, gw1, dim3(256), 0, s, tk->wtmp, blk, tk->wmax);
        hipLaunchKernelGGL(k_split_blocks, gw2, dim3(256), 0, s, tk->wtmp, kBs, tk->wmax, tk->wplanes[0], tk->w_iscale);
        NNGP_HIP_CHECK(hipGetLastError());
        tk->w_ready[0] = true;
    }
    {
        hipLaunchKernelGGL(k_transpose_1024, dim3(32, 32, (unsigned)(nb - 1)), dim3(256), 0, s, l + (int64_t)kBs * ld, ld, (int64_t)kBs * ld + kBs, tk->ltb, tail,
                           nb - 1);
        const int full = (tail == kBs) ? nb - 1 : nb - 2;
        if (full > 0)
            NNGP_TRY(launch_gemm_nt_f32_batched(tk->wtmp + blk, kBs, tk->ltb, kBs, ti.xinv + blk, kBs, kBs, kBs, kBs, 1.0f, 0.0f, false, full, blk, blk, blk, s, 1));
        if (full < nb - 1) {
            NNGP_HIP_CHECK(hipMemsetAsync(tk->wtmp + (int64_t)(nb - 1) * blk, 0, sizeof(float) * blk, s));
            NNGP_TRY(launch_gemm_nt_f32(tk->wtmp + (int64_t)(nb - 1) * blk, kBs, tk->ltb + (int64_t)(nb - 2) * blk, kBs, ti.xinv + (int64_t)(nb - 1) * blk, kBs,
                                        kBs, tail, tail, 1.0f, 0.0f, false, s, 1));
        }
        const dim3 gw1(64, (unsigned)(nb - 1)), gw2((unsigned)((int64_t)kBs * (kBs / 8) / 256), (unsigned)(nb - 1));
        hipLaunchKernelGGL(k_block_absmax, gw1, dim3(256), 0, s, tk->wtmp + blk, blk, tk->wmax + tk->nb_cap + 1);
        hipLaunchKernelGGL(k_split_blocks, gw2, dim3(256), 0, s, tk->wtmp + blk, kBs, tk->wmax + tk->nb_cap + 1, tk->wplanes[1] + (int64_t)kBs * kLdp,
                           tk->w_iscale + tk->nb_cap + 1);
        NNGP_HIP_CHECK(hipGetLastError());
        tk->w_ready[1] = true;
    }
    return 0;
}

bool tk_inverses_ready(const TrsmTickets* tk) { return tk != nullptr && tk->inv_ready; }
void tk_invalidate_inverses(TrsmTickets* tk) { if (tk != nullptr) tk->inv_ready = false; }

bool tk_usable(const TrsmTickets* tk, int64_t m, int64_t np) {
    return tk != nullptr && tk->inv_ready && m % TT == 0 && m >= TT && m <= tk->m_cap && np % TT == 0 && np <= tk->np_cap && np >= 2 * kBs;
}

static int tk_ensure_tables(TrsmTickets* tk, int mt, int nb, int tail_ct) {
    TkTableKey key;
    key.mt = mt; key.nb = nb; key.tail_ct = tail_ct;
    key.merged[0] = (int)tk->w_ready[0]; key.merged[1] = (int)tk->w_ready[1];
    if (tk->key == key) return 0;
    NNGP_HIP_CHECK(hipDeviceSynchronize());
    tk->key = TkTableKey();
    for (int dir = 0; dir < 2; ++dir) {
        std::vector<TkItem> order;
        std::vector<int> qof;
        const int nq = (tk->nq == kMaxQ && (int64_t)mt * nb >= 32) ? kMaxQ : 1;
        tk->nq_dir[dir] = nq;
        tk_build_order(mt, nb, tail_ct, dir == 1, tk->workers, tk->w_ready[dir], order, nq, &qof, tk_dev_switches().order);
        NNGP_REQUIRE((int64_t)order.size() <= tk->items_cap, "tk_solve: item table overflow");
        std::vector<TkItem>& tab = tk->host_items[dir];
        tk_layout_tables(order, qof, nq, tab, tk->q_off[dir]);
        tk->n_items[dir] = (int)tab.size();
        NNGP_HIP_CHECK(hipMemcpy(tk->items[dir], tab.data(), sizeof(TkItem) * tab.size(), hipMemcpyHostToDevice));
    }
    tk->key = key;
    return 0;
}

static TkParams tk_params(const TrsmTickets* tk, float* b, int64_t ldb, const SplitWork& sw, bool backward) {
    const int dir = backward ? 1 : 0;
    TkParams P{};
    P.b = b; P.ldb = ldb;
    P.lplanes = backward ? sw.planes_t : sw.planes;
    P.l_stride = sw.col_stride;
    P.dinv_s = backward ? tk->tinv_s : tk->xinv_s;
    P.dinv_iscale = tk->inv_iscale + (backward ? tk->nb_cap : 0);
    P.wplanes = tk->wplanes[dir];
    P.w_iscale = tk->w_iscale + (backward ? tk->nb_cap : 0);
    P.planes_x = tk->planes_x; P.planes_d = tk->planes_d;
    P.p_stride = tk->m_cap * kLdp;
    P.rinv_x = tk->rinv_x; P.rinv_d = tk->rinv_d;
    P.r_stride = tk->m_cap;
    P.items = tk->items[dir];
    P.n_items = tk->n_items[dir];
    P.nq = tk->nq_dir[dir];
    for (int q = 0; q <= kMaxQ; ++q) P.q_off[q] = tk->q_off[dir][q];
    P.sync = tk->sync;
    P.mt = tk->key.mt; P.nb = tk->key.nb; P.tail_ct = tk->key.tail_ct;
    P.ctiles = (P.nb - 1) * 8 + P.tail_ct;
    P.l_iscale = 1.0f / sw.scale;
    P.backward = dir;
    P.spin_ticks = 200000000ULL;
    P.spin_max = 1u << 22;
    P.fault_ticket = -1;
    return P;
}

#ifdef NNGP_TIMING_KNOBS
static void tk_print_stamps(bool backward, int mt, int nb) {
    unsigned long long h[28];
    (void)hipDeviceSynchronize();
    if (hipMemcpyFromSymbol(h, HIP_SYMBOL(g_tk_stamps), sizeof(h)) != hipSuccess) return;
    static const char* names[6] = {"SB", "D", "SX", "U", "UB", "UW"};
    fprintf(stderr, "tk stamps (%s, mt %d nb %d): %llu workgroups, mean kernel time per workgroup %.1f us\n", backward ? "backward" : "forward", mt, nb, h[25],
            h[25] ? 0.01 * (double)h[24] / (double)h[25] : 0.0);
    for (int t = 0; t < 6; ++t)
        fprintf(stderr, "   %-2s items %6llu: wait %.2f us  body %.2f us  publish %.2f us per item; share of workgroup time: wait %.1f %% body %.1f %% publish %.1f %%\n", names[t],
                h[t * 4 + 3], h[t * 4 + 3] ? 0.01 * h[t * 4] / h[t * 4 + 3] : 0.0, h[t * 4 + 3] ? 0.01 * h[t * 4 + 1] / h[t * 4 + 3] : 0.0,
                h[t * 4 + 3] ? 0.01 * h[t * 4 + 2] / h[t * 4 + 3] : 0.0, 100.0 * h[t * 4] / (double)h[24], 100.0 * h[t * 4 + 1] / (double)h[24], 100.0 * h[t * 4 + 2] / (double)h[24]);
    unsigned long long z[28] = {};
    (void)hipMemcpyToSymbol(HIP_SYMBOL(g_tk_stamps), z, sizeof(z));
}
#endif

int tk_solve(TrsmTickets* tk, float* b, int64_t ldb, int64_t m, int64_t np, const SplitWork& sw, bool backward, hipStream_t s, int reserve_cus) {
    NNGP_REQUIRE(tk_usable(tk, m, np), "tk_solve: not usable for m=%lld np=%lld", (long long)m, (long long)np);
    NNGP_REQUIRE(sw.k_cap == kBs && (backward ? (sw.planes_t != nullptr && sw.lt_ready) : (sw.planes != nullptr && sw.l_ready)),
                 "tk_solve: split copy of the factor not available");
    NNGP_REQUIRE(ldb % 32 == 0 && ldb < (1LL << 26) && ((uintptr_t)b & 127) == 0, "tk_solve: right-hand sides must be 128-byte aligned rows");
    const int mt = (int)(m / TT), nb = (int)((np + kBs - 1) / kBs);
    const int tail_ct = (int)((np - (int64_t)(nb - 1) * kBs) / TT);
    NNGP_TRY(tk_ensure_tables(tk, mt, nb, tail_ct));
    TkParams P = tk_params(tk, b, ldb, sw, backward);
    if (const char* f = getenv("NNGP_TK_FAULT")) {
        P.fault_ticket = atoi(f);
        P.spin_ticks = 5000000ULL;
    }
    const int64_t used = SY_COUNTERS + 3LL * mt * nb + (int64_t)mt * P.ctiles;
    NNGP_REQUIRE(used <= tk->sync_ints, "tk_solve: counter block overflow");
    NNGP_HIP_CHECK(hipMemsetAsync(tk->sync, 0, sizeof(int) * SY_ERROR, s));
    NNGP_HIP_CHECK(hipMemsetAsync(tk->sync + SY_ERROR + 1, 0, sizeof(int) * (used - SY_ERROR - 1), s));
    int grid = tk->workers - (reserve_cus > 0 && reserve_cus < tk->workers / 2 ? reserve_cus : 0);
    if (grid > P.n_items) grid = P.n_items;
    hipLaunchKernelGGL(k_trsm_tickets, dim3((unsigned)grid), dim3(512), 0, s, P);
    NNGP_HIP_CHECK(hipGetLastError());
    NNGP_HIP_CHECK(hipMemcpyAsync(tk->host_err, tk->sync + SY_ERROR, sizeof(int), hipMemcpyDeviceToHost, s));
    NNGP_HIP_CHECK(hipEventRecord(tk->ev_err, s));
    tk->err_pending = true;
#ifdef NNGP_TIMING_KNOBS
    if (getenv("NNGP_TK_STAMPS") != nullptr) tk_print_stamps(backward, mt, nb);
#endif
    return 0;
}

int tk_poll_error(TrsmTickets* tk, bool wait) {
    if (tk == nullptr || !tk->err_pending) return 0;
    if (wait) {
        if (hipEventSynchronize(tk->ev_err) != hipSuccess) return -1;
    } else if (hipEventQuery(tk->ev_err) != hipSuccess) {
        (void)hipGetLastError();
        return 0;
    }
    tk->err_pending = false;
    const int e = tk->host_err[0];
    if (e != 0) {
        tk->host_err[0] = 0;
        (void)hipMemset(tk->sync + SY_ERROR, 0, sizeof(int));
    }
    return e;
}

}
```

Measured before the change: 173,000 GFLOP/s.

## Parallelize diag scale reduction, add split sym slicer, drop ticket CU reserve

The single-workgroup diagonal max/scale kernel is replaced by a multi-block atomicMax reduction followed by a parallel scale pass. A new 64-tile symmetric slice kernel and a head/tail split entry point are added. The ticket TRSM loses its reserve-CU parameter. The inverse split now reuses the tinv absmax for xinv unless a knob is set, which removes one reduction but changes the scaling of xinv.

```diff
diff --git a/include/nngp_i8s.h b/include/nngp_i8s.h
--- a/include/nngp_i8s.h
+++ b/include/nngp_i8s.h
@@ -13,6 +13,11 @@
 int nngp_i8s_cut_sym(const double* src, int64_t ld, int64_t n, int32_t ns, double* scale_out, int8_t* planes, int64_t ldp,
                      int32_t by_rows, double* sqsum, void* stream);
 
+int nngp_i8s_cut_sym_split(const double* src, int64_t ld, int64_t n, int32_t ns, double* scale_out, int8_t* planes, int64_t ldp,
+                           int32_t by_rows, int64_t small_from, double* sqsum, void* stream);
+
+int nngp_i8s_cut_sym_resources(int32_t ns, int32_t* num_regs, int64_t* lds_bytes);
+
 int nngp_i8s_residual(double* out, int64_t ldo, const double* cin, int64_t ldcin, double* z, int64_t ldz, const double* kmat,
                       int64_t ldk, int64_t mp, int64_t n, double alpha, double beta, double gamma, int32_t ns_z, int32_t ns_k,
                       int32_t cut, int32_t round_z, int32_t sym, float* out32, const double* base, double* var, double* delta,
diff --git a/nngp-src_amd/_lib.py b/nngp-src_amd/_lib.py
--- a/nngp-src_amd/_lib.py
+++ b/nngp-src_amd/_lib.py
@@ -62,7 +62,7 @@
                                "nngp_sparse_evidence_grad", "nngp_sparse_evidence_terms", "nngp_sparse_adjoint_rect")
 SPARSE_ARD_ABI_SYMBOLS = ("nngp_sparse_reserve_ard", "nngp_sparse_set_relevance", "nngp_sparse_evidence_grad_ard",
                           "nngp_sparse_ard_terms", "nngp_sparse_ard_rect")
-I8S_ABI_SYMBOLS = ("nngp_i8s_cut_rows", "nngp_i8s_cut_sym", "nngp_i8s_residual")
+I8S_ABI_SYMBOLS = ("nngp_i8s_cut_rows", "nngp_i8s_cut_sym", "nngp_i8s_cut_sym_split", "nngp_i8s_cut_sym_resources", "nngp_i8s_residual")
 MATFREE_ABI_SYMBOLS = ("nngp_matfree_create", "nngp_matfree_destroy", "nngp_matfree_fit", "nngp_matfree_solve",
                        "nngp_matfree_predict", "nngp_matfree_alpha", "nngp_matfree_info", "nngp_kmv_f64")
 BOUND_DTC, BOUND_VFE = 0, 1
@@ -377,6 +377,8 @@
     vp, i64, i32, dbl = ctypes.c_void_p, ctypes.c_int64, ctypes.c_int32, ctypes.c_double
     lib.nngp_i8s_cut_rows.argtypes = [vp, i64, i64, i64, i32, vp, vp, vp, i64, vp, vp]
     lib.nngp_i8s_cut_sym.argtypes = [vp, i64, i64, i32, vp, vp, i64, i32, vp, vp]
+    lib.nngp_i8s_cut_sym_split.argtypes = [vp, i64, i64, i32, vp, vp, i64, i32, i64, vp, vp]
+    lib.nngp_i8s_cut_sym_resources.argtypes = [i32, ctypes.POINTER(i32), ctypes.POINTER(i64)]
     lib.nngp_i8s_residual.argtypes = [vp, i64, vp, i64, vp, i64, vp, i64, i64, i64, dbl, dbl, dbl, i32, i32, i32, i32, i32,
                                       vp, vp, vp, vp, vp, vp, vp, vp]
     for name in I8S_ABI_SYMBOLS:
diff --git a/nngp-src_amd/csrc/api_ops.hip b/nngp-src_amd/csrc/api_ops.hip
--- a/nngp-src_amd/csrc/api_ops.hip
+++ b/nngp-src_amd/csrc/api_ops.hip
@@ -230,6 +230,11 @@
 
 int nngp_i8s_cut_sym(const double* src, int64_t ld, int64_t n, int32_t ns, double* scale_out, int8_t* planes, int64_t ldp,
                      int32_t by_rows, double* sqsum, void* stream) {
+    return nngp_i8s_cut_sym_split(src, ld, n, ns, scale_out, planes, ldp, by_rows, n, sqsum, stream);
+}
+
+int nngp_i8s_cut_sym_split(const double* src, int64_t ld, int64_t n, int32_t ns, double* scale_out, int8_t* planes, int64_t ldp,
+                           int32_t by_rows, int64_t small_from, double* sqsum, void* stream) {
     hipStream_t s = (hipStream_t)stream;
     NNGP_REQUIRE(src != nullptr && planes != nullptr && scale_out != nullptr, "i8s_cut_sym: NULL argument");
     NNGP_REQUIRE(by_rows != 0 ? (ns >= 2 && ns <= 7) : (ns == 5 || ns == 7), "i8s_cut_sym: 5 or 7 planes (by rows: 2..7) (ns=%d)", (int)ns);
@@ -237,12 +242,30 @@
                  TB, (long long)n, (long long)ld);
     NNGP_REQUIRE(ldp >= n && ldp % 16 == 0, "i8s_cut_sym: ldp must be a multiple of 16 and >= n (ldp=%lld)", (long long)ldp);
     NNGP_REQUIRE((((uintptr_t)src | (uintptr_t)planes) & 15) == 0, "i8s_cut_sym: operands must be 16-byte aligned");
-    NNGP_TRY(launch_i8s_diag_bound_scale(src, ld, n, scale_out, s));
-    if (by_rows != 0)
-        NNGP_TRY(launch_i8s_slice_rows(src, ld, n, n, ns, scale_out, nullptr, planes, ldp, n * ldp, s));
-    else
-        NNGP_TRY(launch_i8s_slice_sym(src, ld, n, ns, scale_out, planes, ldp, n * ldp, s));
-    if (sqsum != nullptr) NNGP_TRY(launch_i8s_scale_sqsum(scale_out, n, sqsum, s));
+    NNGP_REQUIRE(small_from >= 0 && small_from <= n && small_from % TB == 0, "i8s_cut_sym: small_from must be a multiple of %d in [0, n] (small_from=%lld)",
+                 TB, (long long)small_from);
+    double* word = sqsum;
+    if (word == nullptr) NNGP_HIP_CHECK(hipMalloc((void**)&word, sizeof(double)));
+    int rc = launch_i8s_diag_bound_scale(src, ld, n, scale_out, word, s);
+    if (rc == 0 && by_rows != 0) rc = launch_i8s_slice_rows(src, ld, n, n, ns, scale_out, nullptr, planes, ldp, n * ldp, s);
+    else {
+        if (rc == 0) rc = launch_i8s_slice_sym(src, ld, n, ns, scale_out, planes, ldp, n * ldp, s, I8S_SYM_HEAD, small_from);
+        if (rc == 0) rc = launch_i8s_slice_sym(src, ld, n, ns, scale_out, planes, ldp, n * ldp, s, I8S_SYM_TAIL, small_from);
+    }
+    if (sqsum != nullptr) {
+        if (rc == 0) rc = launch_i8s_scale_sqsum(scale_out, n, sqsum, s);
+    } else {
+        (void)hipStreamSynchronize(s);
+        (void)hipFree(word);
+    }
+    return rc;
+}
+
+int nngp_i8s_cut_sym_resources(int32_t ns, int32_t* num_regs, int64_t* lds_bytes) {
+    NNGP_REQUIRE((ns == 5 || ns == 7) && num_regs != nullptr && lds_bytes != nullptr, "i8s_cut_sym_resources: 5 or 7 planes, two outputs");
+    int regs = 0;
+    NNGP_TRY(i8s_slice_sym_resources(ns, &regs, lds_bytes));
+    *num_regs = regs;
     return 0;
 }
 
@@ -259,7 +282,7 @@
                     bool round_z, bool sym, float* out32, const double* base, double* var, double* delta, double* zstat,
                     double* floor_rows, double* floor_z, hipStream_t s) {
     const int64_t kr = round_up(n, 256), zr = round_up(mp, 256);
-    NNGP_TRY(launch_i8s_diag_bound_scale(kmat, ldk, n, w.kscale, s));
+    NNGP_TRY(launch_i8s_diag_bound_scale(kmat, ldk, n, w.kscale, w.kscale + n, s));
     if (sym)
         NNGP_TRY(launch_i8s_slice_sym(kmat, ldk, n, ns_k, w.kscale, w.kplanes, n, kr * n, s));
     else
diff --git a/nngp-src_amd/csrc/api_predict.hip b/nngp-src_amd/csrc/api_predict.hip
--- a/nngp-src_amd/csrc/api_predict.hip
+++ b/nngp-src_amd/csrc/api_predict.hip
@@ -158,20 +158,18 @@
     return use_tickets(m, mp) ? SolvePath::Tickets : SolvePath::BlocksH3;
 }
 
-struct TicketSchedule { int gate, reserve, cutstream; };
+struct TicketSchedule { int gate, cutstream; };
 static const TicketSchedule& ticket_schedule() {
 #ifdef NNGP_TIMING_KNOBS
     auto env = [](const char* name, int dflt) { const char* v = getenv(name); return v ? atoi(v) : dflt; };
-    static const TicketSchedule t = {env("NNGP_TK_GATE", 1), env("NNGP_TK_RESERVE", 0), env("NNGP_TK_CUTSTREAM", 2)};
+    static const TicketSchedule t = {env("NNGP_TK_GATE", 1), env("NNGP_TK_CUTSTREAM", 2)};
 #else
-    static const TicketSchedule t = {1, 0, 2};
+    static const TicketSchedule t = {1, 2};
 #endif
     return t;
 }
 
 bool cg_from_the_start(const nngp_model* m, int64_t mp) { return ticket_schedule().gate != 0 && solve_path(m, mp) == SolvePath::Tickets; }
-
-int tickets_reserve(const nngp_model* m) { return m->i8.k_pending ? ticket_schedule().reserve : 0; }
 
 hipStream_t early_cut_stream(const nngp_model* m, int64_t mp) {
     const int cut_stream = ticket_schedule().cutstream;
@@ -210,7 +208,7 @@
     m->split.solve_reserve = (m->alpha_solve.gate_recorded && NNGP_KNOB(13) > 0) ? NNGP_KNOB(13) : 0;
     switch (solve_path(m, mp)) {
     case SolvePath::Recursion128: return trsm_rlt_f32(m->b32, m->np, mp, m->a32, m->ld, m->dinv, m->np, s);
-    case SolvePath::Tickets: return tk_solve(m->tk, m->b32, m->np, mp, m->np, m->split, false, s, tickets_reserve(m));
+    case SolvePath::Tickets: return tk_solve(m->tk, m->b32, m->np, mp, m->np, m->split, false, s);
     case SolvePath::BlocksH3: return trsm_rlt_blocks_h3(m->b32, m->np, mp, m->a32, m->ld, m->tri, m->np, m->trsm_tmp, m->split, s);
     case SolvePath::BlocksF32: break;
     }
@@ -238,7 +236,7 @@
     int slot = -1;
     NNGP_TRY(trsm_timer_begin(m, mp, s, &slot));
     if (path == SolvePath::Tickets)
-        NNGP_TRY(tk_solve(m->tk, m->b32, m->np, mp, m->np, m->split, true, s, tickets_reserve(m)));
+        NNGP_TRY(tk_solve(m->tk, m->b32, m->np, mp, m->np, m->split, true, s));
     else if (path == SolvePath::BlocksH3)
         NNGP_TRY(trsm_rut_blocks_h3(m->b32, m->np, mp, m->lt_ready ? m->lt32 : nullptr, m->np, m->tri, m->np, m->trsm_tmp, m->split, s));
     else
diff --git a/nngp-src_amd/csrc/common.h b/nngp-src_amd/csrc/common.h
--- a/nngp-src_amd/csrc/common.h
+++ b/nngp-src_amd/csrc/common.h
@@ -247,7 +247,8 @@
 };
 int i8s_plan(int nsa, int nsb, int cut, I8Plan* pl);
 int64_t i8s_chunks(int64_t k, const I8Plan* pl = nullptr);
-int launch_i8s_diag_bound_scale(const double* src, int64_t ld, int64_t n, double* scale, hipStream_t s);
+int launch_i8s_diag_bound_scale(const double* src, int64_t ld, int64_t n, double* scale, double* mx_word, hipStream_t s);
+int i8s_slice_sym_resources(int ns, int* num_regs, int64_t* lds_bytes);
 int launch_i8s_scale_sqsum(const double* scale, int64_t n, double* out, hipStream_t s);
 int launch_i8s_floor_ratio(const double* z, int64_t ld, int64_t rows, int64_t cols, const double* var, const I8Plan& pl, int nsa, int nsb,
                            const double* sk2, unsigned long long* out, hipStream_t s);
@@ -256,7 +257,8 @@
 int launch_i8s_slice_rows(const double* src, int64_t ld, int64_t rows, int64_t cols, int ns, const double* scale_in, double* scale_out,
                           int8_t* planes, int64_t ldp, int64_t pstride, hipStream_t s, double* writeback = nullptr);
 int launch_i8s_slice_sym(const double* src, int64_t ld, int64_t n, int ns, const double* scale, int8_t* planes, int64_t ldp,
-                         int64_t pstride, hipStream_t s);
+                         int64_t pstride, hipStream_t s, int part = 0, int64_t split_row = 0);
+enum { I8S_SYM_ALL = 0, I8S_SYM_HEAD = 1, I8S_SYM_TAIL = 2 };
 int launch_gemm_nt_i8s(int32_t* partial, int64_t ldc, int64_t slab, const int8_t* a, int64_t lda, int64_t sa, const int8_t* b,
                        int64_t ldb, int64_t sb, const I8Plan& pl, int64_t m, int64_t n, int64_t k, int* counters, int reserve_cus,
                        hipStream_t s);
@@ -305,7 +307,7 @@
 bool tk_inverses_ready(const TrsmTickets* tk);
 void tk_invalidate_inverses(TrsmTickets* tk);
 bool tk_usable(const TrsmTickets* tk, int64_t m, int64_t np);
-int tk_solve(TrsmTickets* tk, float* b, int64_t ldb, int64_t m, int64_t np, const SplitWork& sw, bool backward, hipStream_t s, int reserve_cus = 0);
+int tk_solve(TrsmTickets* tk, float* b, int64_t ldb, int64_t m, int64_t np, const SplitWork& sw, bool backward, hipStream_t s);
 int tk_poll_error(TrsmTickets* tk, bool wait);
 int launch_symv_f64(const double* a, int64_t lda, int64_t n, const double* x, double* y, double diag_add, double* part,
                     int64_t np, hipStream_t s);
diff --git a/nngp-src_amd/csrc/gemm_i8s.hip b/nngp-src_amd/csrc/gemm_i8s.hip
--- a/nngp-src_amd/csrc/gemm_i8s.hip
+++ b/nngp-src_amd/csrc/gemm_i8s.hip
@@ -30,21 +30,20 @@
     return a < 1.0e300 ? a : __builtin_inf();
 }
 
-__global__ __launch_bounds__(1024) void k_i8s_diag_bound_scale(const double* __restrict__ src, int64_t ld, int64_t n,
-                                                               double* __restrict__ scale) {
-    __shared__ double red[16];
-    double mx = 0.0;
-    for (int64_t i = threadIdx.x; i < n; i += 1024) mx = fmax(mx, i8s_mag(src[i * ld + i]));
+__global__ __launch_bounds__(256) void k_i8s_diag_max(const double* __restrict__ src, int64_t ld, int64_t n, unsigned long long* mx_bits) {
+    const int64_t i = (int64_t)blockIdx.x * 256 + threadIdx.x;
+    double mx = i < n ? i8s_mag(src[i * ld + i]) : 0.0;
 #pragma unroll
     for (int off = 32; off > 0; off >>= 1) mx = fmax(mx, __shfl_xor(mx, off));
-    if ((threadIdx.x & 63) == 0) red[threadIdx.x >> 6] = mx;
-    __syncthreads();
-    mx = 0.0;
-#pragma unroll
-    for (int i = 0; i < 16; ++i) mx = fmax(mx, red[i]);
-    for (int64_t i = threadIdx.x; i < n; i += 1024) {
-        scale[i] = i8s_scale_of(sqrt(fabs(src[i * ld + i]) * mx) * (1.0 + 1e-9));
-    }
+    if ((threadIdx.x & 63) == 0 && mx > 0.0) atomicMax(mx_bits, (unsigned long long)__double_as_longlong(mx));
+}
+
+__global__ __launch_bounds__(256) void k_i8s_diag_bound_scale(const double* __restrict__ src, int64_t ld, int64_t n,
+                                                              const unsigned long long* __restrict__ mx_bits, double* __restrict__ scale) {
+    const int64_t i = (int64_t)blockIdx.x * 256 + threadIdx.x;
+    if (i >= n) return;
+    const double mx = __longlong_as_double((long long)mx_bits[0]);
+    scale[i] = i8s_scale_of(sqrt(fabs(src[i * ld + i]) * mx) * (1.0 + 1e-9));
 }
 
 template <int NS>
@@ -181,6 +180,85 @@
         i8s_digits16<NS>(tile + (16 * g) * kSymLd + col, kSymLd, top / scale[r], dig);
 #pragma unroll
         for (int s = 0; s < NS; ++s) *reinterpret_cast<i32x4*>(planes + s * pstride + r * ldp + I * kSymT + 16 * g) = dig[s];
+    }
+}
+
+constexpr int kSymS = 64, kSymH = 32;
+
+constexpr int kSymSLd = kSymS + 9;
+__device__ __forceinline__ int i8s_sym_at(int r, int c) { return r * kSymSLd + c + ((c >> 5) << 3); }
+
+template <int NS>
+__host__ __device__ __forceinline__ unsigned long long i8s_digit_bytes(long long x) {
+    unsigned long long bias = 0;
+#pragma unroll
+    for (int s = 0; s < NS - 1; ++s) bias |= 0x80ull << (8 * s);
+    return ((unsigned long long)x + bias) ^ bias;
+}
+
+template <int NS>
+__device__ __forceinline__ void i8s_digits16_at(const double* v, int at, int step, double inv, i32x4* dig) {
+#pragma unroll
+    for (int q = 0; q < 4; ++q) {
+        unsigned long long z[4];
+#pragma unroll
+        for (int j = 0; j < 4; ++j) {
+            z[j] = i8s_digit_bytes<NS>(__double2ll_rn(v[at] * inv));
+            at += step;
+            asm volatile("" : "+v"(at));
+            if (j & 1) __builtin_amdgcn_sched_barrier(0);
+        }
+#pragma unroll
+        for (int s = 0; s < NS; ++s) {
+            const int sh = 8 * (NS - 1 - s);
+            dig[s][q] = (int)((unsigned)((z[0] >> sh) & 255) | ((unsigned)((z[1] >> sh) & 255) << 8) | ((unsigned)((z[2] >> sh) & 255) << 16) |
+                              ((unsigned)((z[3] >> sh) & 255) << 24));
+        }
+    }
+}
+
+template <int NS>
+__global__ __launch_bounds__(256) void k_i8s_slice_sym_small(const double* __restrict__ src, int64_t ld, const double* __restrict__ scale,
+                                                             int8_t* __restrict__ planes, int64_t ldp, int64_t pstride, long long first_tile) {
+    __shared__ double tile[kSymH * kSymSLd];
+    const int t = threadIdx.x;
+    const long long b = first_tile + blockIdx.x;
+    long long I = (long long)((sqrt(8.0 * (double)b + 1.0) - 1.0) * 0.5);
+    while ((I + 1) * (I + 2) / 2 <= b) ++I;
+    while (I * (I + 1) / 2 > b) --I;
+    const long long J = b - I * (I + 1) / 2;
+    const double top = ldexp(1.0, 8 * NS);
+    const int item = t & 127;
+    const bool direct = t < 128;
+    const bool active = direct || I != J;
+    const int g = direct ? item & 3 : item & 1, rc = direct ? item >> 2 : item >> 1;
+    const int first = direct ? i8s_sym_at(rc, 16 * g) : i8s_sym_at(16 * g, rc), step = direct ? 1 : kSymSLd;
+    int64_t r = (direct ? I : J) * kSymS + rc;
+    int8_t* dst = planes + r * ldp + (direct ? J : I) * kSymS + 16 * g;
+    const int64_t r_pass = direct ? kSymH : 0, dst_pass = direct ? kSymH * ldp : kSymH;
+    const double* p = src + (I * kSymS + (t >> 5)) * ld + J * kSymS + 2 * (t & 31);
+#pragma unroll 1
+    for (int h = 0; h < 2; ++h) {
+        if (h != 0) __syncthreads();
+#pragma unroll
+        for (int i = 0; i < 4; ++i) {
+            const int row = 8 * i + (t >> 5), col = 2 * (t & 31);
+            const f64x2 v = *reinterpret_cast<const f64x2*>(p + (int64_t)(8 * i) * ld);
+            tile[i8s_sym_at(row, col)] = v[0];
+            tile[i8s_sym_at(row, col + 1)] = v[1];
+        }
+        __syncthreads();
+        if (active) {
+            i32x4 dig[NS];
+            int8_t* d = dst;
+            asm volatile("" : "+v"(d));
+            i8s_digits16_at<NS>(tile, first, step, top / scale[r], dig);
+#pragma unroll
+            for (int s = 0; s < NS; ++s) *reinterpret_cast<i32x4*>(d + s * pstride) = dig[s];
+        }
+        p += (int64_t)kSymH * ld;
+        r += r_pass;
+        dst += dst_pass;
     }
 }
 
@@ -508,13 +586,21 @@
 }
 
 
-__global__ __launch_bounds__(1024) void k_i8s_scale_sqsum(const double* __restrict__ scale, int64_t n, double* __restrict__ out) {
+__global__ __launch_bounds__(256) void k_i8s_scale_sqsum(const double* __restrict__ scale, int64_t n, double* __restrict__ out) {
     __shared__ double red[16];
-    double s = 0.0;
-    for (int64_t i = threadIdx.x; i < n; i += 1024) s += scale[i] * scale[i];
-#pragma unroll
-    for (int off = 32; off > 0; off >>= 1) s += __shfl_down(s, off);
-    if ((threadIdx.x & 63) == 0) red[threadIdx.x >> 6] = s;
+    double acc[4];
+#pragma unroll
+    for (int k = 0; k < 4; ++k) {
+        double s = 0.0;
+        for (int64_t i = 256 * k + threadIdx.x; i < n; i += 1024) s += scale[i] * scale[i];
+#pragma unroll
+        for (int off = 32; off > 0; off >>= 1) s += __shfl_down(s, off);
+        acc[k] = s;
+    }
+    if ((threadIdx.x & 63) == 0) {
+#pragma unroll
+        for (int k = 0; k < 4; ++k) red[4 * k + (threadIdx.x >> 6)] = acc[k];
+    }
     __syncthreads();
     if (threadIdx.x == 0) {
         double t = 0.0;
@@ -565,10 +651,24 @@
 
 }
 
-int launch_i8s_diag_bound_scale(const double* src, int64_t ld, int64_t n, double* scale, hipStream_t s) {
+int launch_i8s_diag_bound_scale(const double* src, int64_t ld, int64_t n, double* scale, double* mx_word, hipStream_t s) {
     if (n <= 0) return 0;
-    hipLaunchKernelGGL(k_i8s_diag_bound_scale, dim3(1), dim3(1024), 0, s, src, ld, n, scale);
+    NNGP_REQUIRE(mx_word != nullptr && (mx_word < scale || mx_word >= scale + n), "i8s_diag_bound_scale: scratch word inside the scales");
+    unsigned long long* mx_bits = reinterpret_cast<unsigned long long*>(mx_word);
+    const dim3 g((unsigned)((n + 255) / 256));
+    NNGP_HIP_CHECK(hipMemsetAsync(mx_bits, 0, sizeof(unsigned long long), s));
+    hipLaunchKernelGGL(k_i8s_diag_max, g, dim3(256), 0, s, src, ld, n, mx_bits);
+    hipLaunchKernelGGL(k_i8s_diag_bound_scale, g, dim3(256), 0, s, src, ld, n, mx_bits, scale);
     NNGP_HIP_CHECK(hipGetLastError());
+    return 0;
+}
+
+int i8s_slice_sym_resources(int ns, int* num_regs, int64_t* lds_bytes) {
+    hipFuncAttributes a;
+    if (ns == 7) NNGP_HIP_CHECK(hipFuncGetAttributes(&a, reinterpret_cast<const void*>(k_i8s_slice_sym_small<7>)));
+    else NNGP_HIP_CHECK(hipFuncGetAttributes(&a, reinterpret_cast<const void*>(k_i8s_slice_sym_small<5>)));
+    *num_regs = a.numRegs;
+    *lds_bytes = (int64_t)a.sharedSizeBytes;
     return 0;
 }
 
@@ -593,13 +693,25 @@
 }
 
 int launch_i8s_slice_sym(const double* src, int64_t ld, int64_t n, int ns, const double* scale, int8_t* planes, int64_t ldp,
-                         int64_t pstride, hipStream_t s) {
+                         int64_t pstride, hipStream_t s, int part, int64_t split_row) {
     if (n <= 0) return 0;
     NNGP_REQUIRE((ns == 5 || ns == 7) && n % kSymT == 0 && ld % 2 == 0 && ((uintptr_t)src & 15) == 0 && ((uintptr_t)planes & 15) == 0 &&
                      ldp >= n && ldp % 16 == 0 && pstride % 16 == 0 && scale != nullptr,
                  "i8s_slice_sym: 5 or 7 planes of a matrix padded to 128");
-    const int64_t tn = n / kSymT, tiles = tn * (tn + 1) / 2;
+    NNGP_REQUIRE(part == I8S_SYM_ALL || (split_row >= 0 && split_row <= n && split_row % kSymT == 0), "i8s_slice_sym: bad split row");
+    if (part == I8S_SYM_TAIL) {
+        const int64_t t0 = split_row / kSymS, t1 = n / kSymS;
+        const int64_t first = t0 * (t0 + 1) / 2, count = t1 * (t1 + 1) / 2 - first;
+        NNGP_REQUIRE(count < 2147483647LL, "i8s_slice_sym: too many tiles");
+        if (count <= 0) return 0;
+        if (ns == 5) hipLaunchKernelGGL(k_i8s_slice_sym_small<5>, dim3((unsigned)count), dim3(256), 0, s, src, ld, scale, planes, ldp, pstride, (long long)first);
+        else hipLaunchKernelGGL(k_i8s_slice_sym_small<7>, dim3((unsigned)count), dim3(256), 0, s, src, ld, scale, planes, ldp, pstride, (long long)first);
+        NNGP_HIP_CHECK(hipGetLastError());
+        return 0;
+    }
+    const int64_t tn = (part == I8S_SYM_HEAD ? split_row : n) / kSymT, tiles = tn * (tn + 1) / 2;
     NNGP_REQUIRE(tiles < 2147483647LL, "i8s_slice_sym: too many tiles");
+    if (tiles <= 0) return 0;
     if (ns == 5) hipLaunchKernelGGL(k_i8s_slice_sym<5>, dim3((unsigned)tiles), dim3(256), 0, s, src, ld, scale, planes, ldp, pstride);
     else hipLaunchKernelGGL(k_i8s_slice_sym<7>, dim3((unsigned)tiles), dim3(256), 0, s, src, ld, scale, planes, ldp, pstride);
     NNGP_HIP_CHECK(hipGetLastError());
@@ -607,7 +719,7 @@
 }
 
 int launch_i8s_scale_sqsum(const double* scale, int64_t n, double* out, hipStream_t s) {
-    hipLaunchKernelGGL(k_i8s_scale_sqsum, dim3(1), dim3(1024), 0, s, scale, n, out);
+    hipLaunchKernelGGL(k_i8s_scale_sqsum, dim3(1), dim3(256), 0, s, scale, n, out);
     NNGP_HIP_CHECK(hipGetLastError());
     return 0;
 }
diff --git a/nngp-src_amd/csrc/model.h b/nngp-src_amd/csrc/model.h
--- a/nngp-src_amd/csrc/model.h
+++ b/nngp-src_amd/csrc/model.h
@@ -280,7 +280,6 @@
 inline bool needs_lt32(SolvePath p) { return p == SolvePath::Recursion128 || p == SolvePath::BlocksF32; }
 bool cg_from_the_start(const nngp_model* m, int64_t mp);
 hipStream_t early_cut_stream(const nngp_model* m, int64_t mp);
-int tickets_reserve(const nngp_model* m);
 int tickets_check(nngp_model* m, bool wait);
 int apply_forward_f32(nngp_model* m, int64_t mp, hipStream_t s);
 int apply_inverse_f32(nngp_model* m, int64_t mp, hipStream_t s);
diff --git a/nngp-src_amd/csrc/residual_i8.hip b/nngp-src_amd/csrc/residual_i8.hip
--- a/nngp-src_amd/csrc/residual_i8.hip
+++ b/nngp-src_amd/csrc/residual_i8.hip
@@ -79,7 +79,7 @@
 
 static int i8s_cut_planes(nngp_model* m, I8Planes& pk, const double* kmat, int64_t kld, hipStream_t s) {
     I8Work& w = m->i8.work;
-    NNGP_TRY(launch_i8s_diag_bound_scale(kmat, kld, m->np, pk.scale, s));
+    NNGP_TRY(launch_i8s_diag_bound_scale(kmat, kld, m->np, pk.scale, pk.scale + m->np_cap, s));
     const bool sym = (kmat == m->kaux64 || m->k64_symmetric) && (pk.alloc_planes == 5 || pk.alloc_planes == 7) && NNGP_KNOB(5) != 62;
     if (sym)
         NNGP_TRY(launch_i8s_slice_sym(kmat, kld, m->np, pk.alloc_planes, pk.scale, pk.planes, m->np_cap, w.k_rows * m->np_cap, s));
diff --git a/nngp-src_amd/csrc/trsm_tickets.hip b/nngp-src_amd/csrc/trsm_tickets.hip
--- a/nngp-src_amd/csrc/trsm_tickets.hip
+++ b/nngp-src_amd/csrc/trsm_tickets.hip
@@ -812,10 +812,14 @@
     const int tail = (int)(np - (int64_t)(nb - 1) * kBs);
     NNGP_HIP_CHECK(hipMemsetAsync(tk->amax, 0, sizeof(unsigned) * 2 * tk->nb_cap, s));
     const dim3 g1(64, (unsigned)nb), g2((unsigned)((int64_t)kBs * (kBs / 8) / 256), (unsigned)nb);
-    hipLaunchKernelGGL(k_block_absmax, g1, dim3(256), 0, s, ti.xinv, (int64_t)kBs * kBs, tk->amax);
-    hipLaunchKernelGGL(k_block_absmax, g1, dim3(256), 0, s, ti.tinv, (int64_t)kBs * kBs, tk->amax + tk->nb_cap);
-    hipLaunchKernelGGL(k_split_blocks, g2, dim3(256), 0, s, ti.xinv, kBs, tk->amax, tk->xinv_s, tk->inv_iscale);
-    hipLaunchKernelGGL(k_split_blocks, g2, dim3(256), 0, s, ti.tinv, kBs, tk->amax + tk->nb_cap, tk->tinv_s, tk->inv_iscale + tk->nb_cap);
+    const unsigned* xmax = tk->amax;
+    hipLaunchKernelGGL(k_block_absmax, g1, dim3(256), 0, s, ti.tinv, (int64_t)kBs * kBs, tk->amax);
+    if (NNGP_KNOB(9) == 17) {
+        hipLaunchKernelGGL(k_block_absmax, g1, dim3(256), 0, s, ti.xinv, (int64_t)kBs * kBs, tk->amax + tk->nb_cap);
+        xmax = tk->amax + tk->nb_cap;
+    }
+    hipLaunchKernelGGL(k_split_blocks, g2, dim3(256), 0, s, ti.xinv, kBs, xmax, tk->xinv_s, tk->inv_iscale);
+    hipLaunchKernelGGL(k_split_blocks, g2, dim3(256), 0, s, ti.tinv, kBs, tk->amax, tk->tinv_s, tk->inv_iscale + tk->nb_cap);
     NNGP_HIP_CHECK(hipGetLastError());
     tk->inv_ready = true;
     tk->w_ready[0] = tk->w_ready[1] = false;
@@ -937,7 +941,7 @@
 }
 #endif
 
-int tk_solve(TrsmTickets* tk, float* b, int64_t ldb, int64_t m, int64_t np, const SplitWork& sw, bool backward, hipStream_t s, int reserve_cus) {
+int tk_solve(TrsmTickets* tk, float* b, int64_t ldb, int64_t m, int64_t np, const SplitWork& sw, bool backward, hipStream_t s) {
     NNGP_REQUIRE(tk_usable(tk, m, np), "tk_solve: not usable for m=%lld np=%lld", (long long)m, (long long)np);
     NNGP_REQUIRE(sw.k_cap == kBs && (backward ? (sw.planes_t != nullptr && sw.lt_ready) : (sw.planes != nullptr && sw.l_ready)),
                  "tk_solve: split copy of the factor not available");
@@ -954,7 +958,7 @@
     NNGP_REQUIRE(used <= tk->sync_ints, "tk_solve: counter block overflow");
     NNGP_HIP_CHECK(hipMemsetAsync(tk->sync, 0, sizeof(int) * SY_ERROR, s));
     NNGP_HIP_CHECK(hipMemsetAsync(tk->sync + SY_ERROR + 1, 0, sizeof(int) * (used - SY_ERROR - 1), s));
-    int grid = tk->workers - (reserve_cus > 0 && reserve_cus < tk->workers / 2 ? reserve_cus : 0);
+    int grid = tk->workers;
     if (grid > P.n_items) grid = P.n_items;
     hipLaunchKernelGGL(k_trsm_tickets, dim3((unsigned)grid), dim3(512), 0, s, P);
     NNGP_HIP_CHECK(hipGetLastError());
```

New measurement: 172,800 GFLOP/s. About the same (-0.1%).
